# osmocom/osmo-trx

Hardware: AMD Instinct MI355X
Metric: Mbursts/s detect+demod (156.25 sym, 4 SPS) (higher is better)
Workload: dtype f32

## Files before the change

### osmo_trx_amd/csrc/trx_kernel_nb.hip

```cpp
#include "trx_k4_common.h"
#include "trx_nb_asm.inc"

#define NB_D_LEN    160
#define NB_CZ_LEN   (TRX_CZ_PAD + TRX_CORR_NARROW + TRX_CZ_PAD)
#define NB_SLICE    (K4_XS + NB_D_LEN + NB_CZ_LEN)
#define NB_COMP_ROWS (TRX_DELAY_FILTS + 1)
#define NB_TABLES_FLOATS (TRX_SINCV_LDS + 16 * WAVE + NB_COMP_ROWS * 36 + 16 + 8 * 8 + 5 * WAVE + 5 * WAVE + 2 * 8 * 16)
#define NB_TABLES_BYTES (NB_TABLES_FLOATS * 4)
#define NB_WPB 16
#define NB_POOL_RING 64
#define NB_POOL_UNSET (-1)
#define NB_POOL_END (-2)
#define NB_NO_BURST 0xffffffffu
#define NB_LDS_TAIL (16 + 4 * NB_POOL_RING)
#define NB_LDS_BYTES (NB_TABLES_BYTES + NB_WPB * NB_SLICE * 8 + NB_LDS_TAIL)
#define NB_MAX_TOA 32



typedef float v3f __attribute__((ext_vector_type(3)));
typedef int v4i __attribute__((ext_vector_type(4)));

template <typename T>
__device__ __forceinline__ unsigned lds_addr(const T *p)
{
	return (unsigned)(uintptr_t)(const __attribute__((address_space(3))) T *)p;
}

__global__ void __launch_bounds__(NB_WPB * WAVE)
nb_pull4_kernel(const uint32_t *__restrict__ iq, const trxhip_burst_params *__restrict__ params,
		trxhip_burst_result *__restrict__ results, float *__restrict__ soft, const trx_tables *__restrict__ tab,
		unsigned n_bursts, float thresh, float full_scale, unsigned *__restrict__ pool_ctr, unsigned *__restrict__ redo,
		float gk5, float gk6, float gk7, float gk8)
{
	static_assert(NB_TABLES_BYTES % 16 == 0 && (NB_SLICE * 8) % 16 == 0 && (K4_XS * 8) % 16 == 0 && (NB_D_LEN * 8) % 16 == 0, "16-byte LDS accesses");
	static_assert(NB_LDS_BYTES <= 160 * 1024, "LDS");
	static_assert(NB_ASM_GDEC_OFF == (TRX_SINCV_LDS + 16 * WAVE + NB_COMP_ROWS * 36) * 4, "tools/gen_nb_asm.py: LDS offset of the decimator taps");
	static_assert(NB_ASM_DEC_MAX_NACT == 15 + NB_ASM_CORR_MAX_LEN, "tools/gen_nb_asm.py: DEC and CORR change form at the same window");
	static_assert(NB_ASM_LSEQ_OFF == (NB_TABLES_FLOATS - 2 * 8 * 16) * 4, "tools/gen_nb_asm.py: LDS offset of the training-sequence taps");
	constexpr int NLD = 10;
	extern __shared__ __attribute__((aligned(16))) char smem[];
	const int lane0 = threadIdx.x & (WAVE - 1);
	const int wave = uni((int)(threadIdx.x >> 6));

	float *const sincv = reinterpret_cast<float *>(smem);
	float *const wa4f = sincv + TRX_SINCV_LDS;
	const float4 *const wa4 = reinterpret_cast<const float4 *>(wa4f);
	float *const comp = wa4f + 16 * WAVE;
	float *const gdec = comp + NB_COMP_ROWS * 36;
	float *const lhdr = gdec + 16;
	int *const pkcl = reinterpret_cast<int *>(lhdr + 8 * 8);
	int *const lcn = pkcl + 5 * WAVE;
	c32 *const lseq = reinterpret_cast<c32 *>(lcn + 5 * WAVE);
	c32 *const wbase = reinterpret_cast<c32 *>(smem + NB_TABLES_BYTES) + (size_t)wave * NB_SLICE;
	int *const wg_next = reinterpret_cast<int *>(reinterpret_cast<c32 *>(smem + NB_TABLES_BYTES) + (size_t)NB_WPB * NB_SLICE);
	int *const pool_g = wg_next + 4;
	c32 *const P = wbase;
	c32 *const D = wbase + K4_XS;
	c32 *const cz = D + NB_D_LEN + TRX_CZ_PAD;

	for (int i = threadIdx.x; i < TRX_SINCV_LDS; i += blockDim.x)
		sincv[i] = (i < TRX_SINCV_LEN) ? tab->sincv[i] : 0.0f;
	for (int i = threadIdx.x; i < 16 * WAVE; i += blockDim.x) {
		const int l = i & (WAVE - 1), u = i >> 6;
		const PeakConst pcl = peak_const(l);
		const int q = (u < 8) ? pcl.loA + 512 * (7 - u) : pcl.hiA + 512 * (u - 8);
		wa4f[((u >> 2) * WAVE + l) * 4 + (u & 3)] = (q < TRX_SINCV_LEN) ? tab->sincv[q] : 0.0f;
	}
	for (int i = threadIdx.x; i < NB_COMP_ROWS * 36; i += blockDim.x) {
		const int f = i / 36, j = i % 36;
		comp[i] = (j >= TRX_FUSED_SH) ? tab->comp_filt[f][j - TRX_FUSED_SH] : 0.0f;
	}
	if (threadIdx.x < 16)
		gdec[threadIdx.x] = tab->dec_taps[threadIdx.x];
	if (threadIdx.x < 128)
		lseq[threadIdx.x] = make_float2(tab->seq[TRX_SEQ_TSC0 + (threadIdx.x >> 4)].taps[threadIdx.x & 15].re,
						tab->seq[TRX_SEQ_TSC0 + (threadIdx.x >> 4)].taps[threadIdx.x & 15].im);
	if (threadIdx.x < 64)
		lhdr[threadIdx.x] = reinterpret_cast<const float *>(&tab->seq[TRX_SEQ_TSC0 + (threadIdx.x >> 3)].gain)[threadIdx.x & 7];
	if (threadIdx.x < WAVE) {
		const PeakConst pc0 = peak_const(threadIdx.x);
		pkcl[0 * WAVE + threadIdx.x] = pc0.flA;
		pkcl[1 * WAVE + threadIdx.x] = pc0.loA;
		pkcl[2 * WAVE + threadIdx.x] = pc0.hiA;
		pkcl[3 * WAVE + threadIdx.x] = pc0.offB;
		pkcl[4 * WAVE + threadIdx.x] = pc0.ratio_off;
		lcn[0 * WAVE + threadIdx.x] = pc0.ratio_off * 8;
		lcn[1 * WAVE + threadIdx.x] = (pc0.flA - 8) * 8;
		lcn[2 * WAVE + threadIdx.x] = pc0.offB;
		const int l = threadIdx.x, e = (l - 52) / 3, t = (l - 52) % 3;
		const bool sp = l >= 52;
		lcn[3 * WAVE + l] = 8 * (sp ? (t == 0 ? e : t == 1 ? e + 3 : e - 3) : 4 + 3 * (l < 49 ? l : 49));
		lcn[4 * WAVE + l] = sp ? (e + (t == 2 ? 4 : 0)) * K4_NTP * 4 : -1;
	}
	for (int i = lane0; i < NB_SLICE; i += WAVE)
		wbase[i] = make_float2(0.0f, 0.0f);
	if (threadIdx.x == 0) {
		wg_next[0] = NB_WPB;
		wg_next[1] = 0;
	}
	if (threadIdx.x < NB_POOL_RING)
		pool_g[threadIdx.x] = NB_POOL_UNSET;
	__syncthreads();

	const float fs_db = 6.02059991f * __log2f(full_scale);
	const float thr2 = thresh * thresh;
	const float gc0 = thr2 * 1.0001e-5f;
	int t5pk = 0;
	bool t5_ok = true;
	for (int t = 0; t < 8; t++) {
		const int v = (int)(lhdr[8 * t + 5] * 512.0f);
		t5_ok = t5_ok && v >= -8 && v <= 7 && (float)v == lhdr[8 * t + 5] * 512.0f;
		t5pk |= (v & 15) << (4 * t);
	}
	t5pk = uni(t5pk);
	const unsigned long long e8_addr = reinterpret_cast<unsigned long long>(&tab->edge8[0][0][0]);
	const unsigned n_wg = gridDim.x;
	const unsigned n_groups = (n_bursts + 15u) >> 4;
	const bool pooled = pool_ctr != nullptr;
	const unsigned n_static_groups = pooled ? ((n_groups - (n_groups >> 3)) / n_wg) * n_wg : n_groups;
	const unsigned n_pool_groups = n_groups - n_static_groups;
	const unsigned gq = n_static_groups / n_wg, gr = n_static_groups % n_wg;
	const unsigned my_groups = gq + (blockIdx.x < gr ? 1u : 0u);
	const unsigned base16 = (blockIdx.x * gq + (blockIdx.x < gr ? blockIdx.x : gr)) << 4;
	unsigned items = my_groups << 4;
	if (base16 + items > n_bursts)
		items = (base16 < n_bursts) ? n_bursts - base16 : 0u;
	auto burst_of = [&](unsigned jj) -> unsigned {
		if (jj < items)
			return base16 + jj;
		if (!pooled)
			return NB_NO_BURST;
		const unsigned k = (jj - items) >> 4;
		volatile int *slot = pool_g + (k & (NB_POOL_RING - 1));
		int g;
		while ((g = *slot) == NB_POOL_UNSET)
			__builtin_amdgcn_s_sleep(2);
		g = uni(g);
		if (g < 0)
			return NB_NO_BURST;
		const unsigned bb = ((n_static_groups + (unsigned)g) << 4) + (jj & 15u);
		return bb < n_bursts ? bb : NB_NO_BURST;
	};
	auto pool_draw = [&](unsigned jj, bool ended, int lane) {
		const unsigned k = (jj + 16u - items) >> 4;
		int g = NB_POOL_END;
		if (!ended) {
			unsigned p = 0;
			if (lane == 0)
				p = __hip_atomic_fetch_add(pool_ctr, 1u, __ATOMIC_RELAXED, __HIP_MEMORY_SCOPE_AGENT);
			p = (unsigned)uni((int)p);
			g = (p < n_pool_groups) ? (int)p : NB_POOL_END;
		}
		if (lane == 0) {
			pool_g[(k + NB_POOL_RING / 2) & (NB_POOL_RING - 1)] = NB_POOL_UNSET;
			pool_g[k & (NB_POOL_RING - 1)] = g;
		}
	};

	uint32_t pre_i[NLD];
	uint32_t pre_prm = 0u;
	auto prefetch = [&](unsigned bb, int lane) {
		pre_prm = reinterpret_cast<const uint32_t *>(params)[2 * (size_t)bb];
		const uint32_t *src = iq + (size_t)bb * 625;
		const unsigned ul = (unsigned)lane & 63u;
#pragma unroll
		for (int r = 0; r < NLD - 1; r++)
			pre_i[r] = __builtin_nontemporal_load(src + (unsigned)(r * WAVE) + ul);
		pre_i[NLD - 1] = __builtin_nontemporal_load(src + (unsigned)((NLD - 1) * WAVE) + min(ul, 48u));
	};
	const unsigned b_first = burst_of((unsigned)wave);
	if (b_first != NB_NO_BURST)
		prefetch(b_first, lane0);

	v3f o = { 0.0f, 0.0f, 0.0f };
	int recw = 0;
	bool pend_any = false;
	bool pend_rec = false;
	unsigned pend_b = 0;
	bool left_any = false;
	int q_xr = 0, q_xi = 0, q_es = 0, q_toa = 0, q_s = 0, q_fl = 0, q_b = 0;
	int q_n = 0;
	auto flush_records = [&](const int lane) {
		if (lane < q_n) {
			const float *const h = lhdr + 8 * (q_fl & 0xff);
			const float xr = __int_as_float(q_xr), xi = __int_as_float(q_xi);
			const float a0 = xr * h[2], a1 = xr * h[3], a2 = xi * h[3], a3 = xi * h[2];
			const float amp_re = a0 - a2, amp_im = a1 + a3;
			const float toa = (float)q_toa * 0.001953125f;
			const float energy = __int_as_float(q_es) * 0.0125f;
			const float rssi = fs_db - 3.01029996f * __log2f(energy);
			const float p2 = xi * xi + xr * xr;
			const float C = p2 * h[7];
			const float S = __int_as_float(q_s);
			const float ci = 3.0103f * __log2f(C * __builtin_amdgcn_rcpf(S - C));
			const v4i r0 = { 1, __float_as_int(toa), __float_as_int(amp_re), __float_as_int(amp_im) };
			const v4i r1 = { __float_as_int(ci), __float_as_int(energy), __float_as_int(rssi), q_fl };
			asm volatile("global_store_dwordx4 %0, %1, off\n\t"
				     "global_store_dwordx4 %0, %2, off offset:16\n\t"
				     "s_nop 1"
				     :: "v"(results + (unsigned)q_b), "v"(r0), "v"(r1) : "memory");
		}
		q_n = 0;
	};

	auto demod_general = [&](const int nk, const c32 ampv, const int lane) -> bool {
		constexpr int L = 625, nwrite = 148;
		c32 *const dec = D;
		const trx_tables *tabc = tab;
		asm volatile("" : "+s"(tabc));
		const int w = nk >> 7, fr = nk & 127;
		const int fidx = (fr >= 2) ? (fr >> 1) : TRX_DELAY_FILTS;
		const float ian = __builtin_amdgcn_rcpf(norm2(ampv));
		const c32 scale = make_float2(ampv.x * ian, -ampv.y * ian);
		const int n_lo = w > 0 ? w : 0;
		const int n_hi = (L - 1 + w < 623) ? L - 1 + w : 623;
		const int i_full_lo = cdiv4(n_lo + 15), i_full_hi = fdiv4(n_hi);
		const int i0l = cdiv4(n_lo), i0h = i_full_hi + 1;
		const bool need_lo = (n_hi >= n_lo) && (i0l < i_full_lo) && (i0l < nwrite);
		const bool need_hi = (n_hi >= n_lo) && (i0h <= fdiv4(n_hi + 15)) && (i0h < nwrite);
		const bool lo_tab = need_lo && (n_hi >= 4 * (i_full_lo - 1));
		float ct0 = 0.0f, ct1 = 0.0f, ct2 = 0.0f;
		const int le = lane >> 4, lt = lane & 15;
		const int li = i0l + le;
		const int lt0 = n_lo + 15 - 4 * li;
		const bool lact = lt0 >= 1;
		if (lo_tab) {
			const float *row = &tabc->edge_lo[fidx][(lact ? lt0 : 1) - 1][lt];
			ct0 = row[0];
			ct1 = row[16];
			ct2 = (lt < 4) ? row[32] : 0.0f;
		}
		const bool hi_tab = need_hi && (w <= -2) && (n_lo <= 4 * i0h - 15);
		if ((need_lo && !lo_tab) || (need_hi && !hi_tab))
			return false;
		float ch0 = 0.0f, ch1 = 0.0f, ch2 = 0.0f;
		const int hi_i = i0h + le;
		const int htm = n_hi + 15 - 4 * hi_i;
		const bool hact = htm >= 0;
		if (hi_tab) {
			const float *row = &tabc->edge_hi[fidx][hact ? htm : 0][lt];
			ch0 = row[0];
			ch1 = row[16];
			ch2 = (lt < 4) ? row[32] : 0.0f;
		}
		{
			const int c_full = -24 - w;
			const int i_min = cdiv4(-36 - c_full), i_max = fdiv4(L + 1 - c_full);
			int ic = 3 * lane;
			if (ic < i_min) ic = i_min;
			if (ic > i_max - 2) ic = i_max - 2;
			v2f acc[3];
			asm volatile(NB_ASM_FIRG
				     : [a0] "=&v"(acc[0]), [a1] "=&v"(acc[1]), [a2] "=&v"(acc[2])
				     : [nk] "s"(nk), [pb] "s"(lds_addr(P)), [cb] "s"(lds_addr(comp) + 4u * (K4_U0 + TRX_FUSED_SH)), [kic] "v"(8 * ic)
				     : NB_ASM_CLOBBERS);
			if (n_lo == 0 && lo_tab && i_full_hi >= nwrite - 1) {
				if (lane < 52) {
#pragma unroll
					for (int j = 0; j < 3; j++)
						dec[3 * lane + j] = cmul(make_float2(acc[j].x, acc[j].y), scale);
				}
			} else {
#pragma unroll
				for (int j = 0; j < 3; j++) {
					const int i = 3 * lane + j;
					const bool full = (i >= i_full_lo) && (i <= i_full_hi);
					const c32 d = full ? cmul(make_float2(acc[j].x, acc[j].y), scale) : make_float2(0.0f, 0.0f);
					if (i < 156)
						dec[i] = d;
				}
			}
		}
		if (lo_tab) {
			const int s0 = 4 * li - 24 - w + lt;
			const c32 *pp = P + ((s0 & 3) * PH_A + PH_M0 + (s0 >> 2));
			const c32 x0 = lds_c32(pp), x1 = lds_c32(pp + 4), x2 = lds_c32(pp + 8);
			float ar = x0.x * ct0, ai = x0.y * ct0;
			ar = fmaf(x1.x, ct1, ar); ai = fmaf(x1.y, ct1, ai);
			ar = fmaf(x2.x, ct2, ar); ai = fmaf(x2.y, ct2, ai);
			const float sr = row_sum(ar), si = row_sum(ai);
			if (lt == 0 && lact)
				dec[li] = cmul(make_float2(sr, si), scale);
		}
		if (hi_tab) {
			const int s0 = 4 * hi_i - 24 - w + lt;
			const c32 *pp = P + ((s0 & 3) * PH_A + PH_M0 + (s0 >> 2));
			const c32 x0 = lds_c32(pp), x1 = lds_c32(pp + 4), x2 = lds_c32(pp + 8);
			float ar = x0.x * ch0, ai = x0.y * ch0;
			ar = fmaf(x1.x, ch1, ar); ai = fmaf(x1.y, ch1, ai);
			ar = fmaf(x2.x, ch2, ar); ai = fmaf(x2.y, ch2, ai);
			const float sr = row_sum(ar), si = row_sum(ai);
			if (lt == 0 && hact && hi_i < 156)
				dec[hi_i] = cmul(make_float2(sr, si), scale);
		}
		wave_sync();
		auto pick = [&](int i) {
			const float d = reinterpret_cast<const float *>(dec + i)[i & 1];
			return __builtin_amdgcn_fmed3f(fmaf((i & 2) ? -0.5f : 0.5f, d, 0.5f), 0.0f, 1.0f);
		};
		const bool reg = lane >= 2 && lane < 50;
		const int i0 = reg ? 3 * lane - 2 : ((((lane - 54) * 11) >> 5) & 3);
		o.x = pick(i0);
		o.y = pick(reg ? i0 + 1 : 0);
		o.z = pick(reg ? i0 + 2 : 0);
		wave_sync();
		return true;
	};

	DIAG_DECL;
	unsigned j_next = 0, b_next = NB_NO_BURST;
	for (unsigned b = b_first; b != NB_NO_BURST; b = b_next) {
		int lane;
		asm volatile("v_mbcnt_lo_u32_b32 %0, -1, 0\n\tv_mbcnt_hi_u32_b32 %0, -1, %0" : "=v"(lane));
		const int ticket = claim_issue(wg_next);
		const unsigned prm0 = (unsigned)uni((int)pre_prm);
		const unsigned max_toa = prm0 >> 16;
		const int tsc = (prm0 >> 8) & 0xff;
		bool leave = ((prm0 & 0xf8ffu) != (unsigned)TRXHIP_TSC) || (max_toa > NB_MAX_TOA) || !t5_ok;

		c32 *const pload = P + (lane & 3) * PH_A + PH_M0 + (lane >> 2);
		float amax = 0.0f, epart = 0.0f;
#ifdef TRX_DIAG
		DIAG_MARK(12);
		asm volatile("s_waitcnt vmcnt(0)" ::: "memory");
		DIAG_MARK(13);
#endif
		if (!leave) {
#pragma unroll
			for (int r = 0; r < NLD; r++) {
				const int i = r * WAVE + lane;
				if (r < NLD - 1 || i < 625) {
					const c32 v = make_float2((float)(int16_t)(pre_i[r] & 0xffffu), (float)(int16_t)(pre_i[r] >> 16));
					pload[16 * r] = v;
					asm("v_max3_f32 %0, %0, |%1|, |%2|" : "+v"(amax) : "v"(v.x), "v"(v.y));
					if (r < 5)
						epart = fmaf(v.x, v.x, fmaf(v.y, v.y, epart));
				}
			}
		} else {
#pragma unroll
			for (int r = 0; r < NLD; r++)
				asm volatile("" :: "v"(pre_i[r]));
		}
		DIAG_MARK(14);
		if (pend_any) {
			float *const so = soft + (size_t)pend_b * 148;
			int *const rp = reinterpret_cast<int *>(results + pend_b);
			const float oe = o.x;
			asm volatile("s_bfm_b64 exec, 48, 2\n\t"
				     "global_store_dwordx3 %0, %1, %2 offset:16\n\t"
				     "s_mov_b32 exec_lo, 0\n\t"
			     "s_mov_b32 exec_hi, 0x92400000\n\t"
				     "global_store_dword %3, %4, %2\n\t"
				     "s_mov_b64 exec, %8\n\t"
				     "global_store_dword %5, %6, %7\n\t"
				     "s_mov_b64 exec, -1\n\t"
				     "s_nop 0"
				     :: "v"((lane - 2) * 12), "v"(o), "s"(so), "v"((((lane - 54) * 11) >> 5) * 4), "v"(oe), "v"(lane * 4), "v"(recw), "s"(rp),
				        "s"(pend_rec ? 0xffull : 0ull)
				     : "memory");
		}
		pend_any = false;
		DIAG_MARK(16);
		j_next = (unsigned)(leave ? claim_take(ticket) : claim_take_behind<5>(ticket));
		b_next = burst_of(j_next);
		if (pooled && (j_next & 15u) == 0u && j_next + 16u >= items)
			pool_draw(j_next, b_next == NB_NO_BURST && j_next >= items, lane);
		DIAG_MARK(17);
		if (b_next != NB_NO_BURST)
			prefetch(b_next, lane);
		DIAG_MARK(15);

		int clip = 0;
		if (!leave) {
			clip = __ballot(amax > TRX_CLIP_THRESH) != 0ull;

			const int len = 16 + (int)max_toa;
			__builtin_assume(len >= 16 && len <= 16 + NB_MAX_TOA);
			const unsigned vd_addr = lds_addr(D) + 8u * (unsigned)lane, vcz_addr = lds_addr(cz) + 8u * (unsigned)lane;
			unsigned long long bad;
			float dr, di;
			asm volatile(NB_ASM_DEC
				     : [bad] "=s"(bad), [dr] "=&v"(dr), [di] "=&v"(di)
				     : [pd] "v"(lds_addr(P + PH_M0 + 52) + 8u * (unsigned)lane), [vd] "v"(vd_addr), [vd4] "v"(vd_addr - 32u), [zero] "v"(0),
				       [nact] "s"(15 + len)
				     : NB_ASM_CLOBBERS);
			DIAG_MARK(2);
			{
				float v;
				const int lag0 = (len <= NB_ASM_CORR_MAX_LEN) ? NB_ASM_CORR_LANE0 : 0;
				asm volatile(NB_ASM_CORR
					     : [nrm] "=&v"(v)
					     : [vd] "v"(vd_addr), [vcz] "v"(vcz_addr), [vdm] "v"(vd_addr - 8u * NB_ASM_CORR_LANE0),
					       [vczm] "v"(vcz_addr - 8u * NB_ASM_CORR_LANE0), [dr] "v"(dr), [di] "v"(di), [len] "s"(len), [tsc] "s"(tsc), [bad] "s"(bad)
					     : NB_ASM_CLOBBERS);
				DIAG_MARK(3);
				int m_bits, es_bits, bidx;
				int kr, ka, kb, kic, ktp;
				asm volatile(NB_ASM_AMAX("ds_read_b32 %[kr], %[l4] offset:%c[lc]", "ds_read_b32 %[ka], %[l4] offset:%c[lc]+256",
							 "ds_read_b32 %[kb], %[l4] offset:%c[lc]+512", "ds_read_b32 %[kic], %[l4] offset:%c[lc]+768",
							 "ds_read_b32 %[ktp], %[l4] offset:%c[lc]+1024", "s_nop 0", "s_nop 0", "s_nop 0")
					     "s_sub_u32 %[bidx], %[bidx], %[lag0]\n\t"
					     "s_waitcnt lgkmcnt(0)"
					     : [m] "=&s"(m_bits), [es] "=&s"(es_bits), [bidx] "=&s"(bidx), [kr] "=&v"(kr), [ka] "=&v"(ka), [kb] "=&v"(kb),
					       [kic] "=&v"(kic), [ktp] "=&v"(ktp)
					     : [nrm] "v"(v), [ep] "v"(epart), [l4] "v"(4 * lane), [lag0] "s"(lag0),
					       [lc] "n"((TRX_SINCV_LDS + 16 * WAVE + NB_COMP_ROWS * 36 + 16 + 64 + 5 * WAVE) * 4)
					     : NB_ASM_CLOBBERS);
				DIAG_MARK(4);
				int hit = 0;
				int toa512 = 0;
				if (m_bits != 0) {
					int st, e512;
					float km;
					asm volatile(NB_ASM_DETA
						     : [st] "=&s"(st), [e] "=&s"(e512), [km] "=&v"(km)
						     : [bidx] "s"(bidx), [len] "s"(len), [czb] "s"(lds_addr(cz)), [kr] "v"(kr), [ka] "v"(ka), [l16] "v"(16 * lane),
						       [k5] "s"(gk5), [k6] "s"(gk6), [k7] "s"(gk7), [k8] "s"(gk8), [c0] "v"(gc0)
						     : NB_ASM_CLOBBERS);
					DIAG_MARK(5);
					int xr_bits = 0, xi_bits = 0;
					if (st == 1) {
						asm volatile(NB_ASM_DETB
							     : [st] "=&s"(st), [toa] "=&s"(toa512), [xr] "=&s"(xr_bits), [xi] "=&s"(xi_bits)
							     : [e] "s"(e512), [kb] "v"(kb), [czb] "s"(lds_addr(cz)), [km] "v"(km)
							     : NB_ASM_CLOBBERS);
						DIAG_MARK(6);
					}
					if (st == 3) {
						if (lane == 0)
							atomicAdd(&g_trx_fast_stats[0], 1ull);
						PeakConst pkc;
						pkc.flA = pkcl[0 * WAVE + lane]; pkc.loA = pkcl[1 * WAVE + lane]; pkc.hiA = pkcl[2 * WAVE + lane];
						pkc.offB = pkcl[3 * WAVE + lane]; pkc.ratio_off = pkcl[4 * WAVE + lane];
						c32 xcorr;
						peak_detect_spec(cz, bidx, sincv, pkc, lane, &toa512, &xcorr, wa4);
						toa512 = uni(toa512);
						xr_bits = uni(__float_as_int(xcorr.x));
						xi_bits = uni(__float_as_int(xcorr.y));
						st = 1;
					}
					if (st == 2) {
						leave = true;
						if (lane == 0) atomicAdd(&g_trx_fast_stats[2], 1ull);
					}
					if (st == 1) {
						hit = 1;
						int ok, s_bits;
						float d0, d1, d2;
						const int t5 = (t5pk << (28 - 4 * tsc)) >> 28;
						asm volatile("s_setprio 0");
						asm volatile(NB_ASM_TAIL
							     : [ok] "=&s"(ok), [ssum] "=&s"(s_bits), [d0] "=&v"(d0), [d1] "=&v"(d1), [d2] "=&v"(d2)
							     : [toa] "s"(toa512), [xr] "s"(xr_bits), [xi] "s"(xi_bits), [t5] "s"(t5), [hdrb] "s"(lds_addr(lhdr) + 32u * (unsigned)tsc),
							       [e8lo] "s"((unsigned)e8_addr), [e8hi] "s"((unsigned)(e8_addr >> 32)), [l16] "v"(16 * lane),
							       [vd] "v"(vd_addr), [pb] "s"(lds_addr(P)), [cb] "s"(lds_addr(comp) + 4u * (K4_U0 + TRX_FUSED_SH)), [db] "s"(lds_addr(D)),
							       [kic] "v"(kic), [ktp] "v"(ktp)
							     : NB_ASM_CLOBBERS);
						DIAG_MARK(10);
						asm volatile("s_setprio 2");
						if (!ok) {
							if (lane == 0) atomicAdd(&g_trx_fast_stats[3], 1ull);
							const float *const h = lhdr + 8 * tsc;
							const float xr = __int_as_float(xr_bits), xi = __int_as_float(xi_bits);
							const float a0 = xr * h[2], a1 = xr * h[3], a2 = xi * h[3], a3 = xi * h[2];
							const c32 ampv = make_float2(unif(a0 - a2), unif(a1 + a3));
							if (!demod_general(t5 + 10 * 512 - toa512, ampv, lane))
								leave = true;
						}
						if (!leave) {
							asm("s_lshl_b64 exec, 1, %[n]\n\t"
						    "v_mov_b32_e32 %[qxr], %[xr]\n\t"
						    "v_mov_b32_e32 %[qxi], %[xi]\n\t"
						    "v_mov_b32_e32 %[qes], %[es]\n\t"
						    "v_mov_b32_e32 %[qtoa], %[toa]\n\t"
						    "v_mov_b32_e32 %[qs], %[ss]\n\t"
						    "v_mov_b32_e32 %[qfl], %[fl]\n\t"
						    "v_mov_b32_e32 %[qb], %[b]\n\t"
						    "s_mov_b64 exec, -1"
						    : [qxr] "+v"(q_xr), [qxi] "+v"(q_xi), [qes] "+v"(q_es), [qtoa] "+v"(q_toa), [qs] "+v"(q_s), [qfl] "+v"(q_fl),
						      [qb] "+v"(q_b)
						    : [n] "s"(uni(q_n)), [xr] "s"(xr_bits), [xi] "s"(xi_bits), [es] "s"(es_bits), [toa] "s"(toa512 - t5 - 10 * 512),
						      [ss] "s"(s_bits), [fl] "s"((int)((uint32_t)tsc | ((uint32_t)clip << 8) | (37u << 24))), [b] "s"((int)b));
						q_n++;
						}
						if (ok) {
							o.x = __builtin_amdgcn_fmed3f(fmaf(0.5f, d0, 0.5f), 0.0f, 1.0f);
							o.y = __builtin_amdgcn_fmed3f(fmaf(0.5f, d1, 0.5f), 0.0f, 1.0f);
							o.z = __builtin_amdgcn_fmed3f(fmaf(0.5f, d2, 0.5f), 0.0f, 1.0f);
						}
					}
				}
				if (!hit && !leave) {
					const float energy = __int_as_float(es_bits) * 0.0125f;
					const float rssi = fs_db - 3.01029996f * __log2f(energy);
					const uint32_t flags = ((uint32_t)clip << 8) | (1u << 16);
					int word = clip ? -TRXHIP_SIGERR_CLIP : 0;
					word = put_lane<1>(word, 0.0f);
					word = put_lane<2>(word, 0.0f);
					word = put_lane<3>(word, 0.0f);
					word = put_lane<4>(word, 0.0f);
					word = put_lane<5>(word, energy);
					word = put_lane<6>(word, rssi);
					word = write_lane<7>(word, (int)flags);
					recw = word;
					o = (v3f){ 0.0f, 0.0f, 0.0f };
				}
				pend_rec = !hit;
			}
		}
		if (leave) {
			if (lane == 0) {
				reinterpret_cast<uint8_t *>(redo + TRX_REDO_HDR)[b] = 1;
				if (!left_any)
					__hip_atomic_store(redo, 1u, __ATOMIC_RELAXED, __HIP_MEMORY_SCOPE_AGENT);
			}
			left_any = true;
			continue;
		}
		pend_b = b;
		pend_any = true;
		if (q_n == WAVE)
			flush_records(lane);
		DIAG_MARK(11);
	}
	if (pend_any) {
		int lane;
		asm volatile("v_mbcnt_lo_u32_b32 %0, -1, 0\n\tv_mbcnt_hi_u32_b32 %0, -1, %0" : "=v"(lane));
		float *const so = soft + (size_t)pend_b * 148;
		int *const rp = reinterpret_cast<int *>(results + pend_b);
		const float oe = o.x;
		asm volatile("s_bfm_b64 exec, 48, 2\n\t"
			     "global_store_dwordx3 %0, %1, %2 offset:16\n\t"
		     "s_mov_b32 exec_lo, 0\n\t"
		     "s_mov_b32 exec_hi, 0x92400000\n\t"
			     "global_store_dword %3, %4, %2\n\t"
			     "s_mov_b64 exec, %8\n\t"
			     "global_store_dword %5, %6, %7\n\t"
			     "s_mov_b64 exec, -1\n\t"
			     "s_nop 0"
			     :: "v"((lane - 2) * 12), "v"(o), "s"(so), "v"((((lane - 54) * 11) >> 5) * 4), "v"(oe), "v"(lane * 4), "v"(recw), "s"(rp),
			        "s"(pend_rec ? 0xffull : 0ull)
			     : "memory");
	}
	{
		int lane;
		asm volatile("v_mbcnt_lo_u32_b32 %0, -1, 0\n\tv_mbcnt_hi_u32_b32 %0, -1, %0" : "=v"(lane));
		flush_records(lane);
	}
	DIAG_FLUSH();
	if (pooled) {
		__syncthreads();
		int tid0;
		asm volatile("v_mbcnt_lo_u32_b32 %0, -1, 0\n\tv_mbcnt_hi_u32_b32 %0, -1, %0" : "=v"(tid0));
		if (tid0 == 0 && atomicAdd(wg_next + 1, 1) == 0) {
			const unsigned d = __hip_atomic_fetch_add(pool_ctr + 1, 1u, __ATOMIC_ACQ_REL, __HIP_MEMORY_SCOPE_AGENT);
			if (d == gridDim.x - 1u) {
				__hip_atomic_store(pool_ctr, 0u, __ATOMIC_RELAXED, __HIP_MEMORY_SCOPE_AGENT);
				__hip_atomic_store(pool_ctr + 1, 0u, __ATOMIC_RELEASE, __HIP_MEMORY_SCOPE_AGENT);
			}
		}
	}
}
```

### osmo_trx_amd/csrc/trx_nb_asm.inc

```
#define NB_ASM_GDEC_OFF 29968
#define NB_ASM_LSEQ_OFF 32848
#define NB_ASM_DEC_MAX_NACT 60
#define NB_ASM_CORR_LANE0 19
#define NB_ASM_CORR_MAX_LEN 45
#define NB_ASM_CLOBBERS "v64", "v65", "v66", "v67", "v68", "v69", "v70", "v71", "v72", "v73", "v74", "v75", "v76", "v77", "v78", "v79", "v80", "v81", "v82", "v83", "v84", "v85", "v86", "v87", "v88", "v89", "v90", "v91", "v92", "v93", "v94", "v95", "v96", "v97", "v98", "v99", "v100", "v101", "v102", "v103", "v104", "v105", "v106", "v107", "v108", "v109", "v110", "v111", "v112", "v113", "v114", "v115", "v116", "v117", "v118", "v119", "v120", "v121", "v122", "v123", "v124", "v125", "v126", "v127", "s87", "s88", "s89", "s90", "s91", "s92", "s93", "s94", "s95", "s96", "s97", "s98", "s99", "vcc", "scc", "memory"
#define NB_ASM_DEC \
	"s_cmp_gt_u32 %[nact], 60\n\t" \
	"s_cbranch_scc1 .Lnb_dec_wide\n\t" \
	"s_sub_u32 s88, 60, %[nact]\n\t" \
	"s_lshr_b64 exec, -1, s88\n\t" \
	"ds_read_b128 v[120:123], %[zero] offset:29968\n\t" \
	"ds_read_b128 v[124:127], %[zero] offset:29984\n\t" \
	"ds_read_b64 v[98:99], %[pd] offset:1440\n\t" \
	"ds_read_b64 v[100:101], %[pd] offset:2880\n\t" \
	"ds_read_b64 v[102:103], %[pd] offset:4320\n\t" \
	"ds_read_b64 v[96:97], %[pd] offset:0\n\t" \
	"s_waitcnt lgkmcnt(3)\n\t" \
	"v_pk_mul_f32 v[64:65], v[98:99], v[120:121] op_sel:[0,0] op_sel_hi:[1,0]\n\t" \
	"s_waitcnt lgkmcnt(2)\n\t" \
	"v_pk_mul_f32 v[66:67], v[100:101], v[120:121] op_sel:[0,1] op_sel_hi:[1,1]\n\t" \
	"s_waitcnt lgkmcnt(1)\n\t" \
	"v_pk_mul_f32 v[68:69], v[102:103], v[122:123] op_sel:[0,0] op_sel_hi:[1,0]\n\t" \
	"v_pk_add_f32 v[104:105], v[64:65], v[66:67]\n\t" \
	"s_waitcnt lgkmcnt(0)\n\t" \
	"v_pk_mul_f32 v[70:71], v[96:97], v[122:123] op_sel:[0,1] op_sel_hi:[1,1]\n\t" \
	"v_pk_add_f32 v[104:105], v[104:105], v[68:69]\n\t" \
	"v_pk_mul_f32 v[72:73], v[98:99], v[124:125] op_sel:[0,0] op_sel_hi:[1,0]\n\t" \
	"v_pk_mul_f32 v[74:75], v[100:101], v[124:125] op_sel:[0,1] op_sel_hi:[1,1]\n\t" \
	"v_add_f32_dpp v104, v104, v70 wave_shr:1 row_mask:0xf bank_mask:0xf bound_ctrl:0\n\t" \
	"v_add_f32_dpp v105, v105, v71 wave_shr:1 row_mask:0xf bank_mask:0xf bound_ctrl:0\n\t" \
	"v_pk_mul_f32 v[76:77], v[102:103], v[126:127] op_sel:[0,0] op_sel_hi:[1,0]\n\t" \
	"v_pk_add_f32 v[104:105], v[104:105], v[72:73]\n\t" \
	"v_pk_mul_f32 v[78:79], v[96:97], v[126:127] op_sel:[0,1] op_sel_hi:[1,1]\n\t" \
	"v_pk_add_f32 v[104:105], v[104:105], v[74:75]\n\t" \
	"v_pk_mul_f32 v[80:81], v[98:99], v[126:127] op_sel:[0,1] op_sel_hi:[1,1]\n\t" \
	"v_pk_add_f32 v[104:105], v[104:105], v[76:77]\n\t" \
	"v_pk_mul_f32 v[82:83], v[100:101], v[126:127] op_sel:[0,0] op_sel_hi:[1,0]\n\t" \
	"v_pk_mul_f32 v[84:85], v[102:103], v[124:125] op_sel:[0,1] op_sel_hi:[1,1]\n\t" \
	"v_add_f32_dpp v104, v104, v78 wave_shr:1 row_mask:0xf bank_mask:0xf bound_ctrl:0\n\t" \
	"v_add_f32_dpp v105, v105, v79 wave_shr:1 row_mask:0xf bank_mask:0xf bound_ctrl:0\n\t" \
	"v_pk_mul_f32 v[86:87], v[96:97], v[124:125] op_sel:[0,0] op_sel_hi:[1,0]\n\t" \
	"v_pk_add_f32 v[104:105], v[104:105], v[80:81]\n\t" \
	"v_pk_mul_f32 v[88:89], v[98:99], v[122:123] op_sel:[0,1] op_sel_hi:[1,1]\n\t" \
	"v_pk_add_f32 v[104:105], v[104:105], v[82:83]\n\t" \
	"v_pk_mul_f32 v[90:91], v[100:101], v[122:123] op_sel:[0,0] op_sel_hi:[1,0]\n\t" \
	"v_pk_add_f32 v[104:105], v[104:105], v[84:85]\n\t" \
	"v_pk_mul_f32 v[92:93], v[102:103], v[120:121] op_sel:[0,1] op_sel_hi:[1,1]\n\t" \
	"v_pk_mul_f32 v[94:95], v[96:97], v[120:121] op_sel:[0,0] op_sel_hi:[1,0]\n\t" \
	"v_add_f32_dpp v104, v104, v86 wave_shr:1 row_mask:0xf bank_mask:0xf bound_ctrl:0\n\t" \
	"v_add_f32_dpp v105, v105, v87 wave_shr:1 row_mask:0xf bank_mask:0xf bound_ctrl:0\n\t" \
	"v_pk_add_f32 v[104:105], v[104:105], v[88:89]\n\t" \
	"s_nop 0\n\t" \
	"v_pk_add_f32 v[104:105], v[104:105], v[90:91]\n\t" \
	"s_nop 0\n\t" \
	"v_pk_add_f32 v[104:105], v[104:105], v[92:93]\n\t" \
	"s_nop 1\n\t" \
	"v_add_f32_dpp %[dr], v104, v94 wave_shr:1 row_mask:0xf bank_mask:0xf bound_ctrl:0\n\t" \
	"v_add_f32_dpp %[di], v105, v95 wave_shr:1 row_mask:0xf bank_mask:0xf bound_ctrl:0\n\t" \
	"s_bfm_b64 exec, %[nact], 4\n\t" \
	"ds_write2_b32 %[vd4], %[dr], %[di] offset1:1\n\t" \
	"v_min_f32_e64 v106, |%[dr]|, |%[di]|\n\t" \
	"v_max_f32_e64 v107, |%[dr]|, |%[di]|\n\t" \
	"v_ldexp_f32 v106, v106, 17\n\t" \
	"v_cmp_lt_f32_e32 vcc, v106, v107\n\t" \
	"s_mov_b64 exec, -1\n\t" \
	"s_mov_b64 %[bad], vcc\n\t" \
	"s_waitcnt lgkmcnt(0)\n\t" \
	"s_branch .Lnb_dec_end\n\t" \
	".Lnb_dec_wide:\n\t" \
	"s_bfm_b64 exec, %[nact], 0\n\t" \
	"ds_read_b128 v[120:123], %[zero] offset:29968\n\t" \
	"ds_read_b128 v[124:127], %[zero] offset:29984\n\t" \
	"ds_read_b64 v[88:89], %[pd] offset:1440\n\t" \
	"ds_read_b64 v[90:91], %[pd] offset:2880\n\t" \
	"ds_read_b64 v[92:93], %[pd] offset:4320\n\t" \
	"ds_read_b64 v[94:95], %[pd] offset:8\n\t" \
	"ds_read_b64 v[96:97], %[pd] offset:1448\n\t" \
	"ds_read_b64 v[98:99], %[pd] offset:2888\n\t" \
	"ds_read_b64 v[100:101], %[pd] offset:4328\n\t" \
	"ds_read_b64 v[102:103], %[pd] offset:16\n\t" \
	"ds_read_b64 v[104:105], %[pd] offset:1456\n\t" \
	"ds_read_b64 v[106:107], %[pd] offset:2896\n\t" \
	"ds_read_b64 v[108:109], %[pd] offset:4336\n\t" \
	"ds_read_b64 v[110:111], %[pd] offset:24\n\t" \
	"ds_read_b64 v[112:113], %[pd] offset:1464\n\t" \
	"ds_read_b64 v[114:115], %[pd] offset:2904\n\t" \
	"ds_read_b64 v[116:117], %[pd] offset:4344\n\t" \
	"ds_read_b64 v[118:119], %[pd] offset:32\n\t" \
	"s_waitcnt lgkmcnt(12)\n\t" \
	"v_pk_mul_f32 v[88:89], v[88:89], v[120:121] op_sel:[0,0] op_sel_hi:[1,0]\n\t" \
	"v_pk_mul_f32 v[90:91], v[90:91], v[120:121] op_sel:[0,1] op_sel_hi:[1,1]\n\t" \
	"v_pk_mul_f32 v[92:93], v[92:93], v[122:123] op_sel:[0,0] op_sel_hi:[1,0]\n\t" \
	"v_pk_add_f32 v[88:89], v[88:89], v[90:91]\n\t" \
	"v_pk_mul_f32 v[94:95], v[94:95], v[122:123] op_sel:[0,1] op_sel_hi:[1,1]\n\t" \
	"v_pk_add_f32 v[88:89], v[88:89], v[92:93]\n\t" \
	"s_waitcnt lgkmcnt(8)\n\t" \
	"v_pk_mul_f32 v[96:97], v[96:97], v[124:125] op_sel:[0,0] op_sel_hi:[1,0]\n\t" \
	"v_pk_add_f32 v[88:89], v[88:89], v[94:95]\n\t" \
	"v_pk_mul_f32 v[98:99], v[98:99], v[124:125] op_sel:[0,1] op_sel_hi:[1,1]\n\t" \
	"v_pk_add_f32 v[88:89], v[88:89], v[96:97]\n\t" \
	"v_pk_mul_f32 v[100:101], v[100:101], v[126:127] op_sel:[0,0] op_sel_hi:[1,0]\n\t" \
	"v_pk_add_f32 v[88:89], v[88:89], v[98:99]\n\t" \
	"v_pk_mul_f32 v[102:103], v[102:103], v[126:127] op_sel:[0,1] op_sel_hi:[1,1]\n\t" \
	"v_pk_add_f32 v[88:89], v[88:89], v[100:101]\n\t" \
	"s_waitcnt lgkmcnt(4)\n\t" \
	"v_pk_mul_f32 v[104:105], v[104:105], v[126:127] op_sel:[0,1] op_sel_hi:[1,1]\n\t" \
	"v_pk_add_f32 v[88:89], v[88:89], v[102:103]\n\t" \
	"v_pk_mul_f32 v[106:107], v[106:107], v[126:127] op_sel:[0,0] op_sel_hi:[1,0]\n\t" \
	"v_pk_add_f32 v[88:89], v[88:89], v[104:105]\n\t" \
	"v_pk_mul_f32 v[108:109], v[108:109], v[124:125] op_sel:[0,1] op_sel_hi:[1,1]\n\t" \
	"v_pk_add_f32 v[88:89], v[88:89], v[106:107]\n\t" \
	"v_pk_mul_f32 v[110:111], v[110:111], v[124:125] op_sel:[0,0] op_sel_hi:[1,0]\n\t" \
	"v_pk_add_f32 v[88:89], v[88:89], v[108:109]\n\t" \
	"s_waitcnt lgkmcnt(0)\n\t" \
	"v_pk_mul_f32 v[112:113], v[112:113], v[122:123] op_sel:[0,1] op_sel_hi:[1,1]\n\t" \
	"v_pk_add_f32 v[88:89], v[88:89], v[110:111]\n\t" \
	"v_pk_mul_f32 v[114:115], v[114:115], v[122:123] op_sel:[0,0] op_sel_hi:[1,0]\n\t" \
	"v_pk_add_f32 v[88:89], v[88:89], v[112:113]\n\t" \
	"v_pk_mul_f32 v[116:117], v[116:117], v[120:121] op_sel:[0,1] op_sel_hi:[1,1]\n\t" \
	"v_pk_add_f32 v[88:89], v[88:89], v[114:115]\n\t" \
	"v_pk_mul_f32 v[118:119], v[118:119], v[120:121] op_sel:[0,0] op_sel_hi:[1,0]\n\t" \
	"v_pk_add_f32 v[88:89], v[88:89], v[116:117]\n\t" \
	"s_nop 0\n\t" \
	"v_pk_add_f32 v[88:89], v[88:89], v[118:119]\n\t" \
	"ds_write_b64 %[vd], v[88:89]\n\t" \
	"v_min_f32_e64 v90, |v88|, |v89|\n\t" \
	"v_max_f32_e64 v91, |v88|, |v89|\n\t" \
	"v_ldexp_f32 v90, v90, 17\n\t" \
	"v_cmp_lt_f32_e32 vcc, v90, v91\n\t" \
	"s_mov_b64 exec, -1\n\t" \
	"s_mov_b64 %[bad], vcc\n\t" \
	"s_waitcnt lgkmcnt(0)\n\t" \
	".Lnb_dec_end:\n\t"
#define NB_ASM_CORR \
	"s_cmp_gt_u32 %[len], 45\n\t" \
	"s_cbranch_scc1 .Lnb_corr_wide\n\t" \
	"v_mov_b64_e32 v[120:121], 0\n\t" \
	"v_mov_b64_e32 v[122:123], 0\n\t" \
	"v_mov_b32_e32 %[nrm], 0\n\t" \
	"s_lshl_b32 s90, %[len], 3\n\t" \
	"s_sub_u32 s91, 45, %[len]\n\t" \
	"v_add_u32_e32 v64, s90, %[vcz]\n\t" \
	"s_lshr_b64 exec, -1, s91\n\t" \
	"s_cmp_lg_u64 %[bad], 0\n\t" \
	"s_cbranch_scc1 .Lnb_corrr_mul\n\t" \
	"s_getpc_b64 s[88:89]\n\t" \
	".Lnb_corrr_pc:\n\t" \
	"s_mul_i32 s90, %[tsc], .Lnb_corrr_v1-.Lnb_corrr_v0\n\t" \
	"s_add_u32 s88, s88, s90\n\t" \
	"s_addc_u32 s89, s89, 0\n\t" \
	"s_add_u32 s88, s88, .Lnb_corrr_v0-.Lnb_corrr_pc\n\t" \
	"s_addc_u32 s89, s89, 0\n\t" \
	"s_setpc_b64 s[88:89]\n\t" \
	".Lnb_corrr_v0:\n\t" \
	"v_sub_f32_e32 v120, 0, %[dr]\n\t" \
	"v_sub_f32_e32 v121, 0, %[di]\n\t" \
	"s_nop 0\n\t" \
	"v_add_f32_dpp v120, v120, %[di] wave_shr:1 row_mask:0xf bank_mask:0xf bound_ctrl:0\n\t" \
	"v_sub_f32_dpp v121, v121, %[dr] wave_shr:1 row_mask:0xf bank_mask:0xf bound_ctrl:0\n\t" \
	"s_nop 0\n\t" \
	"v_add_f32_dpp v120, v120, %[dr] wave_shr:1 row_mask:0xf bank_mask:0xf bound_ctrl:0\n\t" \
	"v_add_f32_dpp v121, v121, %[di] wave_shr:1 row_mask:0xf bank_mask:0xf bound_ctrl:0\n\t" \
	"s_nop 0\n\t" \
	"v_add_f32_dpp v120, v120, %[di] wave_shr:1 row_mask:0xf bank_mask:0xf bound_ctrl:0\n\t" \
	"v_sub_f32_dpp v121, v121, %[dr] wave_shr:1 row_mask:0xf bank_mask:0xf bound_ctrl:0\n\t" \
	"s_nop 0\n\t" \
	"v_sub_f32_dpp v120, v120, %[dr] wave_shr:1 row_mask:0xf bank_mask:0xf bound_ctrl:0\n\t" \
	"v_sub_f32_dpp v121, v121, %[di] wave_shr:1 row_mask:0xf bank_mask:0xf bound_ctrl:0\n\t" \
	"s_nop 0\n\t" \
	"v_add_f32_dpp v120, v120, %[di] wave_shr:1 row_mask:0xf bank_mask:0xf bound_ctrl:0\n\t" \
	"v_sub_f32_dpp v121, v121, %[dr] wave_shr:1 row_mask:0xf bank_mask:0xf bound_ctrl:0\n\t" \
	"s_nop 0\n\t" \
	"v_sub_f32_dpp v120, v120, %[dr] wave_shr:1 row_mask:0xf bank_mask:0xf bound_ctrl:0\n\t" \
	"v_sub_f32_dpp v121, v121, %[di] wave_shr:1 row_mask:0xf bank_mask:0xf bound_ctrl:0\n\t" \
	"s_nop 0\n\t" \
	"v_sub_f32_dpp v120, v120, %[di] wave_shr:1 row_mask:0xf bank_mask:0xf bound_ctrl:0\n\t" \
	"v_add_f32_dpp v121, v121, %[dr] wave_shr:1 row_mask:0xf bank_mask:0xf bound_ctrl:0\n\t" \
	"s_nop 0\n\t" \
	"v_add_f32_dpp v120, v120, %[dr] wave_shr:1 row_mask:0xf bank_mask:0xf bound_ctrl:0\n\t" \
	"v_add_f32_dpp v121, v121, %[di] wave_shr:1 row_mask:0xf bank_mask:0xf bound_ctrl:0\n\t" \
	"s_nop 0\n\t" \
	"v_sub_f32_dpp v120, v120, %[di] wave_shr:1 row_mask:0xf bank_mask:0xf bound_ctrl:0\n\t" \
	"v_add_f32_dpp v121, v121, %[dr] wave_shr:1 row_mask:0xf bank_mask:0xf bound_ctrl:0\n\t" \
	"s_nop 0\n\t" \
	"v_sub_f32_dpp v120, v120, %[dr] wave_shr:1 row_mask:0xf bank_mask:0xf bound_ctrl:0\n\t" \
	"v_sub_f32_dpp v121, v121, %[di] wave_shr:1 row_mask:0xf bank_mask:0xf bound_ctrl:0\n\t" \
	"s_nop 0\n\t" \
	"v_sub_f32_dpp v120, v120, %[di] wave_shr:1 row_mask:0xf bank_mask:0xf bound_ctrl:0\n\t" \
	"v_add_f32_dpp v121, v121, %[dr] wave_shr:1 row_mask:0xf bank_mask:0xf bound_ctrl:0\n\t" \
	"s_nop 0\n\t" \
	"v_add_f32_dpp v120, v120, %[dr] wave_shr:1 row_mask:0xf bank_mask:0xf bound_ctrl:0\n\t" \
	"v_add_f32_dpp v121, v121, %[di] wave_shr:1 row_mask:0xf bank_mask:0xf bound_ctrl:0\n\t" \
	"s_nop 0\n\t" \
	"v_sub_f32_dpp v120, v120, %[di] wave_shr:1 row_mask:0xf bank_mask:0xf bound_ctrl:0\n\t" \
	"v_add_f32_dpp v121, v121, %[dr] wave_shr:1 row_mask:0xf bank_mask:0xf bound_ctrl:0\n\t" \
	"s_nop 0\n\t" \
	"v_sub_f32_dpp v120, v120, %[dr] wave_shr:1 row_mask:0xf bank_mask:0xf bound_ctrl:0\n\t" \
	"v_sub_f32_dpp v121, v121, %[di] wave_shr:1 row_mask:0xf bank_mask:0xf bound_ctrl:0\n\t" \
	"s_nop 0\n\t" \
	"v_sub_f32_dpp v120, v120, %[di] wave_shr:1 row_mask:0xf bank_mask:0xf bound_ctrl:0\n\t" \
	"v_add_f32_dpp v121, v121, %[dr] wave_shr:1 row_mask:0xf bank_mask:0xf bound_ctrl:0\n\t" \
	"s_branch .Lnb_corrr_join\n\t" \
	".Lnb_corrr_v1:\n\t" \
	"v_sub_f32_e32 v120, 0, %[dr]\n\t" \
	"v_sub_f32_e32 v121, 0, %[di]\n\t" \
	"s_nop 0\n\t" \
	"v_add_f32_dpp v120, v120, %[di] wave_shr:1 row_mask:0xf bank_mask:0xf bound_ctrl:0\n\t" \
	"v_sub_f32_dpp v121, v121, %[dr] wave_shr:1 row_mask:0xf bank_mask:0xf bound_ctrl:0\n\t" \
	"s_nop 0\n\t" \
	"v_add_f32_dpp v120, v120, %[dr] wave_shr:1 row_mask:0xf bank_mask:0xf bound_ctrl:0\n\t" \
	"v_add_f32_dpp v121, v121, %[di] wave_shr:1 row_mask:0xf bank_mask:0xf bound_ctrl:0\n\t" \
	"s_nop 0\n\t" \
	"v_add_f32_dpp v120, v120, %[di] wave_shr:1 row_mask:0xf bank_mask:0xf bound_ctrl:0\n\t" \
	"v_sub_f32_dpp v121, v121, %[dr] wave_shr:1 row_mask:0xf bank_mask:0xf bound_ctrl:0\n\t" \
	"s_nop 0\n\t" \
	"v_sub_f32_dpp v120, v120, %[dr] wave_shr:1 row_mask:0xf bank_mask:0xf bound_ctrl:0\n\t" \
	"v_sub_f32_dpp v121, v121, %[di] wave_shr:1 row_mask:0xf bank_mask:0xf bound_ctrl:0\n\t" \
	"s_nop 0\n\t" \
	"v_add_f32_dpp v120, v120, %[di] wave_shr:1 row_mask:0xf bank_mask:0xf bound_ctrl:0\n\t" \
	"v_sub_f32_dpp v121, v121, %[dr] wave_shr:1 row_mask:0xf bank_mask:0xf bound_ctrl:0\n\t" \
	"s_nop 0\n\t" \
	"v_add_f32_dpp v120, v120, %[dr] wave_shr:1 row_mask:0xf bank_mask:0xf bound_ctrl:0\n\t" \
	"v_add_f32_dpp v121, v121, %[di] wave_shr:1 row_mask:0xf bank_mask:0xf bound_ctrl:0\n\t" \
	"s_nop 0\n\t" \
	"v_add_f32_dpp v120, v120, %[di] wave_shr:1 row_mask:0xf bank_mask:0xf bound_ctrl:0\n\t" \
	"v_sub_f32_dpp v121, v121, %[dr] wave_shr:1 row_mask:0xf bank_mask:0xf bound_ctrl:0\n\t" \
	"s_nop 0\n\t" \
	"v_sub_f32_dpp v120, v120, %[dr] wave_shr:1 row_mask:0xf bank_mask:0xf bound_ctrl:0\n\t" \
	"v_sub_f32_dpp v121, v121, %[di] wave_shr:1 row_mask:0xf bank_mask:0xf bound_ctrl:0\n\t" \
	"s_nop 0\n\t" \
	"v_sub_f32_dpp v120, v120, %[di] wave_shr:1 row_mask:0xf bank_mask:0xf bound_ctrl:0\n\t" \
	"v_add_f32_dpp v121, v121, %[dr] wave_shr:1 row_mask:0xf bank_mask:0xf bound_ctrl:0\n\t" \
	"s_nop 0\n\t" \
	"v_sub_f32_dpp v120, v120, %[dr] wave_shr:1 row_mask:0xf bank_mask:0xf bound_ctrl:0\n\t" \
	"v_sub_f32_dpp v121, v121, %[di] wave_shr:1 row_mask:0xf bank_mask:0xf bound_ctrl:0\n\t" \
	"s_nop 0\n\t" \
	"v_sub_f32_dpp v120, v120, %[di] wave_shr:1 row_mask:0xf bank_mask:0xf bound_ctrl:0\n\t" \
	"v_add_f32_dpp v121, v121, %[dr] wave_shr:1 row_mask:0xf bank_mask:0xf bound_ctrl:0\n\t" \
	"s_nop 0\n\t" \
	"v_add_f32_dpp v120, v120, %[dr] wave_shr:1 row_mask:0xf bank_mask:0xf bound_ctrl:0\n\t" \
	"v_add_f32_dpp v121, v121, %[di] wave_shr:1 row_mask:0xf bank_mask:0xf bound_ctrl:0\n\t" \
	"s_nop 0\n\t" \
	"v_sub_f32_dpp v120, v120, %[di] wave_shr:1 row_mask:0xf bank_mask:0xf bound_ctrl:0\n\t" \
	"v_add_f32_dpp v121, v121, %[dr] wave_shr:1 row_mask:0xf bank_mask:0xf bound_ctrl:0\n\t" \
	"s_nop 0\n\t" \
	"v_sub_f32_dpp v120, v120, %[dr] wave_shr:1 row_mask:0xf bank_mask:0xf bound_ctrl:0\n\t" \
	"v_sub_f32_dpp v121, v121, %[di] wave_shr:1 row_mask:0xf bank_mask:0xf bound_ctrl:0\n\t" \
	"s_nop 0\n\t" \
	"v_add_f32_dpp v120, v120, %[di] wave_shr:1 row_mask:0xf bank_mask:0xf bound_ctrl:0\n\t" \
	"v_sub_f32_dpp v121, v121, %[dr] wave_shr:1 row_mask:0xf bank_mask:0xf bound_ctrl:0\n\t" \
	"s_branch .Lnb_corrr_join\n\t" \
	".Lnb_corrr_v2:\n\t" \
	"v_add_f32_e32 v120, 0, %[dr]\n\t" \
	"v_add_f32_e32 v121, 0, %[di]\n\t" \
	"s_nop 0\n\t" \
	"v_sub_f32_dpp v120, v120, %[di] wave_shr:1 row_mask:0xf bank_mask:0xf bound_ctrl:0\n\t" \
	"v_add_f32_dpp v121, v121, %[dr] wave_shr:1 row_mask:0xf bank_mask:0xf bound_ctrl:0\n\t" \
	"s_nop 0\n\t" \
	"v_add_f32_dpp v120, v120, %[dr] wave_shr:1 row_mask:0xf bank_mask:0xf bound_ctrl:0\n\t" \
	"v_add_f32_dpp v121, v121, %[di] wave_shr:1 row_mask:0xf bank_mask:0xf bound_ctrl:0\n\t" \
	"s_nop 0\n\t" \
	"v_add_f32_dpp v120, v120, %[di] wave_shr:1 row_mask:0xf bank_mask:0xf bound_ctrl:0\n\t" \
	"v_sub_f32_dpp v121, v121, %[dr] wave_shr:1 row_mask:0xf bank_mask:0xf bound_ctrl:0\n\t" \
	"s_nop 0\n\t" \
	"v_add_f32_dpp v120, v120, %[dr] wave_shr:1 row_mask:0xf bank_mask:0xf bound_ctrl:0\n\t" \
	"v_add_f32_dpp v121, v121, %[di] wave_shr:1 row_mask:0xf bank_mask:0xf bound_ctrl:0\n\t" \
	"s_nop 0\n\t" \
	"v_sub_f32_dpp v120, v120, %[di] wave_shr:1 row_mask:0xf bank_mask:0xf bound_ctrl:0\n\t" \
	"v_add_f32_dpp v121, v121, %[dr] wave_shr:1 row_mask:0xf bank_mask:0xf bound_ctrl:0\n\t" \
	"s_nop 0\n\t" \
	"v_add_f32_dpp v120, v120, %[dr] wave_shr:1 row_mask:0xf bank_mask:0xf bound_ctrl:0\n\t" \
	"v_add_f32_dpp v121, v121, %[di] wave_shr:1 row_mask:0xf bank_mask:0xf bound_ctrl:0\n\t" \
	"s_nop 0\n\t" \
	"v_add_f32_dpp v120, v120, %[di] wave_shr:1 row_mask:0xf bank_mask:0xf bound_ctrl:0\n\t" \
	"v_sub_f32_dpp v121, v121, %[dr] wave_shr:1 row_mask:0xf bank_mask:0xf bound_ctrl:0\n\t" \
	"s_nop 0\n\t" \
	"v_add_f32_dpp v120, v120, %[dr] wave_shr:1 row_mask:0xf bank_mask:0xf bound_ctrl:0\n\t" \
	"v_add_f32_dpp v121, v121, %[di] wave_shr:1 row_mask:0xf bank_mask:0xf bound_ctrl:0\n\t" \
	"s_nop 0\n\t" \
	"v_sub_f32_dpp v120, v120, %[di] wave_shr:1 row_mask:0xf bank_mask:0xf bound_ctrl:0\n\t" \
	"v_add_f32_dpp v121, v121, %[dr] wave_shr:1 row_mask:0xf bank_mask:0xf bound_ctrl:0\n\t" \
	"s_nop 0\n\t" \
	"v_sub_f32_dpp v120, v120, %[dr] wave_shr:1 row_mask:0xf bank_mask:0xf bound_ctrl:0\n\t" \
	"v_sub_f32_dpp v121, v121, %[di] wave_shr:1 row_mask:0xf bank_mask:0xf bound_ctrl:0\n\t" \
	"s_nop 0\n\t" \
	"v_sub_f32_dpp v120, v120, %[di] wave_shr:1 row_mask:0xf bank_mask:0xf bound_ctrl:0\n\t" \
	"v_add_f32_dpp v121, v121, %[dr] wave_shr:1 row_mask:0xf bank_mask:0xf bound_ctrl:0\n\t" \
	"s_nop 0\n\t" \
	"v_sub_f32_dpp v120, v120, %[dr] wave_shr:1 row_mask:0xf bank_mask:0xf bound_ctrl:0\n\t" \
	"v_sub_f32_dpp v121, v121, %[di] wave_shr:1 row_mask:0xf bank_mask:0xf bound_ctrl:0\n\t" \
	"s_nop 0\n\t" \
	"v_add_f32_dpp v120, v120, %[di] wave_shr:1 row_mask:0xf bank_mask:0xf bound_ctrl:0\n\t" \
	"v_sub_f32_dpp v121, v121, %[dr] wave_shr:1 row_mask:0xf bank_mask:0xf bound_ctrl:0\n\t" \
	"s_nop 0\n\t" \
	"v_sub_f32_dpp v120, v120, %[dr] wave_shr:1 row_mask:0xf bank_mask:0xf bound_ctrl:0\n\t" \
	"v_sub_f32_dpp v121, v121, %[di] wave_shr:1 row_mask:0xf bank_mask:0xf bound_ctrl:0\n\t" \
	"s_nop 0\n\t" \
	"v_sub_f32_dpp v120, v120, %[di] wave_shr:1 row_mask:0xf bank_mask:0xf bound_ctrl:0\n\t" \
	"v_add_f32_dpp v121, v121, %[dr] wave_shr:1 row_mask:0xf bank_mask:0xf bound_ctrl:0\n\t" \
	"s_branch .Lnb_corrr_join\n\t" \
	".Lnb_corrr_v3:\n\t" \
	"v_sub_f32_e32 v120, 0, %[dr]\n\t" \
	"v_sub_f32_e32 v121, 0, %[di]\n\t" \
	"s_nop 0\n\t" \
	"v_sub_f32_dpp v120, v120, %[di] wave_shr:1 row_mask:0xf bank_mask:0xf bound_ctrl:0\n\t" \
	"v_add_f32_dpp v121, v121, %[dr] wave_shr:1 row_mask:0xf bank_mask:0xf bound_ctrl:0\n\t" \
	"s_nop 0\n\t" \
	"v_add_f32_dpp v120, v120, %[dr] wave_shr:1 row_mask:0xf bank_mask:0xf bound_ctrl:0\n\t" \
	"v_add_f32_dpp v121, v121, %[di] wave_shr:1 row_mask:0xf bank_mask:0xf bound_ctrl:0\n\t" \
	"s_nop 0\n\t" \
	"v_add_f32_dpp v120, v120, %[di] wave_shr:1 row_mask:0xf bank_mask:0xf bound_ctrl:0\n\t" \
	"v_sub_f32_dpp v121, v121, %[dr] wave_shr:1 row_mask:0xf bank_mask:0xf bound_ctrl:0\n\t" \
	"s_nop 0\n\t" \
	"v_add_f32_dpp v120, v120, %[dr] wave_shr:1 row_mask:0xf bank_mask:0xf bound_ctrl:0\n\t" \
	"v_add_f32_dpp v121, v121, %[di] wave_shr:1 row_mask:0xf bank_mask:0xf bound_ctrl:0\n\t" \
	"s_nop 0\n\t" \
	"v_sub_f32_dpp v120, v120, %[di] wave_shr:1 row_mask:0xf bank_mask:0xf bound_ctrl:0\n\t" \
	"v_add_f32_dpp v121, v121, %[dr] wave_shr:1 row_mask:0xf bank_mask:0xf bound_ctrl:0\n\t" \
	"s_nop 0\n\t" \
	"v_add_f32_dpp v120, v120, %[dr] wave_shr:1 row_mask:0xf bank_mask:0xf bound_ctrl:0\n\t" \
	"v_add_f32_dpp v121, v121, %[di] wave_shr:1 row_mask:0xf bank_mask:0xf bound_ctrl:0\n\t" \
	"s_nop 0\n\t" \
	"v_sub_f32_dpp v120, v120, %[di] wave_shr:1 row_mask:0xf bank_mask:0xf bound_ctrl:0\n\t" \
	"v_add_f32_dpp v121, v121, %[dr] wave_shr:1 row_mask:0xf bank_mask:0xf bound_ctrl:0\n\t" \
	"s_nop 0\n\t" \
	"v_sub_f32_dpp v120, v120, %[dr] wave_shr:1 row_mask:0xf bank_mask:0xf bound_ctrl:0\n\t" \
	"v_sub_f32_dpp v121, v121, %[di] wave_shr:1 row_mask:0xf bank_mask:0xf bound_ctrl:0\n\t" \
	"s_nop 0\n\t" \
	"v_add_f32_dpp v120, v120, %[di] wave_shr:1 row_mask:0xf bank_mask:0xf bound_ctrl:0\n\t" \
	"v_sub_f32_dpp v121, v121, %[dr] wave_shr:1 row_mask:0xf bank_mask:0xf bound_ctrl:0\n\t" \
	"s_nop 0\n\t" \
	"v_sub_f32_dpp v120, v120, %[dr] wave_shr:1 row_mask:0xf bank_mask:0xf bound_ctrl:0\n\t" \
	"v_sub_f32_dpp v121, v121, %[di] wave_shr:1 row_mask:0xf bank_mask:0xf bound_ctrl:0\n\t" \
	"s_nop 0\n\t" \
	"v_sub_f32_dpp v120, v120, %[di] wave_shr:1 row_mask:0xf bank_mask:0xf bound_ctrl:0\n\t" \
	"v_add_f32_dpp v121, v121, %[dr] wave_shr:1 row_mask:0xf bank_mask:0xf bound_ctrl:0\n\t" \
	"s_nop 0\n\t" \
	"v_sub_f32_dpp v120, v120, %[dr] wave_shr:1 row_mask:0xf bank_mask:0xf bound_ctrl:0\n\t" \
	"v_sub_f32_dpp v121, v121, %[di] wave_shr:1 row_mask:0xf bank_mask:0xf bound_ctrl:0\n\t" \
	"s_nop 0\n\t" \
	"v_add_f32_dpp v120, v120, %[di] wave_shr:1 row_mask:0xf bank_mask:0xf bound_ctrl:0\n\t" \
	"v_sub_f32_dpp v121, v121, %[dr] wave_shr:1 row_mask:0xf bank_mask:0xf bound_ctrl:0\n\t" \
	"s_nop 0\n\t" \
	"v_sub_f32_dpp v120, v120, %[dr] wave_shr:1 row_mask:0xf bank_mask:0xf bound_ctrl:0\n\t" \
	"v_sub_f32_dpp v121, v121, %[di] wave_shr:1 row_mask:0xf bank_mask:0xf bound_ctrl:0\n\t" \
	"s_nop 0\n\t" \
	"v_sub_f32_dpp v120, v120, %[di] wave_shr:1 row_mask:0xf bank_mask:0xf bound_ctrl:0\n\t" \
	"v_add_f32_dpp v121, v121, %[dr] wave_shr:1 row_mask:0xf bank_mask:0xf bound_ctrl:0\n\t" \
	"s_branch .Lnb_corrr_join\n\t" \
	".Lnb_corrr_v4:\n\t" \
	"v_add_f32_e32 v120, 0, %[dr]\n\t" \
	"v_add_f32_e32 v121, 0, %[di]\n\t" \
	"s_nop 0\n\t" \
	"v_sub_f32_dpp v120, v120, %[di] wave_shr:1 row_mask:0xf bank_mask:0xf bound_ctrl:0\n\t" \
	"v_add_f32_dpp v121, v121, %[dr] wave_shr:1 row_mask:0xf bank_mask:0xf bound_ctrl:0\n\t" \
	"s_nop 0\n\t" \
	"v_sub_f32_dpp v120, v120, %[dr] wave_shr:1 row_mask:0xf bank_mask:0xf bound_ctrl:0\n\t" \
	"v_sub_f32_dpp v121, v121, %[di] wave_shr:1 row_mask:0xf bank_mask:0xf bound_ctrl:0\n\t" \
	"s_nop 0\n\t" \
	"v_add_f32_dpp v120, v120, %[di] wave_shr:1 row_mask:0xf bank_mask:0xf bound_ctrl:0\n\t" \
	"v_sub_f32_dpp v121, v121, %[dr] wave_shr:1 row_mask:0xf bank_mask:0xf bound_ctrl:0\n\t" \
	"s_nop 0\n\t" \
	"v_sub_f32_dpp v120, v120, %[dr] wave_shr:1 row_mask:0xf bank_mask:0xf bound_ctrl:0\n\t" \
	"v_sub_f32_dpp v121, v121, %[di] wave_shr:1 row_mask:0xf bank_mask:0xf bound_ctrl:0\n\t" \
	"s_nop 0\n\t" \
	"v_sub_f32_dpp v120, v120, %[di] wave_shr:1 row_mask:0xf bank_mask:0xf bound_ctrl:0\n\t" \
	"v_add_f32_dpp v121, v121, %[dr] wave_shr:1 row_mask:0xf bank_mask:0xf bound_ctrl:0\n\t" \
	"s_nop 0\n\t" \
	"v_sub_f32_dpp v120, v120, %[dr] wave_shr:1 row_mask:0xf bank_mask:0xf bound_ctrl:0\n\t" \
	"v_sub_f32_dpp v121, v121, %[di] wave_shr:1 row_mask:0xf bank_mask:0xf bound_ctrl:0\n\t" \
	"s_nop 0\n\t" \
	"v_sub_f32_dpp v120, v120, %[di] wave_shr:1 row_mask:0xf bank_mask:0xf bound_ctrl:0\n\t" \
	"v_add_f32_dpp v121, v121, %[dr] wave_shr:1 row_mask:0xf bank_mask:0xf bound_ctrl:0\n\t" \
	"s_nop 0\n\t" \
	"v_sub_f32_dpp v120, v120, %[dr] wave_shr:1 row_mask:0xf bank_mask:0xf bound_ctrl:0\n\t" \
	"v_sub_f32_dpp v121, v121, %[di] wave_shr:1 row_mask:0xf bank_mask:0xf bound_ctrl:0\n\t" \
	"s_nop 0\n\t" \
	"v_add_f32_dpp v120, v120, %[di] wave_shr:1 row_mask:0xf bank_mask:0xf bound_ctrl:0\n\t" \
	"v_sub_f32_dpp v121, v121, %[dr] wave_shr:1 row_mask:0xf bank_mask:0xf bound_ctrl:0\n\t" \
	"s_nop 0\n\t" \
	"v_sub_f32_dpp v120, v120, %[dr] wave_shr:1 row_mask:0xf bank_mask:0xf bound_ctrl:0\n\t" \
	"v_sub_f32_dpp v121, v121, %[di] wave_shr:1 row_mask:0xf bank_mask:0xf bound_ctrl:0\n\t" \
	"s_nop 0\n\t" \
	"v_sub_f32_dpp v120, v120, %[di] wave_shr:1 row_mask:0xf bank_mask:0xf bound_ctrl:0\n\t" \
	"v_add_f32_dpp v121, v121, %[dr] wave_shr:1 row_mask:0xf bank_mask:0xf bound_ctrl:0\n\t" \
	"s_nop 0\n\t" \
	"v_add_f32_dpp v120, v120, %[dr] wave_shr:1 row_mask:0xf bank_mask:0xf bound_ctrl:0\n\t" \
	"v_add_f32_dpp v121, v121, %[di] wave_shr:1 row_mask:0xf bank_mask:0xf bound_ctrl:0\n\t" \
	"s_nop 0\n\t" \
	"v_add_f32_dpp v120, v120, %[di] wave_shr:1 row_mask:0xf bank_mask:0xf bound_ctrl:0\n\t" \
	"v_sub_f32_dpp v121, v121, %[dr] wave_shr:1 row_mask:0xf bank_mask:0xf bound_ctrl:0\n\t" \
	"s_nop 0\n\t" \
	"v_add_f32_dpp v120, v120, %[dr] wave_shr:1 row_mask:0xf bank_mask:0xf bound_ctrl:0\n\t" \
	"v_add_f32_dpp v121, v121, %[di] wave_shr:1 row_mask:0xf bank_mask:0xf bound_ctrl:0\n\t" \
	"s_nop 0\n\t" \
	"v_add_f32_dpp v120, v120, %[di] wave_shr:1 row_mask:0xf bank_mask:0xf bound_ctrl:0\n\t" \
	"v_sub_f32_dpp v121, v121, %[dr] wave_shr:1 row_mask:0xf bank_mask:0xf bound_ctrl:0\n\t" \
	"s_branch .Lnb_corrr_join\n\t" \
	".Lnb_corrr_v5:\n\t" \
	"v_sub_f32_e32 v120, 0, %[dr]\n\t" \
	"v_sub_f32_e32 v121, 0, %[di]\n\t" \
	"s_nop 0\n\t" \
	"v_sub_f32_dpp v120, v120, %[di] wave_shr:1 row_mask:0xf bank_mask:0xf bound_ctrl:0\n\t" \
	"v_add_f32_dpp v121, v121, %[dr] wave_shr:1 row_mask:0xf bank_mask:0xf bound_ctrl:0\n\t" \
	"s_nop 0\n\t" \
	"v_sub_f32_dpp v120, v120, %[dr] wave_shr:1 row_mask:0xf bank_mask:0xf bound_ctrl:0\n\t" \
	"v_sub_f32_dpp v121, v121, %[di] wave_shr:1 row_mask:0xf bank_mask:0xf bound_ctrl:0\n\t" \
	"s_nop 0\n\t" \
	"v_add_f32_dpp v120, v120, %[di] wave_shr:1 row_mask:0xf bank_mask:0xf bound_ctrl:0\n\t" \
	"v_sub_f32_dpp v121, v121, %[dr] wave_shr:1 row_mask:0xf bank_mask:0xf bound_ctrl:0\n\t" \
	"s_nop 0\n\t" \
	"v_add_f32_dpp v120, v120, %[dr] wave_shr:1 row_mask:0xf bank_mask:0xf bound_ctrl:0\n\t" \
	"v_add_f32_dpp v121, v121, %[di] wave_shr:1 row_mask:0xf bank_mask:0xf bound_ctrl:0\n\t" \
	"s_nop 0\n\t" \
	"v_sub_f32_dpp v120, v120, %[di] wave_shr:1 row_mask:0xf bank_mask:0xf bound_ctrl:0\n\t" \
	"v_add_f32_dpp v121, v121, %[dr] wave_shr:1 row_mask:0xf bank_mask:0xf bound_ctrl:0\n\t" \
	"s_nop 0\n\t" \
	"v_add_f32_dpp v120, v120, %[dr] wave_shr:1 row_mask:0xf bank_mask:0xf bound_ctrl:0\n\t" \
	"v_add_f32_dpp v121, v121, %[di] wave_shr:1 row_mask:0xf bank_mask:0xf bound_ctrl:0\n\t" \
	"s_nop 0\n\t" \
	"v_sub_f32_dpp v120, v120, %[di] wave_shr:1 row_mask:0xf bank_mask:0xf bound_ctrl:0\n\t" \
	"v_add_f32_dpp v121, v121, %[dr] wave_shr:1 row_mask:0xf bank_mask:0xf bound_ctrl:0\n\t" \
	"s_nop 0\n\t" \
	"v_add_f32_dpp v120, v120, %[dr] wave_shr:1 row_mask:0xf bank_mask:0xf bound_ctrl:0\n\t" \
	"v_add_f32_dpp v121, v121, %[di] wave_shr:1 row_mask:0xf bank_mask:0xf bound_ctrl:0\n\t" \
	"s_nop 0\n\t" \
	"v_add_f32_dpp v120, v120, %[di] wave_shr:1 row_mask:0xf bank_mask:0xf bound_ctrl:0\n\t" \
	"v_sub_f32_dpp v121, v121, %[dr] wave_shr:1 row_mask:0xf bank_mask:0xf bound_ctrl:0\n\t" \
	"s_nop 0\n\t" \
	"v_sub_f32_dpp v120, v120, %[dr] wave_shr:1 row_mask:0xf bank_mask:0xf bound_ctrl:0\n\t" \
	"v_sub_f32_dpp v121, v121, %[di] wave_shr:1 row_mask:0xf bank_mask:0xf bound_ctrl:0\n\t" \
	"s_nop 0\n\t" \
	"v_sub_f32_dpp v120, v120, %[di] wave_shr:1 row_mask:0xf bank_mask:0xf bound_ctrl:0\n\t" \
	"v_add_f32_dpp v121, v121, %[dr] wave_shr:1 row_mask:0xf bank_mask:0xf bound_ctrl:0\n\t" \
	"s_nop 0\n\t" \
	"v_sub_f32_dpp v120, v120, %[dr] wave_shr:1 row_mask:0xf bank_mask:0xf bound_ctrl:0\n\t" \
	"v_sub_f32_dpp v121, v121, %[di] wave_shr:1 row_mask:0xf bank_mask:0xf bound_ctrl:0\n\t" \
	"s_nop 0\n\t" \
	"v_add_f32_dpp v120, v120, %[di] wave_shr:1 row_mask:0xf bank_mask:0xf bound_ctrl:0\n\t" \
	"v_sub_f32_dpp v121, v121, %[dr] wave_shr:1 row_mask:0xf bank_mask:0xf bound_ctrl:0\n\t" \
	"s_nop 0\n\t" \
	"v_sub_f32_dpp v120, v120, %[dr] wave_shr:1 row_mask:0xf bank_mask:0xf bound_ctrl:0\n\t" \
	"v_sub_f32_dpp v121, v121, %[di] wave_shr:1 row_mask:0xf bank_mask:0xf bound_ctrl:0\n\t" \
	"s_nop 0\n\t" \
	"v_add_f32_dpp v120, v120, %[di] wave_shr:1 row_mask:0xf bank_mask:0xf bound_ctrl:0\n\t" \
	"v_sub_f32_dpp v121, v121, %[dr] wave_shr:1 row_mask:0xf bank_mask:0xf bound_ctrl:0\n\t" \
	"s_branch .Lnb_corrr_join\n\t" \
	".Lnb_corrr_v6:\n\t" \
	"v_sub_f32_e32 v120, 0, %[dr]\n\t" \
	"v_sub_f32_e32 v121, 0, %[di]\n\t" \
	"s_nop 0\n\t" \
	"v_sub_f32_dpp v120, v120, %[di] wave_shr:1 row_mask:0xf bank_mask:0xf bound_ctrl:0\n\t" \
	"v_add_f32_dpp v121, v121, %[dr] wave_shr:1 row_mask:0xf bank_mask:0xf bound_ctrl:0\n\t" \
	"s_nop 0\n\t" \
	"v_add_f32_dpp v120, v120, %[dr] wave_shr:1 row_mask:0xf bank_mask:0xf bound_ctrl:0\n\t" \
	"v_add_f32_dpp v121, v121, %[di] wave_shr:1 row_mask:0xf bank_mask:0xf bound_ctrl:0\n\t" \
	"s_nop 0\n\t" \
	"v_add_f32_dpp v120, v120, %[di] wave_shr:1 row_mask:0xf bank_mask:0xf bound_ctrl:0\n\t" \
	"v_sub_f32_dpp v121, v121, %[dr] wave_shr:1 row_mask:0xf bank_mask:0xf bound_ctrl:0\n\t" \
	"s_nop 0\n\t" \
	"v_sub_f32_dpp v120, v120, %[dr] wave_shr:1 row_mask:0xf bank_mask:0xf bound_ctrl:0\n\t" \
	"v_sub_f32_dpp v121, v121, %[di] wave_shr:1 row_mask:0xf bank_mask:0xf bound_ctrl:0\n\t" \
	"s_nop 0\n\t" \
	"v_add_f32_dpp v120, v120, %[di] wave_shr:1 row_mask:0xf bank_mask:0xf bound_ctrl:0\n\t" \
	"v_sub_f32_dpp v121, v121, %[dr] wave_shr:1 row_mask:0xf bank_mask:0xf bound_ctrl:0\n\t" \
	"s_nop 0\n\t" \
	"v_add_f32_dpp v120, v120, %[dr] wave_shr:1 row_mask:0xf bank_mask:0xf bound_ctrl:0\n\t" \
	"v_add_f32_dpp v121, v121, %[di] wave_shr:1 row_mask:0xf bank_mask:0xf bound_ctrl:0\n\t" \
	"s_nop 0\n\t" \
	"v_add_f32_dpp v120, v120, %[di] wave_shr:1 row_mask:0xf bank_mask:0xf bound_ctrl:0\n\t" \
	"v_sub_f32_dpp v121, v121, %[dr] wave_shr:1 row_mask:0xf bank_mask:0xf bound_ctrl:0\n\t" \
	"s_nop 0\n\t" \
	"v_add_f32_dpp v120, v120, %[dr] wave_shr:1 row_mask:0xf bank_mask:0xf bound_ctrl:0\n\t" \
	"v_add_f32_dpp v121, v121, %[di] wave_shr:1 row_mask:0xf bank_mask:0xf bound_ctrl:0\n\t" \
	"s_nop 0\n\t" \
	"v_add_f32_dpp v120, v120, %[di] wave_shr:1 row_mask:0xf bank_mask:0xf bound_ctrl:0\n\t" \
	"v_sub_f32_dpp v121, v121, %[dr] wave_shr:1 row_mask:0xf bank_mask:0xf bound_ctrl:0\n\t" \
	"s_nop 0\n\t" \
	"v_sub_f32_dpp v120, v120, %[dr] wave_shr:1 row_mask:0xf bank_mask:0xf bound_ctrl:0\n\t" \
	"v_sub_f32_dpp v121, v121, %[di] wave_shr:1 row_mask:0xf bank_mask:0xf bound_ctrl:0\n\t" \
	"s_nop 0\n\t" \
	"v_add_f32_dpp v120, v120, %[di] wave_shr:1 row_mask:0xf bank_mask:0xf bound_ctrl:0\n\t" \
	"v_sub_f32_dpp v121, v121, %[dr] wave_shr:1 row_mask:0xf bank_mask:0xf bound_ctrl:0\n\t" \
	"s_nop 0\n\t" \
	"v_add_f32_dpp v120, v120, %[dr] wave_shr:1 row_mask:0xf bank_mask:0xf bound_ctrl:0\n\t" \
	"v_add_f32_dpp v121, v121, %[di] wave_shr:1 row_mask:0xf bank_mask:0xf bound_ctrl:0\n\t" \
	"s_nop 0\n\t" \
	"v_sub_f32_dpp v120, v120, %[di] wave_shr:1 row_mask:0xf bank_mask:0xf bound_ctrl:0\n\t" \
	"v_add_f32_dpp v121, v121, %[dr] wave_shr:1 row_mask:0xf bank_mask:0xf bound_ctrl:0\n\t" \
	"s_nop 0\n\t" \
	"v_sub_f32_dpp v120, v120, %[dr] wave_shr:1 row_mask:0xf bank_mask:0xf bound_ctrl:0\n\t" \
	"v_sub_f32_dpp v121, v121, %[di] wave_shr:1 row_mask:0xf bank_mask:0xf bound_ctrl:0\n\t" \
	"s_nop 0\n\t" \
	"v_sub_f32_dpp v120, v120, %[di] wave_shr:1 row_mask:0xf bank_mask:0xf bound_ctrl:0\n\t" \
	"v_add_f32_dpp v121, v121, %[dr] wave_shr:1 row_mask:0xf bank_mask:0xf bound_ctrl:0\n\t" \
	"s_branch .Lnb_corrr_join\n\t" \
	".Lnb_corrr_v7:\n\t" \
	"v_sub_f32_e32 v120, 0, %[dr]\n\t" \
	"v_sub_f32_e32 v121, 0, %[di]\n\t" \
	"s_nop 0\n\t" \
	"v_sub_f32_dpp v120, v120, %[di] wave_shr:1 row_mask:0xf bank_mask:0xf bound_ctrl:0\n\t" \
	"v_add_f32_dpp v121, v121, %[dr] wave_shr:1 row_mask:0xf bank_mask:0xf bound_ctrl:0\n\t" \
	"s_nop 0\n\t" \
	"v_add_f32_dpp v120, v120, %[dr] wave_shr:1 row_mask:0xf bank_mask:0xf bound_ctrl:0\n\t" \
	"v_add_f32_dpp v121, v121, %[di] wave_shr:1 row_mask:0xf bank_mask:0xf bound_ctrl:0\n\t" \
	"s_nop 0\n\t" \
	"v_sub_f32_dpp v120, v120, %[di] wave_shr:1 row_mask:0xf bank_mask:0xf bound_ctrl:0\n\t" \
	"v_add_f32_dpp v121, v121, %[dr] wave_shr:1 row_mask:0xf bank_mask:0xf bound_ctrl:0\n\t" \
	"s_nop 0\n\t" \
	"v_add_f32_dpp v120, v120, %[dr] wave_shr:1 row_mask:0xf bank_mask:0xf bound_ctrl:0\n\t" \
	"v_add_f32_dpp v121, v121, %[di] wave_shr:1 row_mask:0xf bank_mask:0xf bound_ctrl:0\n\t" \
	"s_nop 0\n\t" \
	"v_add_f32_dpp v120, v120, %[di] wave_shr:1 row_mask:0xf bank_mask:0xf bound_ctrl:0\n\t" \
	"v_sub_f32_dpp v121, v121, %[dr] wave_shr:1 row_mask:0xf bank_mask:0xf bound_ctrl:0\n\t" \
	"s_nop 0\n\t" \
	"v_add_f32_dpp v120, v120, %[dr] wave_shr:1 row_mask:0xf bank_mask:0xf bound_ctrl:0\n\t" \
	"v_add_f32_dpp v121, v121, %[di] wave_shr:1 row_mask:0xf bank_mask:0xf bound_ctrl:0\n\t" \
	"s_nop 0\n\t" \
	"v_sub_f32_dpp v120, v120, %[di] wave_shr:1 row_mask:0xf bank_mask:0xf bound_ctrl:0\n\t" \
	"v_add_f32_dpp v121, v121, %[dr] wave_shr:1 row_mask:0xf bank_mask:0xf bound_ctrl:0\n\t" \
	"s_nop 0\n\t" \
	"v_add_f32_dpp v120, v120, %[dr] wave_shr:1 row_mask:0xf bank_mask:0xf bound_ctrl:0\n\t" \
	"v_add_f32_dpp v121, v121, %[di] wave_shr:1 row_mask:0xf bank_mask:0xf bound_ctrl:0\n\t" \
	"s_nop 0\n\t" \
	"v_sub_f32_dpp v120, v120, %[di] wave_shr:1 row_mask:0xf bank_mask:0xf bound_ctrl:0\n\t" \
	"v_add_f32_dpp v121, v121, %[dr] wave_shr:1 row_mask:0xf bank_mask:0xf bound_ctrl:0\n\t" \
	"s_nop 0\n\t" \
	"v_sub_f32_dpp v120, v120, %[dr] wave_shr:1 row_mask:0xf bank_mask:0xf bound_ctrl:0\n\t" \
	"v_sub_f32_dpp v121, v121, %[di] wave_shr:1 row_mask:0xf bank_mask:0xf bound_ctrl:0\n\t" \
	"s_nop 0\n\t" \
	"v_add_f32_dpp v120, v120, %[di] wave_shr:1 row_mask:0xf bank_mask:0xf bound_ctrl:0\n\t" \
	"v_sub_f32_dpp v121, v121, %[dr] wave_shr:1 row_mask:0xf bank_mask:0xf bound_ctrl:0\n\t" \
	"s_nop 0\n\t" \
	"v_sub_f32_dpp v120, v120, %[dr] wave_shr:1 row_mask:0xf bank_mask:0xf bound_ctrl:0\n\t" \
	"v_sub_f32_dpp v121, v121, %[di] wave_shr:1 row_mask:0xf bank_mask:0xf bound_ctrl:0\n\t" \
	"s_nop 0\n\t" \
	"v_sub_f32_dpp v120, v120, %[di] wave_shr:1 row_mask:0xf bank_mask:0xf bound_ctrl:0\n\t" \
	"v_add_f32_dpp v121, v121, %[dr] wave_shr:1 row_mask:0xf bank_mask:0xf bound_ctrl:0\n\t" \
	"s_nop 0\n\t" \
	"v_sub_f32_dpp v120, v120, %[dr] wave_shr:1 row_mask:0xf bank_mask:0xf bound_ctrl:0\n\t" \
	"v_sub_f32_dpp v121, v121, %[di] wave_shr:1 row_mask:0xf bank_mask:0xf bound_ctrl:0\n\t" \
	"s_nop 0\n\t" \
	"v_add_f32_dpp v120, v120, %[di] wave_shr:1 row_mask:0xf bank_mask:0xf bound_ctrl:0\n\t" \
	"v_sub_f32_dpp v121, v121, %[dr] wave_shr:1 row_mask:0xf bank_mask:0xf bound_ctrl:0\n\t" \
	"s_branch .Lnb_corrr_join\n\t" \
	".Lnb_corrr_join:\n\t" \
	"s_bfm_b64 exec, 12, 0\n\t" \
	"ds_write_b64 v64, v[122:123]\n\t" \
	"s_bfm_b64 exec, %[len], 19\n\t" \
	"ds_write_b64 %[vczm], v[120:121]\n\t" \
	"v_pk_mul_f32 v[124:125], v[120:121], v[120:121]\n\t" \
	"s_nop 0\n\t" \
	"v_add_f32_e32 %[nrm], v125, v124\n\t" \
	"s_mov_b64 exec, -1\n\t" \
	"s_waitcnt lgkmcnt(0)\n\t" \
	"s_branch .Lnb_corr_end\n\t" \
	".Lnb_corrr_mul:\n\t" \
	"s_bfm_b64 exec, %[len], 19\n\t" \
	"ds_read_b64 v[88:89], %[vdm] offset:0\n\t" \
	"ds_read_b64 v[90:91], %[vdm] offset:8\n\t" \
	"ds_read_b64 v[92:93], %[vdm] offset:16\n\t" \
	"ds_read_b64 v[94:95], %[vdm] offset:24\n\t" \
	"ds_read_b64 v[96:97], %[vdm] offset:32\n\t" \
	"ds_read_b64 v[98:99], %[vdm] offset:40\n\t" \
	"ds_read_b64 v[100:101], %[vdm] offset:48\n\t" \
	"ds_read_b64 v[102:103], %[vdm] offset:56\n\t" \
	"ds_read_b64 v[104:105], %[vdm] offset:64\n\t" \
	"ds_read_b64 v[106:107], %[vdm] offset:72\n\t" \
	"ds_read_b64 v[108:109], %[vdm] offset:80\n\t" \
	"ds_read_b64 v[110:111], %[vdm] offset:88\n\t" \
	"ds_read_b64 v[112:113], %[vdm] offset:96\n\t" \
	"ds_read_b64 v[114:115], %[vdm] offset:104\n\t" \
	"ds_read_b64 v[116:117], %[vdm] offset:112\n\t" \
	"ds_read_b64 v[118:119], %[vdm] offset:120\n\t" \
	"s_lshl_b32 s90, %[tsc], 7\n\t" \
	"v_mov_b32_e32 v64, s90\n\t" \
	"ds_read_b128 v[66:69], v64 offset:32848\n\t" \
	"ds_read_b128 v[70:73], v64 offset:32864\n\t" \
	"ds_read_b128 v[74:77], v64 offset:32880\n\t" \
	"ds_read_b128 v[78:81], v64 offset:32896\n\t" \
	"s_waitcnt lgkmcnt(0)\n\t" \
	"v_pk_mul_f32 v[82:83], v[88:89], v[66:67] op_sel:[0,0] op_sel_hi:[0,1]\n\t" \
	"v_pk_mul_f32 v[84:85], v[88:89], v[66:67] op_sel:[1,1] op_sel_hi:[1,0]\n\t" \
	"s_nop 0\n\t" \
	"v_pk_add_f32 v[86:87], v[82:83], v[84:85] neg_lo:[0,1] neg_hi:[0,0]\n\t" \
	"s_nop 0\n\t" \
	"v_pk_add_f32 v[120:121], v[120:121], v[86:87]\n\t" \
	"v_pk_mul_f32 v[82:83], v[90:91], v[68:69] op_sel:[0,0] op_sel_hi:[0,1]\n\t" \
	"v_pk_mul_f32 v[84:85], v[90:91], v[68:69] op_sel:[1,1] op_sel_hi:[1,0]\n\t" \
	"s_nop 0\n\t" \
	"v_pk_add_f32 v[86:87], v[82:83], v[84:85] neg_lo:[0,1] neg_hi:[0,0]\n\t" \
	"s_nop 0\n\t" \
	"v_pk_add_f32 v[120:121], v[120:121], v[86:87]\n\t" \
	"v_pk_mul_f32 v[82:83], v[92:93], v[70:71] op_sel:[0,0] op_sel_hi:[0,1]\n\t" \
	"v_pk_mul_f32 v[84:85], v[92:93], v[70:71] op_sel:[1,1] op_sel_hi:[1,0]\n\t" \
	"s_nop 0\n\t" \
	"v_pk_add_f32 v[86:87], v[82:83], v[84:85] neg_lo:[0,1] neg_hi:[0,0]\n\t" \
	"s_nop 0\n\t" \
	"v_pk_add_f32 v[120:121], v[120:121], v[86:87]\n\t" \
	"v_pk_mul_f32 v[82:83], v[94:95], v[72:73] op_sel:[0,0] op_sel_hi:[0,1]\n\t" \
	"v_pk_mul_f32 v[84:85], v[94:95], v[72:73] op_sel:[1,1] op_sel_hi:[1,0]\n\t" \
	"s_nop 0\n\t" \
	"v_pk_add_f32 v[86:87], v[82:83], v[84:85] neg_lo:[0,1] neg_hi:[0,0]\n\t" \
	"s_nop 0\n\t" \
	"v_pk_add_f32 v[120:121], v[120:121], v[86:87]\n\t" \
	"v_pk_mul_f32 v[82:83], v[96:97], v[74:75] op_sel:[0,0] op_sel_hi:[0,1]\n\t" \
	"v_pk_mul_f32 v[84:85], v[96:97], v[74:75] op_sel:[1,1] op_sel_hi:[1,0]\n\t" \
	"s_nop 0\n\t" \
	"v_pk_add_f32 v[86:87], v[82:83], v[84:85] neg_lo:[0,1] neg_hi:[0,0]\n\t" \
	"s_nop 0\n\t" \
	"v_pk_add_f32 v[120:121], v[120:121], v[86:87]\n\t" \
	"v_pk_mul_f32 v[82:83], v[98:99], v[76:77] op_sel:[0,0] op_sel_hi:[0,1]\n\t" \
	"v_pk_mul_f32 v[84:85], v[98:99], v[76:77] op_sel:[1,1] op_sel_hi:[1,0]\n\t" \
	"s_nop 0\n\t" \
	"v_pk_add_f32 v[86:87], v[82:83], v[84:85] neg_lo:[0,1] neg_hi:[0,0]\n\t" \
	"s_nop 0\n\t" \
	"v_pk_add_f32 v[120:121], v[120:121], v[86:87]\n\t" \
	"v_pk_mul_f32 v[82:83], v[100:101], v[78:79] op_sel:[0,0] op_sel_hi:[0,1]\n\t" \
	"v_pk_mul_f32 v[84:85], v[100:101], v[78:79] op_sel:[1,1] op_sel_hi:[1,0]\n\t" \
	"s_nop 0\n\t" \
	"v_pk_add_f32 v[86:87], v[82:83], v[84:85] neg_lo:[0,1] neg_hi:[0,0]\n\t" \
	"s_nop 0\n\t" \
	"v_pk_add_f32 v[120:121], v[120:121], v[86:87]\n\t" \
	"v_pk_mul_f32 v[82:83], v[102:103], v[80:81] op_sel:[0,0] op_sel_hi:[0,1]\n\t" \
	"v_pk_mul_f32 v[84:85], v[102:103], v[80:81] op_sel:[1,1] op_sel_hi:[1,0]\n\t" \
	"s_nop 0\n\t" \
	"v_pk_add_f32 v[86:87], v[82:83], v[84:85] neg_lo:[0,1] neg_hi:[0,0]\n\t" \
	"s_nop 0\n\t" \
	"v_pk_add_f32 v[120:121], v[120:121], v[86:87]\n\t" \
	"ds_read_b128 v[66:69], v64 offset:32912\n\t" \
	"ds_read_b128 v[70:73], v64 offset:32928\n\t" \
	"ds_read_b128 v[74:77], v64 offset:32944\n\t" \
	"ds_read_b128 v[78:81], v64 offset:32960\n\t" \
	"s_waitcnt lgkmcnt(0)\n\t" \
	"v_pk_mul_f32 v[82:83], v[104:105], v[66:67] op_sel:[0,0] op_sel_hi:[0,1]\n\t" \
	"v_pk_mul_f32 v[84:85], v[104:105], v[66:67] op_sel:[1,1] op_sel_hi:[1,0]\n\t" \
	"s_nop 0\n\t" \
	"v_pk_add_f32 v[86:87], v[82:83], v[84:85] neg_lo:[0,1] neg_hi:[0,0]\n\t" \
	"s_nop 0\n\t" \
	"v_pk_add_f32 v[120:121], v[120:121], v[86:87]\n\t" \
	"v_pk_mul_f32 v[82:83], v[106:107], v[68:69] op_sel:[0,0] op_sel_hi:[0,1]\n\t" \
	"v_pk_mul_f32 v[84:85], v[106:107], v[68:69] op_sel:[1,1] op_sel_hi:[1,0]\n\t" \
	"s_nop 0\n\t" \
	"v_pk_add_f32 v[86:87], v[82:83], v[84:85] neg_lo:[0,1] neg_hi:[0,0]\n\t" \
	"s_nop 0\n\t" \
	"v_pk_add_f32 v[120:121], v[120:121], v[86:87]\n\t" \
	"v_pk_mul_f32 v[82:83], v[108:109], v[70:71] op_sel:[0,0] op_sel_hi:[0,1]\n\t" \
	"v_pk_mul_f32 v[84:85], v[108:109], v[70:71] op_sel:[1,1] op_sel_hi:[1,0]\n\t" \
	"s_nop 0\n\t" \
	"v_pk_add_f32 v[86:87], v[82:83], v[84:85] neg_lo:[0,1] neg_hi:[0,0]\n\t" \
	"s_nop 0\n\t" \
	"v_pk_add_f32 v[120:121], v[120:121], v[86:87]\n\t" \
	"v_pk_mul_f32 v[82:83], v[110:111], v[72:73] op_sel:[0,0] op_sel_hi:[0,1]\n\t" \
	"v_pk_mul_f32 v[84:85], v[110:111], v[72:73] op_sel:[1,1] op_sel_hi:[1,0]\n\t" \
	"s_nop 0\n\t" \
	"v_pk_add_f32 v[86:87], v[82:83], v[84:85] neg_lo:[0,1] neg_hi:[0,0]\n\t" \
	"s_nop 0\n\t" \
	"v_pk_add_f32 v[120:121], v[120:121], v[86:87]\n\t" \
	"v_pk_mul_f32 v[82:83], v[112:113], v[74:75] op_sel:[0,0] op_sel_hi:[0,1]\n\t" \
	"v_pk_mul_f32 v[84:85], v[112:113], v[74:75] op_sel:[1,1] op_sel_hi:[1,0]\n\t" \
	"s_nop 0\n\t" \
	"v_pk_add_f32 v[86:87], v[82:83], v[84:85] neg_lo:[0,1] neg_hi:[0,0]\n\t" \
	"s_nop 0\n\t" \
	"v_pk_add_f32 v[120:121], v[120:121], v[86:87]\n\t" \
	"v_pk_mul_f32 v[82:83], v[114:115], v[76:77] op_sel:[0,0] op_sel_hi:[0,1]\n\t" \
	"v_pk_mul_f32 v[84:85], v[114:115], v[76:77] op_sel:[1,1] op_sel_hi:[1,0]\n\t" \
	"s_nop 0\n\t" \
	"v_pk_add_f32 v[86:87], v[82:83], v[84:85] neg_lo:[0,1] neg_hi:[0,0]\n\t" \
	"s_nop 0\n\t" \
	"v_pk_add_f32 v[120:121], v[120:121], v[86:87]\n\t" \
	"v_pk_mul_f32 v[82:83], v[116:117], v[78:79] op_sel:[0,0] op_sel_hi:[0,1]\n\t" \
	"v_pk_mul_f32 v[84:85], v[116:117], v[78:79] op_sel:[1,1] op_sel_hi:[1,0]\n\t" \
	"s_nop 0\n\t" \
	"v_pk_add_f32 v[86:87], v[82:83], v[84:85] neg_lo:[0,1] neg_hi:[0,0]\n\t" \
	"s_nop 0\n\t" \
	"v_pk_add_f32 v[120:121], v[120:121], v[86:87]\n\t" \
	"v_pk_mul_f32 v[82:83], v[118:119], v[80:81] op_sel:[0,0] op_sel_hi:[0,1]\n\t" \
	"v_pk_mul_f32 v[84:85], v[118:119], v[80:81] op_sel:[1,1] op_sel_hi:[1,0]\n\t" \
	"s_nop 0\n\t" \
	"v_pk_add_f32 v[86:87], v[82:83], v[84:85] neg_lo:[0,1] neg_hi:[0,0]\n\t" \
	"s_nop 0\n\t" \
	"v_pk_add_f32 v[120:121], v[120:121], v[86:87]\n\t" \
	"s_branch .Lnb_corrr_join\n\t" \
	".Lnb_corr_wide:\n\t" \
	"v_mov_b64_e32 v[120:121], 0\n\t" \
	"s_bfm_b64 exec, %[len], 0\n\t" \
	"ds_read_b64 v[88:89], %[vd] offset:0\n\t" \
	"ds_read_b64 v[90:91], %[vd] offset:8\n\t" \
	"ds_read_b64 v[92:93], %[vd] offset:16\n\t" \
	"ds_read_b64 v[94:95], %[vd] offset:24\n\t" \
	"ds_read_b64 v[96:97], %[vd] offset:32\n\t" \
	"ds_read_b64 v[98:99], %[vd] offset:40\n\t" \
	"ds_read_b64 v[100:101], %[vd] offset:48\n\t" \
	"ds_read_b64 v[102:103], %[vd] offset:56\n\t" \
	"ds_read_b64 v[104:105], %[vd] offset:64\n\t" \
	"ds_read_b64 v[106:107], %[vd] offset:72\n\t" \
	"ds_read_b64 v[108:109], %[vd] offset:80\n\t" \
	"ds_read_b64 v[110:111], %[vd] offset:88\n\t" \
	"ds_read_b64 v[112:113], %[vd] offset:96\n\t" \
	"ds_read_b64 v[114:115], %[vd] offset:104\n\t" \
	"ds_read_b64 v[116:117], %[vd] offset:112\n\t" \
	"ds_read_b64 v[118:119], %[vd] offset:120\n\t" \
	"s_cmp_lg_u64 %[bad], 0\n\t" \
	"s_cbranch_scc1 .Lnb_corrw_mul\n\t" \
	"s_getpc_b64 s[88:89]\n\t" \
	".Lnb_corrw_pc:\n\t" \
	"s_mul_i32 s90, %[tsc], .Lnb_corrw_v1-.Lnb_corrw_v0\n\t" \
	"s_add_u32 s88, s88, s90\n\t" \
	"s_addc_u32 s89, s89, 0\n\t" \
	"s_add_u32 s88, s88, .Lnb_corrw_v0-.Lnb_corrw_pc\n\t" \
	"s_addc_u32 s89, s89, 0\n\t" \
	"s_setpc_b64 s[88:89]\n\t" \
	".Lnb_corrw_v0:\n\t" \
	"s_waitcnt lgkmcnt(15)\n\t" \
	"v_pk_add_f32 v[120:121], v[120:121], v[88:89] neg_lo:[0,1] neg_hi:[0,1]\n\t" \
	"s_waitcnt lgkmcnt(14)\n\t" \
	"v_pk_add_f32 v[120:121], v[120:121], v[90:91] op_sel:[0,1] op_sel_hi:[1,0] neg_lo:[0,0] neg_hi:[0,1]\n\t" \
	"s_waitcnt lgkmcnt(13)\n\t" \
	"v_pk_add_f32 v[120:121], v[120:121], v[92:93]\n\t" \
	"s_waitcnt lgkmcnt(12)\n\t" \
	"v_pk_add_f32 v[120:121], v[120:121], v[94:95] op_sel:[0,1] op_sel_hi:[1,0] neg_lo:[0,0] neg_hi:[0,1]\n\t" \
	"s_waitcnt lgkmcnt(11)\n\t" \
	"v_pk_add_f32 v[120:121], v[120:121], v[96:97] neg_lo:[0,1] neg_hi:[0,1]\n\t" \
	"s_waitcnt lgkmcnt(10)\n\t" \
	"v_pk_add_f32 v[120:121], v[120:121], v[98:99] op_sel:[0,1] op_sel_hi:[1,0] neg_lo:[0,0] neg_hi:[0,1]\n\t" \
	"s_waitcnt lgkmcnt(9)\n\t" \
	"v_pk_add_f32 v[120:121], v[120:121], v[100:101] neg_lo:[0,1] neg_hi:[0,1]\n\t" \
	"s_waitcnt lgkmcnt(8)\n\t" \
	"v_pk_add_f32 v[120:121], v[120:121], v[102:103] op_sel:[0,1] op_sel_hi:[1,0] neg_lo:[0,1] neg_hi:[0,0]\n\t" \
	"s_waitcnt lgkmcnt(7)\n\t" \
	"v_pk_add_f32 v[120:121], v[120:121], v[104:105]\n\t" \
	"s_waitcnt lgkmcnt(6)\n\t" \
	"v_pk_add_f32 v[120:121], v[120:121], v[106:107] op_sel:[0,1] op_sel_hi:[1,0] neg_lo:[0,1] neg_hi:[0,0]\n\t" \
	"s_waitcnt lgkmcnt(5)\n\t" \
	"v_pk_add_f32 v[120:121], v[120:121], v[108:109] neg_lo:[0,1] neg_hi:[0,1]\n\t" \
	"s_waitcnt lgkmcnt(4)\n\t" \
	"v_pk_add_f32 v[120:121], v[120:121], v[110:111] op_sel:[0,1] op_sel_hi:[1,0] neg_lo:[0,1] neg_hi:[0,0]\n\t" \
	"s_waitcnt lgkmcnt(3)\n\t" \
	"v_pk_add_f32 v[120:121], v[120:121], v[112:113]\n\t" \
	"s_waitcnt lgkmcnt(2)\n\t" \
	"v_pk_add_f32 v[120:121], v[120:121], v[114:115] op_sel:[0,1] op_sel_hi:[1,0] neg_lo:[0,1] neg_hi:[0,0]\n\t" \
	"s_waitcnt lgkmcnt(1)\n\t" \
	"v_pk_add_f32 v[120:121], v[120:121], v[116:117] neg_lo:[0,1] neg_hi:[0,1]\n\t" \
	"s_waitcnt lgkmcnt(0)\n\t" \
	"v_pk_add_f32 v[120:121], v[120:121], v[118:119] op_sel:[0,1] op_sel_hi:[1,0] neg_lo:[0,1] neg_hi:[0,0]\n\t" \
	"s_branch .Lnb_corrw_join\n\t" \
	".Lnb_corrw_v1:\n\t" \
	"s_waitcnt lgkmcnt(15)\n\t" \
	"v_pk_add_f32 v[120:121], v[120:121], v[88:89] neg_lo:[0,1] neg_hi:[0,1]\n\t" \
	"s_waitcnt lgkmcnt(14)\n\t" \
	"v_pk_add_f32 v[120:121], v[120:121], v[90:91] op_sel:[0,1] op_sel_hi:[1,0] neg_lo:[0,0] neg_hi:[0,1]\n\t" \
	"s_waitcnt lgkmcnt(13)\n\t" \
	"v_pk_add_f32 v[120:121], v[120:121], v[92:93]\n\t" \
	"s_waitcnt lgkmcnt(12)\n\t" \
	"v_pk_add_f32 v[120:121], v[120:121], v[94:95] op_sel:[0,1] op_sel_hi:[1,0] neg_lo:[0,0] neg_hi:[0,1]\n\t" \
	"s_waitcnt lgkmcnt(11)\n\t" \
	"v_pk_add_f32 v[120:121], v[120:121], v[96:97] neg_lo:[0,1] neg_hi:[0,1]\n\t" \
	"s_waitcnt lgkmcnt(10)\n\t" \
	"v_pk_add_f32 v[120:121], v[120:121], v[98:99] op_sel:[0,1] op_sel_hi:[1,0] neg_lo:[0,0] neg_hi:[0,1]\n\t" \
	"s_waitcnt lgkmcnt(9)\n\t" \
	"v_pk_add_f32 v[120:121], v[120:121], v[100:101]\n\t" \
	"s_waitcnt lgkmcnt(8)\n\t" \
	"v_pk_add_f32 v[120:121], v[120:121], v[102:103] op_sel:[0,1] op_sel_hi:[1,0] neg_lo:[0,0] neg_hi:[0,1]\n\t" \
	"s_waitcnt lgkmcnt(7)\n\t" \
	"v_pk_add_f32 v[120:121], v[120:121], v[104:105] neg_lo:[0,1] neg_hi:[0,1]\n\t" \
	"s_waitcnt lgkmcnt(6)\n\t" \
	"v_pk_add_f32 v[120:121], v[120:121], v[106:107] op_sel:[0,1] op_sel_hi:[1,0] neg_lo:[0,1] neg_hi:[0,0]\n\t" \
	"s_waitcnt lgkmcnt(5)\n\t" \
	"v_pk_add_f32 v[120:121], v[120:121], v[108:109] neg_lo:[0,1] neg_hi:[0,1]\n\t" \
	"s_waitcnt lgkmcnt(4)\n\t" \
	"v_pk_add_f32 v[120:121], v[120:121], v[110:111] op_sel:[0,1] op_sel_hi:[1,0] neg_lo:[0,1] neg_hi:[0,0]\n\t" \
	"s_waitcnt lgkmcnt(3)\n\t" \
	"v_pk_add_f32 v[120:121], v[120:121], v[112:113]\n\t" \
	"s_waitcnt lgkmcnt(2)\n\t" \
	"v_pk_add_f32 v[120:121], v[120:121], v[114:115] op_sel:[0,1] op_sel_hi:[1,0] neg_lo:[0,1] neg_hi:[0,0]\n\t" \
	"s_waitcnt lgkmcnt(1)\n\t" \
	"v_pk_add_f32 v[120:121], v[120:121], v[116:117] neg_lo:[0,1] neg_hi:[0,1]\n\t" \
	"s_waitcnt lgkmcnt(0)\n\t" \
	"v_pk_add_f32 v[120:121], v[120:121], v[118:119] op_sel:[0,1] op_sel_hi:[1,0] neg_lo:[0,0] neg_hi:[0,1]\n\t" \
	"s_branch .Lnb_corrw_join\n\t" \
	".Lnb_corrw_v2:\n\t" \
	"s_waitcnt lgkmcnt(15)\n\t" \
	"v_pk_add_f32 v[120:121], v[120:121], v[88:89]\n\t" \
	"s_waitcnt lgkmcnt(14)\n\t" \
	"v_pk_add_f32 v[120:121], v[120:121], v[90:91] op_sel:[0,1] op_sel_hi:[1,0] neg_lo:[0,1] neg_hi:[0,0]\n\t" \
	"s_waitcnt lgkmcnt(13)\n\t" \
	"v_pk_add_f32 v[120:121], v[120:121], v[92:93]\n\t" \
	"s_waitcnt lgkmcnt(12)\n\t" \
	"v_pk_add_f32 v[120:121], v[120:121], v[94:95] op_sel:[0,1] op_sel_hi:[1,0] neg_lo:[0,0] neg_hi:[0,1]\n\t" \
	"s_waitcnt lgkmcnt(11)\n\t" \
	"v_pk_add_f32 v[120:121], v[120:121], v[96:97]\n\t" \
	"s_waitcnt lgkmcnt(10)\n\t" \
	"v_pk_add_f32 v[120:121], v[120:121], v[98:99] op_sel:[0,1] op_sel_hi:[1,0] neg_lo:[0,1] neg_hi:[0,0]\n\t" \
	"s_waitcnt lgkmcnt(9)\n\t" \
	"v_pk_add_f32 v[120:121], v[120:121], v[100:101]\n\t" \
	"s_waitcnt lgkmcnt(8)\n\t" \
	"v_pk_add_f32 v[120:121], v[120:121], v[102:103] op_sel:[0,1] op_sel_hi:[1,0] neg_lo:[0,0] neg_hi:[0,1]\n\t" \
	"s_waitcnt lgkmcnt(7)\n\t" \
	"v_pk_add_f32 v[120:121], v[120:121], v[104:105]\n\t" \
	"s_waitcnt lgkmcnt(6)\n\t" \
	"v_pk_add_f32 v[120:121], v[120:121], v[106:107] op_sel:[0,1] op_sel_hi:[1,0] neg_lo:[0,1] neg_hi:[0,0]\n\t" \
	"s_waitcnt lgkmcnt(5)\n\t" \
	"v_pk_add_f32 v[120:121], v[120:121], v[108:109] neg_lo:[0,1] neg_hi:[0,1]\n\t" \
	"s_waitcnt lgkmcnt(4)\n\t" \
	"v_pk_add_f32 v[120:121], v[120:121], v[110:111] op_sel:[0,1] op_sel_hi:[1,0] neg_lo:[0,1] neg_hi:[0,0]\n\t" \
	"s_waitcnt lgkmcnt(3)\n\t" \
	"v_pk_add_f32 v[120:121], v[120:121], v[112:113] neg_lo:[0,1] neg_hi:[0,1]\n\t" \
	"s_waitcnt lgkmcnt(2)\n\t" \
	"v_pk_add_f32 v[120:121], v[120:121], v[114:115] op_sel:[0,1] op_sel_hi:[1,0] neg_lo:[0,0] neg_hi:[0,1]\n\t" \
	"s_waitcnt lgkmcnt(1)\n\t" \
	"v_pk_add_f32 v[120:121], v[120:121], v[116:117] neg_lo:[0,1] neg_hi:[0,1]\n\t" \
	"s_waitcnt lgkmcnt(0)\n\t" \
	"v_pk_add_f32 v[120:121], v[120:121], v[118:119] op_sel:[0,1] op_sel_hi:[1,0] neg_lo:[0,1] neg_hi:[0,0]\n\t" \
	"s_branch .Lnb_corrw_join\n\t" \
	".Lnb_corrw_v3:\n\t" \
	"s_waitcnt lgkmcnt(15)\n\t" \
	"v_pk_add_f32 v[120:121], v[120:121], v[88:89] neg_lo:[0,1] neg_hi:[0,1]\n\t" \
	"s_waitcnt lgkmcnt(14)\n\t" \
	"v_pk_add_f32 v[120:121], v[120:121], v[90:91] op_sel:[0,1] op_sel_hi:[1,0] neg_lo:[0,1] neg_hi:[0,0]\n\t" \
	"s_waitcnt lgkmcnt(13)\n\t" \
	"v_pk_add_f32 v[120:121], v[120:121], v[92:93]\n\t" \
	"s_waitcnt lgkmcnt(12)\n\t" \
	"v_pk_add_f32 v[120:121], v[120:121], v[94:95] op_sel:[0,1] op_sel_hi:[1,0] neg_lo:[0,0] neg_hi:[0,1]\n\t" \
	"s_waitcnt lgkmcnt(11)\n\t" \
	"v_pk_add_f32 v[120:121], v[120:121], v[96:97]\n\t" \
	"s_waitcnt lgkmcnt(10)\n\t" \
	"v_pk_add_f32 v[120:121], v[120:121], v[98:99] op_sel:[0,1] op_sel_hi:[1,0] neg_lo:[0,1] neg_hi:[0,0]\n\t" \
	"s_waitcnt lgkmcnt(9)\n\t" \
	"v_pk_add_f32 v[120:121], v[120:121], v[100:101]\n\t" \
	"s_waitcnt lgkmcnt(8)\n\t" \
	"v_pk_add_f32 v[120:121], v[120:121], v[102:103] op_sel:[0,1] op_sel_hi:[1,0] neg_lo:[0,1] neg_hi:[0,0]\n\t" \
	"s_waitcnt lgkmcnt(7)\n\t" \
	"v_pk_add_f32 v[120:121], v[120:121], v[104:105] neg_lo:[0,1] neg_hi:[0,1]\n\t" \
	"s_waitcnt lgkmcnt(6)\n\t" \
	"v_pk_add_f32 v[120:121], v[120:121], v[106:107] op_sel:[0,1] op_sel_hi:[1,0] neg_lo:[0,0] neg_hi:[0,1]\n\t" \
	"s_waitcnt lgkmcnt(5)\n\t" \
	"v_pk_add_f32 v[120:121], v[120:121], v[108:109] neg_lo:[0,1] neg_hi:[0,1]\n\t" \
	"s_waitcnt lgkmcnt(4)\n\t" \
	"v_pk_add_f32 v[120:121], v[120:121], v[110:111] op_sel:[0,1] op_sel_hi:[1,0] neg_lo:[0,1] neg_hi:[0,0]\n\t" \
	"s_waitcnt lgkmcnt(3)\n\t" \
	"v_pk_add_f32 v[120:121], v[120:121], v[112:113] neg_lo:[0,1] neg_hi:[0,1]\n\t" \
	"s_waitcnt lgkmcnt(2)\n\t" \
	"v_pk_add_f32 v[120:121], v[120:121], v[114:115] op_sel:[0,1] op_sel_hi:[1,0] neg_lo:[0,0] neg_hi:[0,1]\n\t" \
	"s_waitcnt lgkmcnt(1)\n\t" \
	"v_pk_add_f32 v[120:121], v[120:121], v[116:117] neg_lo:[0,1] neg_hi:[0,1]\n\t" \
	"s_waitcnt lgkmcnt(0)\n\t" \
	"v_pk_add_f32 v[120:121], v[120:121], v[118:119] op_sel:[0,1] op_sel_hi:[1,0] neg_lo:[0,1] neg_hi:[0,0]\n\t" \
	"s_branch .Lnb_corrw_join\n\t" \
	".Lnb_corrw_v4:\n\t" \
	"s_waitcnt lgkmcnt(15)\n\t" \
	"v_pk_add_f32 v[120:121], v[120:121], v[88:89]\n\t" \
	"s_waitcnt lgkmcnt(14)\n\t" \
	"v_pk_add_f32 v[120:121], v[120:121], v[90:91] op_sel:[0,1] op_sel_hi:[1,0] neg_lo:[0,1] neg_hi:[0,0]\n\t" \
	"s_waitcnt lgkmcnt(13)\n\t" \
	"v_pk_add_f32 v[120:121], v[120:121], v[92:93] neg_lo:[0,1] neg_hi:[0,1]\n\t" \
	"s_waitcnt lgkmcnt(12)\n\t" \
	"v_pk_add_f32 v[120:121], v[120:121], v[94:95] op_sel:[0,1] op_sel_hi:[1,0] neg_lo:[0,0] neg_hi:[0,1]\n\t" \
	"s_waitcnt lgkmcnt(11)\n\t" \
	"v_pk_add_f32 v[120:121], v[120:121], v[96:97] neg_lo:[0,1] neg_hi:[0,1]\n\t" \
	"s_waitcnt lgkmcnt(10)\n\t" \
	"v_pk_add_f32 v[120:121], v[120:121], v[98:99] op_sel:[0,1] op_sel_hi:[1,0] neg_lo:[0,1] neg_hi:[0,0]\n\t" \
	"s_waitcnt lgkmcnt(9)\n\t" \
	"v_pk_add_f32 v[120:121], v[120:121], v[100:101] neg_lo:[0,1] neg_hi:[0,1]\n\t" \
	"s_waitcnt lgkmcnt(8)\n\t" \
	"v_pk_add_f32 v[120:121], v[120:121], v[102:103] op_sel:[0,1] op_sel_hi:[1,0] neg_lo:[0,1] neg_hi:[0,0]\n\t" \
	"s_waitcnt lgkmcnt(7)\n\t" \
	"v_pk_add_f32 v[120:121], v[120:121], v[104:105] neg_lo:[0,1] neg_hi:[0,1]\n\t" \
	"s_waitcnt lgkmcnt(6)\n\t" \
	"v_pk_add_f32 v[120:121], v[120:121], v[106:107] op_sel:[0,1] op_sel_hi:[1,0] neg_lo:[0,0] neg_hi:[0,1]\n\t" \
	"s_waitcnt lgkmcnt(5)\n\t" \
	"v_pk_add_f32 v[120:121], v[120:121], v[108:109] neg_lo:[0,1] neg_hi:[0,1]\n\t" \
	"s_waitcnt lgkmcnt(4)\n\t" \
	"v_pk_add_f32 v[120:121], v[120:121], v[110:111] op_sel:[0,1] op_sel_hi:[1,0] neg_lo:[0,1] neg_hi:[0,0]\n\t" \
	"s_waitcnt lgkmcnt(3)\n\t" \
	"v_pk_add_f32 v[120:121], v[120:121], v[112:113]\n\t" \
	"s_waitcnt lgkmcnt(2)\n\t" \
	"v_pk_add_f32 v[120:121], v[120:121], v[114:115] op_sel:[0,1] op_sel_hi:[1,0] neg_lo:[0,0] neg_hi:[0,1]\n\t" \
	"s_waitcnt lgkmcnt(1)\n\t" \
	"v_pk_add_f32 v[120:121], v[120:121], v[116:117]\n\t" \
	"s_waitcnt lgkmcnt(0)\n\t" \
	"v_pk_add_f32 v[120:121], v[120:121], v[118:119] op_sel:[0,1] op_sel_hi:[1,0] neg_lo:[0,0] neg_hi:[0,1]\n\t" \
	"s_branch .Lnb_corrw_join\n\t" \
	".Lnb_corrw_v5:\n\t" \
	"s_waitcnt lgkmcnt(15)\n\t" \
	"v_pk_add_f32 v[120:121], v[120:121], v[88:89] neg_lo:[0,1] neg_hi:[0,1]\n\t" \
	"s_waitcnt lgkmcnt(14)\n\t" \
	"v_pk_add_f32 v[120:121], v[120:121], v[90:91] op_sel:[0,1] op_sel_hi:[1,0] neg_lo:[0,1] neg_hi:[0,0]\n\t" \
	"s_waitcnt lgkmcnt(13)\n\t" \
	"v_pk_add_f32 v[120:121], v[120:121], v[92:93] neg_lo:[0,1] neg_hi:[0,1]\n\t" \
	"s_waitcnt lgkmcnt(12)\n\t" \
	"v_pk_add_f32 v[120:121], v[120:121], v[94:95] op_sel:[0,1] op_sel_hi:[1,0] neg_lo:[0,0] neg_hi:[0,1]\n\t" \
	"s_waitcnt lgkmcnt(11)\n\t" \
	"v_pk_add_f32 v[120:121], v[120:121], v[96:97]\n\t" \
	"s_waitcnt lgkmcnt(10)\n\t" \
	"v_pk_add_f32 v[120:121], v[120:121], v[98:99] op_sel:[0,1] op_sel_hi:[1,0] neg_lo:[0,1] neg_hi:[0,0]\n\t" \
	"s_waitcnt lgkmcnt(9)\n\t" \
	"v_pk_add_f32 v[120:121], v[120:121], v[100:101]\n\t" \
	"s_waitcnt lgkmcnt(8)\n\t" \
	"v_pk_add_f32 v[120:121], v[120:121], v[102:103] op_sel:[0,1] op_sel_hi:[1,0] neg_lo:[0,1] neg_hi:[0,0]\n\t" \
	"s_waitcnt lgkmcnt(7)\n\t" \
	"v_pk_add_f32 v[120:121], v[120:121], v[104:105]\n\t" \
	"s_waitcnt lgkmcnt(6)\n\t" \
	"v_pk_add_f32 v[120:121], v[120:121], v[106:107] op_sel:[0,1] op_sel_hi:[1,0] neg_lo:[0,0] neg_hi:[0,1]\n\t" \
	"s_waitcnt lgkmcnt(5)\n\t" \
	"v_pk_add_f32 v[120:121], v[120:121], v[108:109] neg_lo:[0,1] neg_hi:[0,1]\n\t" \
	"s_waitcnt lgkmcnt(4)\n\t" \
	"v_pk_add_f32 v[120:121], v[120:121], v[110:111] op_sel:[0,1] op_sel_hi:[1,0] neg_lo:[0,1] neg_hi:[0,0]\n\t" \
	"s_waitcnt lgkmcnt(3)\n\t" \
	"v_pk_add_f32 v[120:121], v[120:121], v[112:113] neg_lo:[0,1] neg_hi:[0,1]\n\t" \
	"s_waitcnt lgkmcnt(2)\n\t" \
	"v_pk_add_f32 v[120:121], v[120:121], v[114:115] op_sel:[0,1] op_sel_hi:[1,0] neg_lo:[0,0] neg_hi:[0,1]\n\t" \
	"s_waitcnt lgkmcnt(1)\n\t" \
	"v_pk_add_f32 v[120:121], v[120:121], v[116:117] neg_lo:[0,1] neg_hi:[0,1]\n\t" \
	"s_waitcnt lgkmcnt(0)\n\t" \
	"v_pk_add_f32 v[120:121], v[120:121], v[118:119] op_sel:[0,1] op_sel_hi:[1,0] neg_lo:[0,0] neg_hi:[0,1]\n\t" \
	"s_branch .Lnb_corrw_join\n\t" \
	".Lnb_corrw_v6:\n\t" \
	"s_waitcnt lgkmcnt(15)\n\t" \
	"v_pk_add_f32 v[120:121], v[120:121], v[88:89] neg_lo:[0,1] neg_hi:[0,1]\n\t" \
	"s_waitcnt lgkmcnt(14)\n\t" \
	"v_pk_add_f32 v[120:121], v[120:121], v[90:91] op_sel:[0,1] op_sel_hi:[1,0] neg_lo:[0,1] neg_hi:[0,0]\n\t" \
	"s_waitcnt lgkmcnt(13)\n\t" \
	"v_pk_add_f32 v[120:121], v[120:121], v[92:93]\n\t" \
	"s_waitcnt lgkmcnt(12)\n\t" \
	"v_pk_add_f32 v[120:121], v[120:121], v[94:95] op_sel:[0,1] op_sel_hi:[1,0] neg_lo:[0,0] neg_hi:[0,1]\n\t" \
	"s_waitcnt lgkmcnt(11)\n\t" \
	"v_pk_add_f32 v[120:121], v[120:121], v[96:97] neg_lo:[0,1] neg_hi:[0,1]\n\t" \
	"s_waitcnt lgkmcnt(10)\n\t" \
	"v_pk_add_f32 v[120:121], v[120:121], v[98:99] op_sel:[0,1] op_sel_hi:[1,0] neg_lo:[0,0] neg_hi:[0,1]\n\t" \
	"s_waitcnt lgkmcnt(9)\n\t" \
	"v_pk_add_f32 v[120:121], v[120:121], v[100:101]\n\t" \
	"s_waitcnt lgkmcnt(8)\n\t" \
	"v_pk_add_f32 v[120:121], v[120:121], v[102:103] op_sel:[0,1] op_sel_hi:[1,0] neg_lo:[0,0] neg_hi:[0,1]\n\t" \
	"s_waitcnt lgkmcnt(7)\n\t" \
	"v_pk_add_f32 v[120:121], v[120:121], v[104:105]\n\t" \
	"s_waitcnt lgkmcnt(6)\n\t" \
	"v_pk_add_f32 v[120:121], v[120:121], v[106:107] op_sel:[0,1] op_sel_hi:[1,0] neg_lo:[0,0] neg_hi:[0,1]\n\t" \
	"s_waitcnt lgkmcnt(5)\n\t" \
	"v_pk_add_f32 v[120:121], v[120:121], v[108:109] neg_lo:[0,1] neg_hi:[0,1]\n\t" \
	"s_waitcnt lgkmcnt(4)\n\t" \
	"v_pk_add_f32 v[120:121], v[120:121], v[110:111] op_sel:[0,1] op_sel_hi:[1,0] neg_lo:[0,0] neg_hi:[0,1]\n\t" \
	"s_waitcnt lgkmcnt(3)\n\t" \
	"v_pk_add_f32 v[120:121], v[120:121], v[112:113]\n\t" \
	"s_waitcnt lgkmcnt(2)\n\t" \
	"v_pk_add_f32 v[120:121], v[120:121], v[114:115] op_sel:[0,1] op_sel_hi:[1,0] neg_lo:[0,1] neg_hi:[0,0]\n\t" \
	"s_waitcnt lgkmcnt(1)\n\t" \
	"v_pk_add_f32 v[120:121], v[120:121], v[116:117] neg_lo:[0,1] neg_hi:[0,1]\n\t" \
	"s_waitcnt lgkmcnt(0)\n\t" \
	"v_pk_add_f32 v[120:121], v[120:121], v[118:119] op_sel:[0,1] op_sel_hi:[1,0] neg_lo:[0,1] neg_hi:[0,0]\n\t" \
	"s_branch .Lnb_corrw_join\n\t" \
	".Lnb_corrw_v7:\n\t" \
	"s_waitcnt lgkmcnt(15)\n\t" \
	"v_pk_add_f32 v[120:121], v[120:121], v[88:89] neg_lo:[0,1] neg_hi:[0,1]\n\t" \
	"s_waitcnt lgkmcnt(14)\n\t" \
	"v_pk_add_f32 v[120:121], v[120:121], v[90:91] op_sel:[0,1] op_sel_hi:[1,0] neg_lo:[0,1] neg_hi:[0,0]\n\t" \
	"s_waitcnt lgkmcnt(13)\n\t" \
	"v_pk_add_f32 v[120:121], v[120:121], v[92:93]\n\t" \
	"s_waitcnt lgkmcnt(12)\n\t" \
	"v_pk_add_f32 v[120:121], v[120:121], v[94:95] op_sel:[0,1] op_sel_hi:[1,0] neg_lo:[0,1] neg_hi:[0,0]\n\t" \
	"s_waitcnt lgkmcnt(11)\n\t" \
	"v_pk_add_f32 v[120:121], v[120:121], v[96:97]\n\t" \
	"s_waitcnt lgkmcnt(10)\n\t" \
	"v_pk_add_f32 v[120:121], v[120:121], v[98:99] op_sel:[0,1] op_sel_hi:[1,0] neg_lo:[0,0] neg_hi:[0,1]\n\t" \
	"s_waitcnt lgkmcnt(9)\n\t" \
	"v_pk_add_f32 v[120:121], v[120:121], v[100:101]\n\t" \
	"s_waitcnt lgkmcnt(8)\n\t" \
	"v_pk_add_f32 v[120:121], v[120:121], v[102:103] op_sel:[0,1] op_sel_hi:[1,0] neg_lo:[0,1] neg_hi:[0,0]\n\t" \
	"s_waitcnt lgkmcnt(7)\n\t" \
	"v_pk_add_f32 v[120:121], v[120:121], v[104:105]\n\t" \
	"s_waitcnt lgkmcnt(6)\n\t" \
	"v_pk_add_f32 v[120:121], v[120:121], v[106:107] op_sel:[0,1] op_sel_hi:[1,0] neg_lo:[0,1] neg_hi:[0,0]\n\t" \
	"s_waitcnt lgkmcnt(5)\n\t" \
	"v_pk_add_f32 v[120:121], v[120:121], v[108:109] neg_lo:[0,1] neg_hi:[0,1]\n\t" \
	"s_waitcnt lgkmcnt(4)\n\t" \
	"v_pk_add_f32 v[120:121], v[120:121], v[110:111] op_sel:[0,1] op_sel_hi:[1,0] neg_lo:[0,0] neg_hi:[0,1]\n\t" \
	"s_waitcnt lgkmcnt(3)\n\t" \
	"v_pk_add_f32 v[120:121], v[120:121], v[112:113] neg_lo:[0,1] neg_hi:[0,1]\n\t" \
	"s_waitcnt lgkmcnt(2)\n\t" \
	"v_pk_add_f32 v[120:121], v[120:121], v[114:115] op_sel:[0,1] op_sel_hi:[1,0] neg_lo:[0,1] neg_hi:[0,0]\n\t" \
	"s_waitcnt lgkmcnt(1)\n\t" \
	"v_pk_add_f32 v[120:121], v[120:121], v[116:117] neg_lo:[0,1] neg_hi:[0,1]\n\t" \
	"s_waitcnt lgkmcnt(0)\n\t" \
	"v_pk_add_f32 v[120:121], v[120:121], v[118:119] op_sel:[0,1] op_sel_hi:[1,0] neg_lo:[0,0] neg_hi:[0,1]\n\t" \
	"s_branch .Lnb_corrw_join\n\t" \
	".Lnb_corrw_join:\n\t" \
	"s_add_u32 s90, %[len], 12\n\t" \
	"s_bfm_b64 exec, s90, 0\n\t" \
// ... 823 lines not shown
```

Measured before the change: 1069.

## Interleave raw-sample conversion into DEC/CORR asm to fill LDS latency and DPP nops

Only rows 3..7 of the raw int16 IQ samples are converted and stored to LDS before the decimator. Rows 0..4 and rows 8..9 are now converted inside the DEC and CORR inline-asm blocks, placed in the LDS-read wait gaps and in place of the s_nop slots between dependent DPP ops. DEC and CORR also move ahead of the next-burst prefetch, and the claim-behind count shrinks to match the new number of head LDS writes. This hides conversion ALU work behind latency the wave already spends waiting, but it couples the layout assumptions tightly to the generated asm, with a risk of ordering errors in LDS writes and waitcnts.

```diff
diff --git a/osmo_trx_amd/csrc/trx_kernel_nb.hip b/osmo_trx_amd/csrc/trx_kernel_nb.hip
--- a/osmo_trx_amd/csrc/trx_kernel_nb.hip
+++ b/osmo_trx_amd/csrc/trx_kernel_nb.hip
@@ -38,6 +38,8 @@
 	static_assert(NB_ASM_GDEC_OFF == (TRX_SINCV_LDS + 16 * WAVE + NB_COMP_ROWS * 36) * 4, "tools/gen_nb_asm.py: LDS offset of the decimator taps");
 	static_assert(NB_ASM_DEC_MAX_NACT == 15 + NB_ASM_CORR_MAX_LEN, "tools/gen_nb_asm.py: DEC and CORR change form at the same window");
 	static_assert(NB_ASM_LSEQ_OFF == (NB_TABLES_FLOATS - 2 * 8 * 16) * 4, "tools/gen_nb_asm.py: LDS offset of the training-sequence taps");
+	static_assert(NB_ASM_HEAD_ROW0 == 3 && NB_ASM_HEAD_ROW1 == 7, "tools/gen_nb_asm.py: DEC's operands p0..p4 and CORR's p8, p9 are the rows the head leaves");
+	static_assert(64 * NB_ASM_HEAD_ROW0 <= 4 * 52 + 1 && 4 * (52 + 63 + 4) + 3 < 64 * (NB_ASM_HEAD_ROW1 + 1), "the head converts every raw sample DEC reads");
 	constexpr int NLD = 10;
 	extern __shared__ __attribute__((aligned(16))) char smem[];
 	const int lane0 = threadIdx.x & (WAVE - 1);
@@ -326,22 +328,16 @@
 		asm volatile("s_waitcnt vmcnt(0)" ::: "memory");
 		DIAG_MARK(13);
 #endif
-		if (!leave) {
 #pragma unroll
-			for (int r = 0; r < NLD; r++) {
-				const int i = r * WAVE + lane;
-				if (r < NLD - 1 || i < 625) {
-					const c32 v = make_float2((float)(int16_t)(pre_i[r] & 0xffffu), (float)(int16_t)(pre_i[r] >> 16));
-					pload[16 * r] = v;
-					asm("v_max3_f32 %0, %0, |%1|, |%2|" : "+v"(amax) : "v"(v.x), "v"(v.y));
-					if (r < 5)
-						epart = fmaf(v.x, v.x, fmaf(v.y, v.y, epart));
-				}
+		for (int r = 0; r < NLD; r++)
+			asm volatile("" :: "v"(pre_i[r]));
+		if (__builtin_expect(!leave, 1)) {
+#pragma unroll
+			for (int r = NB_ASM_HEAD_ROW0; r <= NB_ASM_HEAD_ROW1; r++) {
+				const c32 v = make_float2((float)(int16_t)(pre_i[r] & 0xffffu), (float)(int16_t)(pre_i[r] >> 16));
+				pload[16 * r] = v;
+				asm("v_max3_f32 %0, %0, |%1|, |%2|" : "+v"(amax) : "v"(v.x), "v"(v.y));
 			}
-		} else {
-#pragma unroll
-			for (int r = 0; r < NLD; r++)
-				asm volatile("" :: "v"(pre_i[r]));
 		}
 		DIAG_MARK(14);
 		if (pend_any) {
@@ -363,11 +359,33 @@
 		}
 		pend_any = false;
 		DIAG_MARK(16);
-		j_next = (unsigned)(leave ? claim_take(ticket) : claim_take_behind<5>(ticket));
+		j_next = (unsigned)(leave ? claim_take(ticket) : claim_take_behind<NB_ASM_HEAD_LDS_WRITES>(ticket));
 		b_next = burst_of(j_next);
 		if (pooled && (j_next & 15u) == 0u && j_next + 16u >= items)
 			pool_draw(j_next, b_next == NB_NO_BURST && j_next >= items, lane);
 		DIAG_MARK(17);
+
+		unsigned long long bad = 0ull;
+		float dr = 0.0f, di = 0.0f, nrm = 0.0f;
+		const int len = 16 + (int)max_toa;
+		const unsigned vd_addr = lds_addr(D) + 8u * (unsigned)lane, vcz_addr = lds_addr(cz) + 8u * (unsigned)lane;
+		if (!leave) {
+			__builtin_assume(len >= 16 && len <= 16 + NB_MAX_TOA);
+			asm volatile(NB_ASM_DEC
+				     : [bad] "=s"(bad), [dr] "=&v"(dr), [di] "=&v"(di), [amax] "+v"(amax), [ep] "+v"(epart)
+				     : [pl] "v"(lds_addr(pload)), [p0] "v"(pre_i[0]), [p1] "v"(pre_i[1]), [p2] "v"(pre_i[2]), [p3] "v"(pre_i[3]), [p4] "v"(pre_i[4]),
+				       [pd] "v"(lds_addr(P + PH_M0 + 52) + 8u * (unsigned)lane), [vd] "v"(vd_addr), [vd4] "v"(vd_addr - 32u), [zero] "v"(0),
+				       [nact] "s"(15 + len)
+				     : NB_ASM_CLOBBERS);
+			DIAG_MARK(2);
+			asm volatile(NB_ASM_CORR
+				     : [nrm] "=&v"(nrm), [amax] "+v"(amax)
+				     : [pl] "v"(lds_addr(pload)), [p8] "v"(pre_i[NLD - 2]), [p9] "v"(pre_i[NLD - 1]),
+				       [vd] "v"(vd_addr), [vcz] "v"(vcz_addr), [vdm] "v"(vd_addr - 8u * NB_ASM_CORR_LANE0),
+				       [vczm] "v"(vcz_addr - 8u * NB_ASM_CORR_LANE0), [dr] "v"(dr), [di] "v"(di), [len] "s"(len), [tsc] "s"(tsc), [bad] "s"(bad)
+				     : NB_ASM_CLOBBERS);
+			DIAG_MARK(3);
+		}
 		if (b_next != NB_NO_BURST)
 			prefetch(b_next, lane);
 		DIAG_MARK(15);
@@ -375,27 +393,9 @@
 		int clip = 0;
 		if (!leave) {
 			clip = __ballot(amax > TRX_CLIP_THRESH) != 0ull;
-
-			const int len = 16 + (int)max_toa;
-			__builtin_assume(len >= 16 && len <= 16 + NB_MAX_TOA);
-			const unsigned vd_addr = lds_addr(D) + 8u * (unsigned)lane, vcz_addr = lds_addr(cz) + 8u * (unsigned)lane;
-			unsigned long long bad;
-			float dr, di;
-			asm volatile(NB_ASM_DEC
-				     : [bad] "=s"(bad), [dr] "=&v"(dr), [di] "=&v"(di)
-				     : [pd] "v"(lds_addr(P + PH_M0 + 52) + 8u * (unsigned)lane), [vd] "v"(vd_addr), [vd4] "v"(vd_addr - 32u), [zero] "v"(0),
-				       [nact] "s"(15 + len)
-				     : NB_ASM_CLOBBERS);
-			DIAG_MARK(2);
 			{
-				float v;
+				const float v = nrm;
 				const int lag0 = (len <= NB_ASM_CORR_MAX_LEN) ? NB_ASM_CORR_LANE0 : 0;
-				asm volatile(NB_ASM_CORR
-					     : [nrm] "=&v"(v)
-					     : [vd] "v"(vd_addr), [vcz] "v"(vcz_addr), [vdm] "v"(vd_addr - 8u * NB_ASM_CORR_LANE0),
-					       [vczm] "v"(vcz_addr - 8u * NB_ASM_CORR_LANE0), [dr] "v"(dr), [di] "v"(di), [len] "s"(len), [tsc] "s"(tsc), [bad] "s"(bad)
-					     : NB_ASM_CLOBBERS);
-				DIAG_MARK(3);
 				int m_bits, es_bits, bidx;
 				int kr, ka, kb, kic, ktp;
 				asm volatile(NB_ASM_AMAX("ds_read_b32 %[kr], %[l4] offset:%c[lc]", "ds_read_b32 %[ka], %[l4] offset:%c[lc]+256",
diff --git a/osmo_trx_amd/csrc/trx_nb_asm.inc b/osmo_trx_amd/csrc/trx_nb_asm.inc
--- a/osmo_trx_amd/csrc/trx_nb_asm.inc
+++ b/osmo_trx_amd/csrc/trx_nb_asm.inc
@@ -3,6 +3,9 @@
 #define NB_ASM_DEC_MAX_NACT 60
 #define NB_ASM_CORR_LANE0 19
 #define NB_ASM_CORR_MAX_LEN 45
+#define NB_ASM_HEAD_ROW0 3
+#define NB_ASM_HEAD_ROW1 7
+#define NB_ASM_HEAD_LDS_WRITES 3
 #define NB_ASM_CLOBBERS "v64", "v65", "v66", "v67", "v68", "v69", "v70", "v71", "v72", "v73", "v74", "v75", "v76", "v77", "v78", "v79", "v80", "v81", "v82", "v83", "v84", "v85", "v86", "v87", "v88", "v89", "v90", "v91", "v92", "v93", "v94", "v95", "v96", "v97", "v98", "v99", "v100", "v101", "v102", "v103", "v104", "v105", "v106", "v107", "v108", "v109", "v110", "v111", "v112", "v113", "v114", "v115", "v116", "v117", "v118", "v119", "v120", "v121", "v122", "v123", "v124", "v125", "v126", "v127", "s87", "s88", "s89", "s90", "s91", "s92", "s93", "s94", "s95", "s96", "s97", "s98", "s99", "vcc", "scc", "memory"
 #define NB_ASM_DEC \
 	"s_cmp_gt_u32 %[nact], 60\n\t" \
@@ -15,14 +18,41 @@
 	"ds_read_b64 v[100:101], %[pd] offset:2880\n\t" \
 	"ds_read_b64 v[102:103], %[pd] offset:4320\n\t" \
 	"ds_read_b64 v[96:97], %[pd] offset:0\n\t" \
+	"s_mov_b64 exec, -1\n\t" \
+	"v_cvt_f32_i32_sdwa v109, sext(%[p0]) dst_sel:DWORD dst_unused:UNUSED_PAD src0_sel:WORD_1\n\t" \
+	"v_cvt_f32_i32_sdwa v108, sext(%[p0]) dst_sel:DWORD dst_unused:UNUSED_PAD src0_sel:WORD_0\n\t" \
+	"v_cvt_f32_i32_sdwa v111, sext(%[p1]) dst_sel:DWORD dst_unused:UNUSED_PAD src0_sel:WORD_1\n\t" \
+	"v_cvt_f32_i32_sdwa v110, sext(%[p1]) dst_sel:DWORD dst_unused:UNUSED_PAD src0_sel:WORD_0\n\t" \
+	"v_cvt_f32_i32_sdwa v113, sext(%[p2]) dst_sel:DWORD dst_unused:UNUSED_PAD src0_sel:WORD_1\n\t" \
+	"v_cvt_f32_i32_sdwa v112, sext(%[p2]) dst_sel:DWORD dst_unused:UNUSED_PAD src0_sel:WORD_0\n\t" \
+	"v_cvt_f32_i32_sdwa v115, sext(%[p3]) dst_sel:DWORD dst_unused:UNUSED_PAD src0_sel:WORD_1\n\t" \
+	"v_cvt_f32_i32_sdwa v114, sext(%[p3]) dst_sel:DWORD dst_unused:UNUSED_PAD src0_sel:WORD_0\n\t" \
+	"v_cvt_f32_i32_sdwa v117, sext(%[p4]) dst_sel:DWORD dst_unused:UNUSED_PAD src0_sel:WORD_1\n\t" \
+	"v_cvt_f32_i32_sdwa v116, sext(%[p4]) dst_sel:DWORD dst_unused:UNUSED_PAD src0_sel:WORD_0\n\t" \
+	"v_max3_f32 %[amax], %[amax], |v108|, |v109|\n\t" \
+	"v_max3_f32 %[amax], %[amax], |v110|, |v111|\n\t" \
+	"v_max3_f32 %[amax], %[amax], |v112|, |v113|\n\t" \
+	"v_fmac_f32_e32 %[ep], v109, v109\n\t" \
+	"v_fmac_f32_e32 %[ep], v108, v108\n\t" \
+	"v_fmac_f32_e32 %[ep], v111, v111\n\t" \
+	"v_fmac_f32_e32 %[ep], v110, v110\n\t" \
+	"v_fmac_f32_e32 %[ep], v113, v113\n\t" \
+	"v_fmac_f32_e32 %[ep], v112, v112\n\t" \
+	"v_fmac_f32_e32 %[ep], v115, v115\n\t" \
+	"v_fmac_f32_e32 %[ep], v114, v114\n\t" \
+	"v_fmac_f32_e32 %[ep], v117, v117\n\t" \
+	"v_fmac_f32_e32 %[ep], v116, v116\n\t" \
+	"ds_write2_b64 %[pl], v[108:109], v[110:111] offset0:0 offset1:16\n\t" \
+	"ds_write_b64 %[pl], v[112:113] offset:256\n\t" \
+	"s_lshr_b64 exec, -1, s88\n\t" \
+	"s_waitcnt lgkmcnt(5)\n\t" \
+	"v_pk_mul_f32 v[64:65], v[98:99], v[120:121] op_sel:[0,0] op_sel_hi:[1,0]\n\t" \
+	"s_waitcnt lgkmcnt(4)\n\t" \
+	"v_pk_mul_f32 v[66:67], v[100:101], v[120:121] op_sel:[0,1] op_sel_hi:[1,1]\n\t" \
 	"s_waitcnt lgkmcnt(3)\n\t" \
-	"v_pk_mul_f32 v[64:65], v[98:99], v[120:121] op_sel:[0,0] op_sel_hi:[1,0]\n\t" \
-	"s_waitcnt lgkmcnt(2)\n\t" \
-	"v_pk_mul_f32 v[66:67], v[100:101], v[120:121] op_sel:[0,1] op_sel_hi:[1,1]\n\t" \
-	"s_waitcnt lgkmcnt(1)\n\t" \
 	"v_pk_mul_f32 v[68:69], v[102:103], v[122:123] op_sel:[0,0] op_sel_hi:[1,0]\n\t" \
 	"v_pk_add_f32 v[104:105], v[64:65], v[66:67]\n\t" \
-	"s_waitcnt lgkmcnt(0)\n\t" \
+	"s_waitcnt lgkmcnt(2)\n\t" \
 	"v_pk_mul_f32 v[70:71], v[96:97], v[122:123] op_sel:[0,1] op_sel_hi:[1,1]\n\t" \
 	"v_pk_add_f32 v[104:105], v[104:105], v[68:69]\n\t" \
 	"v_pk_mul_f32 v[72:73], v[98:99], v[124:125] op_sel:[0,0] op_sel_hi:[1,0]\n\t" \
@@ -68,6 +98,31 @@
 	"s_waitcnt lgkmcnt(0)\n\t" \
 	"s_branch .Lnb_dec_end\n\t" \
 	".Lnb_dec_wide:\n\t" \
+	"v_cvt_f32_i32_sdwa v65, sext(%[p0]) dst_sel:DWORD dst_unused:UNUSED_PAD src0_sel:WORD_1\n\t" \
+	"v_cvt_f32_i32_sdwa v64, sext(%[p0]) dst_sel:DWORD dst_unused:UNUSED_PAD src0_sel:WORD_0\n\t" \
+	"v_cvt_f32_i32_sdwa v67, sext(%[p1]) dst_sel:DWORD dst_unused:UNUSED_PAD src0_sel:WORD_1\n\t" \
+	"v_cvt_f32_i32_sdwa v66, sext(%[p1]) dst_sel:DWORD dst_unused:UNUSED_PAD src0_sel:WORD_0\n\t" \
+	"v_cvt_f32_i32_sdwa v69, sext(%[p2]) dst_sel:DWORD dst_unused:UNUSED_PAD src0_sel:WORD_1\n\t" \
+	"v_cvt_f32_i32_sdwa v68, sext(%[p2]) dst_sel:DWORD dst_unused:UNUSED_PAD src0_sel:WORD_0\n\t" \
+	"v_cvt_f32_i32_sdwa v71, sext(%[p3]) dst_sel:DWORD dst_unused:UNUSED_PAD src0_sel:WORD_1\n\t" \
+	"v_cvt_f32_i32_sdwa v70, sext(%[p3]) dst_sel:DWORD dst_unused:UNUSED_PAD src0_sel:WORD_0\n\t" \
+	"v_cvt_f32_i32_sdwa v73, sext(%[p4]) dst_sel:DWORD dst_unused:UNUSED_PAD src0_sel:WORD_1\n\t" \
+	"v_cvt_f32_i32_sdwa v72, sext(%[p4]) dst_sel:DWORD dst_unused:UNUSED_PAD src0_sel:WORD_0\n\t" \
+	"v_max3_f32 %[amax], %[amax], |v64|, |v65|\n\t" \
+	"v_max3_f32 %[amax], %[amax], |v66|, |v67|\n\t" \
+	"v_max3_f32 %[amax], %[amax], |v68|, |v69|\n\t" \
+	"v_fmac_f32_e32 %[ep], v65, v65\n\t" \
+	"v_fmac_f32_e32 %[ep], v64, v64\n\t" \
+	"v_fmac_f32_e32 %[ep], v67, v67\n\t" \
+	"v_fmac_f32_e32 %[ep], v66, v66\n\t" \
+	"v_fmac_f32_e32 %[ep], v69, v69\n\t" \
+	"v_fmac_f32_e32 %[ep], v68, v68\n\t" \
+	"v_fmac_f32_e32 %[ep], v71, v71\n\t" \
+	"v_fmac_f32_e32 %[ep], v70, v70\n\t" \
+	"v_fmac_f32_e32 %[ep], v73, v73\n\t" \
+	"v_fmac_f32_e32 %[ep], v72, v72\n\t" \
+	"ds_write2_b64 %[pl], v[64:65], v[66:67] offset0:0 offset1:16\n\t" \
+	"ds_write_b64 %[pl], v[68:69] offset:256\n\t" \
 	"s_bfm_b64 exec, %[nact], 0\n\t" \
 	"ds_read_b128 v[120:123], %[zero] offset:29968\n\t" \
 	"ds_read_b128 v[124:127], %[zero] offset:29984\n\t" \
@@ -139,9 +194,7 @@
 	"v_mov_b64_e32 v[122:123], 0\n\t" \
 	"v_mov_b32_e32 %[nrm], 0\n\t" \
 	"s_lshl_b32 s90, %[len], 3\n\t" \
-	"s_sub_u32 s91, 45, %[len]\n\t" \
 	"v_add_u32_e32 v64, s90, %[vcz]\n\t" \
-	"s_lshr_b64 exec, -1, s91\n\t" \
 	"s_cmp_lg_u64 %[bad], 0\n\t" \
 	"s_cbranch_scc1 .Lnb_corrr_mul\n\t" \
 	"s_getpc_b64 s[88:89]\n\t" \
@@ -155,28 +208,30 @@
 	".Lnb_corrr_v0:\n\t" \
 	"v_sub_f32_e32 v120, 0, %[dr]\n\t" \
 	"v_sub_f32_e32 v121, 0, %[di]\n\t" \
-	"s_nop 0\n\t" \
-	"v_add_f32_dpp v120, v120, %[di] wave_shr:1 row_mask:0xf bank_mask:0xf bound_ctrl:0\n\t" \
-	"v_sub_f32_dpp v121, v121, %[dr] wave_shr:1 row_mask:0xf bank_mask:0xf bound_ctrl:0\n\t" \
-	"s_nop 0\n\t" \
-	"v_add_f32_dpp v120, v120, %[dr] wave_shr:1 row_mask:0xf bank_mask:0xf bound_ctrl:0\n\t" \
-	"v_add_f32_dpp v121, v121, %[di] wave_shr:1 row_mask:0xf bank_mask:0xf bound_ctrl:0\n\t" \
-	"s_nop 0\n\t" \
-	"v_add_f32_dpp v120, v120, %[di] wave_shr:1 row_mask:0xf bank_mask:0xf bound_ctrl:0\n\t" \
-	"v_sub_f32_dpp v121, v121, %[dr] wave_shr:1 row_mask:0xf bank_mask:0xf bound_ctrl:0\n\t" \
-	"s_nop 0\n\t" \
-	"v_sub_f32_dpp v120, v120, %[dr] wave_shr:1 row_mask:0xf bank_mask:0xf bound_ctrl:0\n\t" \
-	"v_sub_f32_dpp v121, v121, %[di] wave_shr:1 row_mask:0xf bank_mask:0xf bound_ctrl:0\n\t" \
-	"s_nop 0\n\t" \
-	"v_add_f32_dpp v120, v120, %[di] wave_shr:1 row_mask:0xf bank_mask:0xf bound_ctrl:0\n\t" \
-	"v_sub_f32_dpp v121, v121, %[dr] wave_shr:1 row_mask:0xf bank_mask:0xf bound_ctrl:0\n\t" \
-	"s_nop 0\n\t" \
-	"v_sub_f32_dpp v120, v120, %[dr] wave_shr:1 row_mask:0xf bank_mask:0xf bound_ctrl:0\n\t" \
-	"v_sub_f32_dpp v121, v121, %[di] wave_shr:1 row_mask:0xf bank_mask:0xf bound_ctrl:0\n\t" \
-	"s_nop 0\n\t" \
-	"v_sub_f32_dpp v120, v120, %[di] wave_shr:1 row_mask:0xf bank_mask:0xf bound_ctrl:0\n\t" \
-	"v_add_f32_dpp v121, v121, %[dr] wave_shr:1 row_mask:0xf bank_mask:0xf bound_ctrl:0\n\t" \
-	"s_nop 0\n\t" \
+	"v_cvt_f32_i32_sdwa v67, sext(%[p8]) dst_sel:DWORD dst_unused:UNUSED_PAD src0_sel:WORD_1\n\t" \
+	"v_add_f32_dpp v120, v120, %[di] wave_shr:1 row_mask:0xf bank_mask:0xf bound_ctrl:0\n\t" \
+	"v_sub_f32_dpp v121, v121, %[dr] wave_shr:1 row_mask:0xf bank_mask:0xf bound_ctrl:0\n\t" \
+	"v_cvt_f32_i32_sdwa v66, sext(%[p8]) dst_sel:DWORD dst_unused:UNUSED_PAD src0_sel:WORD_0\n\t" \
+	"v_add_f32_dpp v120, v120, %[dr] wave_shr:1 row_mask:0xf bank_mask:0xf bound_ctrl:0\n\t" \
+	"v_add_f32_dpp v121, v121, %[di] wave_shr:1 row_mask:0xf bank_mask:0xf bound_ctrl:0\n\t" \
+	"v_cvt_f32_i32_sdwa v69, sext(%[p9]) dst_sel:DWORD dst_unused:UNUSED_PAD src0_sel:WORD_1\n\t" \
+	"v_add_f32_dpp v120, v120, %[di] wave_shr:1 row_mask:0xf bank_mask:0xf bound_ctrl:0\n\t" \
+	"v_sub_f32_dpp v121, v121, %[dr] wave_shr:1 row_mask:0xf bank_mask:0xf bound_ctrl:0\n\t" \
+	"v_cvt_f32_i32_sdwa v68, sext(%[p9]) dst_sel:DWORD dst_unused:UNUSED_PAD src0_sel:WORD_0\n\t" \
+	"v_sub_f32_dpp v120, v120, %[dr] wave_shr:1 row_mask:0xf bank_mask:0xf bound_ctrl:0\n\t" \
+	"v_sub_f32_dpp v121, v121, %[di] wave_shr:1 row_mask:0xf bank_mask:0xf bound_ctrl:0\n\t" \
+	"v_max3_f32 %[amax], %[amax], |v66|, |v67|\n\t" \
+	"v_add_f32_dpp v120, v120, %[di] wave_shr:1 row_mask:0xf bank_mask:0xf bound_ctrl:0\n\t" \
+	"v_sub_f32_dpp v121, v121, %[dr] wave_shr:1 row_mask:0xf bank_mask:0xf bound_ctrl:0\n\t" \
+	"v_max3_f32 %[amax], %[amax], |v68|, |v69|\n\t" \
+	"v_sub_f32_dpp v120, v120, %[dr] wave_shr:1 row_mask:0xf bank_mask:0xf bound_ctrl:0\n\t" \
+	"v_sub_f32_dpp v121, v121, %[di] wave_shr:1 row_mask:0xf bank_mask:0xf bound_ctrl:0\n\t" \
+	"ds_write_b64 %[pl], v[66:67] offset:1024\n\t" \
+	"v_sub_f32_dpp v120, v120, %[di] wave_shr:1 row_mask:0xf bank_mask:0xf bound_ctrl:0\n\t" \
+	"v_add_f32_dpp v121, v121, %[dr] wave_shr:1 row_mask:0xf bank_mask:0xf bound_ctrl:0\n\t" \
+	"s_bfm_b64 exec, 49, 0\n\t" \
+	"ds_write_b64 %[pl], v[68:69] offset:1152\n\t" \
+	"s_mov_b64 exec, -1\n\t" \
 	"v_add_f32_dpp v120, v120, %[dr] wave_shr:1 row_mask:0xf bank_mask:0xf bound_ctrl:0\n\t" \
 	"v_add_f32_dpp v121, v121, %[di] wave_shr:1 row_mask:0xf bank_mask:0xf bound_ctrl:0\n\t" \
 	"s_nop 0\n\t" \
@@ -204,28 +259,30 @@
 	".Lnb_corrr_v1:\n\t" \
 	"v_sub_f32_e32 v120, 0, %[dr]\n\t" \
 	"v_sub_f32_e32 v121, 0, %[di]\n\t" \
-	"s_nop 0\n\t" \
-	"v_add_f32_dpp v120, v120, %[di] wave_shr:1 row_mask:0xf bank_mask:0xf bound_ctrl:0\n\t" \
-	"v_sub_f32_dpp v121, v121, %[dr] wave_shr:1 row_mask:0xf bank_mask:0xf bound_ctrl:0\n\t" \
-	"s_nop 0\n\t" \
-	"v_add_f32_dpp v120, v120, %[dr] wave_shr:1 row_mask:0xf bank_mask:0xf bound_ctrl:0\n\t" \
-	"v_add_f32_dpp v121, v121, %[di] wave_shr:1 row_mask:0xf bank_mask:0xf bound_ctrl:0\n\t" \
-	"s_nop 0\n\t" \
-	"v_add_f32_dpp v120, v120, %[di] wave_shr:1 row_mask:0xf bank_mask:0xf bound_ctrl:0\n\t" \
-	"v_sub_f32_dpp v121, v121, %[dr] wave_shr:1 row_mask:0xf bank_mask:0xf bound_ctrl:0\n\t" \
-	"s_nop 0\n\t" \
-	"v_sub_f32_dpp v120, v120, %[dr] wave_shr:1 row_mask:0xf bank_mask:0xf bound_ctrl:0\n\t" \
-	"v_sub_f32_dpp v121, v121, %[di] wave_shr:1 row_mask:0xf bank_mask:0xf bound_ctrl:0\n\t" \
-	"s_nop 0\n\t" \
-	"v_add_f32_dpp v120, v120, %[di] wave_shr:1 row_mask:0xf bank_mask:0xf bound_ctrl:0\n\t" \
-	"v_sub_f32_dpp v121, v121, %[dr] wave_shr:1 row_mask:0xf bank_mask:0xf bound_ctrl:0\n\t" \
-	"s_nop 0\n\t" \
-	"v_add_f32_dpp v120, v120, %[dr] wave_shr:1 row_mask:0xf bank_mask:0xf bound_ctrl:0\n\t" \
-	"v_add_f32_dpp v121, v121, %[di] wave_shr:1 row_mask:0xf bank_mask:0xf bound_ctrl:0\n\t" \
-	"s_nop 0\n\t" \
-	"v_add_f32_dpp v120, v120, %[di] wave_shr:1 row_mask:0xf bank_mask:0xf bound_ctrl:0\n\t" \
-	"v_sub_f32_dpp v121, v121, %[dr] wave_shr:1 row_mask:0xf bank_mask:0xf bound_ctrl:0\n\t" \
-	"s_nop 0\n\t" \
+	"v_cvt_f32_i32_sdwa v67, sext(%[p8]) dst_sel:DWORD dst_unused:UNUSED_PAD src0_sel:WORD_1\n\t" \
+	"v_add_f32_dpp v120, v120, %[di] wave_shr:1 row_mask:0xf bank_mask:0xf bound_ctrl:0\n\t" \
+	"v_sub_f32_dpp v121, v121, %[dr] wave_shr:1 row_mask:0xf bank_mask:0xf bound_ctrl:0\n\t" \
+	"v_cvt_f32_i32_sdwa v66, sext(%[p8]) dst_sel:DWORD dst_unused:UNUSED_PAD src0_sel:WORD_0\n\t" \
+	"v_add_f32_dpp v120, v120, %[dr] wave_shr:1 row_mask:0xf bank_mask:0xf bound_ctrl:0\n\t" \
+	"v_add_f32_dpp v121, v121, %[di] wave_shr:1 row_mask:0xf bank_mask:0xf bound_ctrl:0\n\t" \
+	"v_cvt_f32_i32_sdwa v69, sext(%[p9]) dst_sel:DWORD dst_unused:UNUSED_PAD src0_sel:WORD_1\n\t" \
+	"v_add_f32_dpp v120, v120, %[di] wave_shr:1 row_mask:0xf bank_mask:0xf bound_ctrl:0\n\t" \
+	"v_sub_f32_dpp v121, v121, %[dr] wave_shr:1 row_mask:0xf bank_mask:0xf bound_ctrl:0\n\t" \
+	"v_cvt_f32_i32_sdwa v68, sext(%[p9]) dst_sel:DWORD dst_unused:UNUSED_PAD src0_sel:WORD_0\n\t" \
+	"v_sub_f32_dpp v120, v120, %[dr] wave_shr:1 row_mask:0xf bank_mask:0xf bound_ctrl:0\n\t" \
+	"v_sub_f32_dpp v121, v121, %[di] wave_shr:1 row_mask:0xf bank_mask:0xf bound_ctrl:0\n\t" \
+	"v_max3_f32 %[amax], %[amax], |v66|, |v67|\n\t" \
+	"v_add_f32_dpp v120, v120, %[di] wave_shr:1 row_mask:0xf bank_mask:0xf bound_ctrl:0\n\t" \
+	"v_sub_f32_dpp v121, v121, %[dr] wave_shr:1 row_mask:0xf bank_mask:0xf bound_ctrl:0\n\t" \
+	"v_max3_f32 %[amax], %[amax], |v68|, |v69|\n\t" \
+	"v_add_f32_dpp v120, v120, %[dr] wave_shr:1 row_mask:0xf bank_mask:0xf bound_ctrl:0\n\t" \
+	"v_add_f32_dpp v121, v121, %[di] wave_shr:1 row_mask:0xf bank_mask:0xf bound_ctrl:0\n\t" \
+	"ds_write_b64 %[pl], v[66:67] offset:1024\n\t" \
+	"v_add_f32_dpp v120, v120, %[di] wave_shr:1 row_mask:0xf bank_mask:0xf bound_ctrl:0\n\t" \
+	"v_sub_f32_dpp v121, v121, %[dr] wave_shr:1 row_mask:0xf bank_mask:0xf bound_ctrl:0\n\t" \
+	"s_bfm_b64 exec, 49, 0\n\t" \
+	"ds_write_b64 %[pl], v[68:69] offset:1152\n\t" \
+	"s_mov_b64 exec, -1\n\t" \
 	"v_sub_f32_dpp v120, v120, %[dr] wave_shr:1 row_mask:0xf bank_mask:0xf bound_ctrl:0\n\t" \
 	"v_sub_f32_dpp v121, v121, %[di] wave_shr:1 row_mask:0xf bank_mask:0xf bound_ctrl:0\n\t" \
 	"s_nop 0\n\t" \
@@ -253,28 +310,30 @@
 	".Lnb_corrr_v2:\n\t" \
 	"v_add_f32_e32 v120, 0, %[dr]\n\t" \
 	"v_add_f32_e32 v121, 0, %[di]\n\t" \
-	"s_nop 0\n\t" \
-	"v_sub_f32_dpp v120, v120, %[di] wave_shr:1 row_mask:0xf bank_mask:0xf bound_ctrl:0\n\t" \
-	"v_add_f32_dpp v121, v121, %[dr] wave_shr:1 row_mask:0xf bank_mask:0xf bound_ctrl:0\n\t" \
-	"s_nop 0\n\t" \
-	"v_add_f32_dpp v120, v120, %[dr] wave_shr:1 row_mask:0xf bank_mask:0xf bound_ctrl:0\n\t" \
-	"v_add_f32_dpp v121, v121, %[di] wave_shr:1 row_mask:0xf bank_mask:0xf bound_ctrl:0\n\t" \
-	"s_nop 0\n\t" \
-	"v_add_f32_dpp v120, v120, %[di] wave_shr:1 row_mask:0xf bank_mask:0xf bound_ctrl:0\n\t" \
-	"v_sub_f32_dpp v121, v121, %[dr] wave_shr:1 row_mask:0xf bank_mask:0xf bound_ctrl:0\n\t" \
-	"s_nop 0\n\t" \
-	"v_add_f32_dpp v120, v120, %[dr] wave_shr:1 row_mask:0xf bank_mask:0xf bound_ctrl:0\n\t" \
-	"v_add_f32_dpp v121, v121, %[di] wave_shr:1 row_mask:0xf bank_mask:0xf bound_ctrl:0\n\t" \
-	"s_nop 0\n\t" \
-	"v_sub_f32_dpp v120, v120, %[di] wave_shr:1 row_mask:0xf bank_mask:0xf bound_ctrl:0\n\t" \
-	"v_add_f32_dpp v121, v121, %[dr] wave_shr:1 row_mask:0xf bank_mask:0xf bound_ctrl:0\n\t" \
-	"s_nop 0\n\t" \
-	"v_add_f32_dpp v120, v120, %[dr] wave_shr:1 row_mask:0xf bank_mask:0xf bound_ctrl:0\n\t" \
-	"v_add_f32_dpp v121, v121, %[di] wave_shr:1 row_mask:0xf bank_mask:0xf bound_ctrl:0\n\t" \
-	"s_nop 0\n\t" \
-	"v_add_f32_dpp v120, v120, %[di] wave_shr:1 row_mask:0xf bank_mask:0xf bound_ctrl:0\n\t" \
-	"v_sub_f32_dpp v121, v121, %[dr] wave_shr:1 row_mask:0xf bank_mask:0xf bound_ctrl:0\n\t" \
-	"s_nop 0\n\t" \
+	"v_cvt_f32_i32_sdwa v67, sext(%[p8]) dst_sel:DWORD dst_unused:UNUSED_PAD src0_sel:WORD_1\n\t" \
+	"v_sub_f32_dpp v120, v120, %[di] wave_shr:1 row_mask:0xf bank_mask:0xf bound_ctrl:0\n\t" \
+	"v_add_f32_dpp v121, v121, %[dr] wave_shr:1 row_mask:0xf bank_mask:0xf bound_ctrl:0\n\t" \
+	"v_cvt_f32_i32_sdwa v66, sext(%[p8]) dst_sel:DWORD dst_unused:UNUSED_PAD src0_sel:WORD_0\n\t" \
+	"v_add_f32_dpp v120, v120, %[dr] wave_shr:1 row_mask:0xf bank_mask:0xf bound_ctrl:0\n\t" \
+	"v_add_f32_dpp v121, v121, %[di] wave_shr:1 row_mask:0xf bank_mask:0xf bound_ctrl:0\n\t" \
+	"v_cvt_f32_i32_sdwa v69, sext(%[p9]) dst_sel:DWORD dst_unused:UNUSED_PAD src0_sel:WORD_1\n\t" \
+	"v_add_f32_dpp v120, v120, %[di] wave_shr:1 row_mask:0xf bank_mask:0xf bound_ctrl:0\n\t" \
+	"v_sub_f32_dpp v121, v121, %[dr] wave_shr:1 row_mask:0xf bank_mask:0xf bound_ctrl:0\n\t" \
+	"v_cvt_f32_i32_sdwa v68, sext(%[p9]) dst_sel:DWORD dst_unused:UNUSED_PAD src0_sel:WORD_0\n\t" \
+	"v_add_f32_dpp v120, v120, %[dr] wave_shr:1 row_mask:0xf bank_mask:0xf bound_ctrl:0\n\t" \
+	"v_add_f32_dpp v121, v121, %[di] wave_shr:1 row_mask:0xf bank_mask:0xf bound_ctrl:0\n\t" \
+	"v_max3_f32 %[amax], %[amax], |v66|, |v67|\n\t" \
+	"v_sub_f32_dpp v120, v120, %[di] wave_shr:1 row_mask:0xf bank_mask:0xf bound_ctrl:0\n\t" \
+	"v_add_f32_dpp v121, v121, %[dr] wave_shr:1 row_mask:0xf bank_mask:0xf bound_ctrl:0\n\t" \
+	"v_max3_f32 %[amax], %[amax], |v68|, |v69|\n\t" \
+	"v_add_f32_dpp v120, v120, %[dr] wave_shr:1 row_mask:0xf bank_mask:0xf bound_ctrl:0\n\t" \
+	"v_add_f32_dpp v121, v121, %[di] wave_shr:1 row_mask:0xf bank_mask:0xf bound_ctrl:0\n\t" \
+	"ds_write_b64 %[pl], v[66:67] offset:1024\n\t" \
+	"v_add_f32_dpp v120, v120, %[di] wave_shr:1 row_mask:0xf bank_mask:0xf bound_ctrl:0\n\t" \
+	"v_sub_f32_dpp v121, v121, %[dr] wave_shr:1 row_mask:0xf bank_mask:0xf bound_ctrl:0\n\t" \
+	"s_bfm_b64 exec, 49, 0\n\t" \
+	"ds_write_b64 %[pl], v[68:69] offset:1152\n\t" \
+	"s_mov_b64 exec, -1\n\t" \
 	"v_add_f32_dpp v120, v120, %[dr] wave_shr:1 row_mask:0xf bank_mask:0xf bound_ctrl:0\n\t" \
 	"v_add_f32_dpp v121, v121, %[di] wave_shr:1 row_mask:0xf bank_mask:0xf bound_ctrl:0\n\t" \
 	"s_nop 0\n\t" \
@@ -302,28 +361,30 @@
 	".Lnb_corrr_v3:\n\t" \
 	"v_sub_f32_e32 v120, 0, %[dr]\n\t" \
 	"v_sub_f32_e32 v121, 0, %[di]\n\t" \
-	"s_nop 0\n\t" \
-	"v_sub_f32_dpp v120, v120, %[di] wave_shr:1 row_mask:0xf bank_mask:0xf bound_ctrl:0\n\t" \
-	"v_add_f32_dpp v121, v121, %[dr] wave_shr:1 row_mask:0xf bank_mask:0xf bound_ctrl:0\n\t" \
-	"s_nop 0\n\t" \
-	"v_add_f32_dpp v120, v120, %[dr] wave_shr:1 row_mask:0xf bank_mask:0xf bound_ctrl:0\n\t" \
-	"v_add_f32_dpp v121, v121, %[di] wave_shr:1 row_mask:0xf bank_mask:0xf bound_ctrl:0\n\t" \
-	"s_nop 0\n\t" \
-	"v_add_f32_dpp v120, v120, %[di] wave_shr:1 row_mask:0xf bank_mask:0xf bound_ctrl:0\n\t" \
-	"v_sub_f32_dpp v121, v121, %[dr] wave_shr:1 row_mask:0xf bank_mask:0xf bound_ctrl:0\n\t" \
-	"s_nop 0\n\t" \
-	"v_add_f32_dpp v120, v120, %[dr] wave_shr:1 row_mask:0xf bank_mask:0xf bound_ctrl:0\n\t" \
-	"v_add_f32_dpp v121, v121, %[di] wave_shr:1 row_mask:0xf bank_mask:0xf bound_ctrl:0\n\t" \
-	"s_nop 0\n\t" \
-	"v_sub_f32_dpp v120, v120, %[di] wave_shr:1 row_mask:0xf bank_mask:0xf bound_ctrl:0\n\t" \
-	"v_add_f32_dpp v121, v121, %[dr] wave_shr:1 row_mask:0xf bank_mask:0xf bound_ctrl:0\n\t" \
-	"s_nop 0\n\t" \
-	"v_add_f32_dpp v120, v120, %[dr] wave_shr:1 row_mask:0xf bank_mask:0xf bound_ctrl:0\n\t" \
-	"v_add_f32_dpp v121, v121, %[di] wave_shr:1 row_mask:0xf bank_mask:0xf bound_ctrl:0\n\t" \
-	"s_nop 0\n\t" \
-	"v_sub_f32_dpp v120, v120, %[di] wave_shr:1 row_mask:0xf bank_mask:0xf bound_ctrl:0\n\t" \
-	"v_add_f32_dpp v121, v121, %[dr] wave_shr:1 row_mask:0xf bank_mask:0xf bound_ctrl:0\n\t" \
-	"s_nop 0\n\t" \
+	"v_cvt_f32_i32_sdwa v67, sext(%[p8]) dst_sel:DWORD dst_unused:UNUSED_PAD src0_sel:WORD_1\n\t" \
+	"v_sub_f32_dpp v120, v120, %[di] wave_shr:1 row_mask:0xf bank_mask:0xf bound_ctrl:0\n\t" \
+	"v_add_f32_dpp v121, v121, %[dr] wave_shr:1 row_mask:0xf bank_mask:0xf bound_ctrl:0\n\t" \
+	"v_cvt_f32_i32_sdwa v66, sext(%[p8]) dst_sel:DWORD dst_unused:UNUSED_PAD src0_sel:WORD_0\n\t" \
+	"v_add_f32_dpp v120, v120, %[dr] wave_shr:1 row_mask:0xf bank_mask:0xf bound_ctrl:0\n\t" \
+	"v_add_f32_dpp v121, v121, %[di] wave_shr:1 row_mask:0xf bank_mask:0xf bound_ctrl:0\n\t" \
+	"v_cvt_f32_i32_sdwa v69, sext(%[p9]) dst_sel:DWORD dst_unused:UNUSED_PAD src0_sel:WORD_1\n\t" \
+	"v_add_f32_dpp v120, v120, %[di] wave_shr:1 row_mask:0xf bank_mask:0xf bound_ctrl:0\n\t" \
+	"v_sub_f32_dpp v121, v121, %[dr] wave_shr:1 row_mask:0xf bank_mask:0xf bound_ctrl:0\n\t" \
+	"v_cvt_f32_i32_sdwa v68, sext(%[p9]) dst_sel:DWORD dst_unused:UNUSED_PAD src0_sel:WORD_0\n\t" \
+	"v_add_f32_dpp v120, v120, %[dr] wave_shr:1 row_mask:0xf bank_mask:0xf bound_ctrl:0\n\t" \
+	"v_add_f32_dpp v121, v121, %[di] wave_shr:1 row_mask:0xf bank_mask:0xf bound_ctrl:0\n\t" \
+	"v_max3_f32 %[amax], %[amax], |v66|, |v67|\n\t" \
+	"v_sub_f32_dpp v120, v120, %[di] wave_shr:1 row_mask:0xf bank_mask:0xf bound_ctrl:0\n\t" \
+	"v_add_f32_dpp v121, v121, %[dr] wave_shr:1 row_mask:0xf bank_mask:0xf bound_ctrl:0\n\t" \
+	"v_max3_f32 %[amax], %[amax], |v68|, |v69|\n\t" \
+	"v_add_f32_dpp v120, v120, %[dr] wave_shr:1 row_mask:0xf bank_mask:0xf bound_ctrl:0\n\t" \
+	"v_add_f32_dpp v121, v121, %[di] wave_shr:1 row_mask:0xf bank_mask:0xf bound_ctrl:0\n\t" \
+	"ds_write_b64 %[pl], v[66:67] offset:1024\n\t" \
+	"v_sub_f32_dpp v120, v120, %[di] wave_shr:1 row_mask:0xf bank_mask:0xf bound_ctrl:0\n\t" \
+	"v_add_f32_dpp v121, v121, %[dr] wave_shr:1 row_mask:0xf bank_mask:0xf bound_ctrl:0\n\t" \
+	"s_bfm_b64 exec, 49, 0\n\t" \
+	"ds_write_b64 %[pl], v[68:69] offset:1152\n\t" \
+	"s_mov_b64 exec, -1\n\t" \
 	"v_sub_f32_dpp v120, v120, %[dr] wave_shr:1 row_mask:0xf bank_mask:0xf bound_ctrl:0\n\t" \
 	"v_sub_f32_dpp v121, v121, %[di] wave_shr:1 row_mask:0xf bank_mask:0xf bound_ctrl:0\n\t" \
 	"s_nop 0\n\t" \
@@ -351,28 +412,30 @@
 	".Lnb_corrr_v4:\n\t" \
 	"v_add_f32_e32 v120, 0, %[dr]\n\t" \
 	"v_add_f32_e32 v121, 0, %[di]\n\t" \
-	"s_nop 0\n\t" \
-	"v_sub_f32_dpp v120, v120, %[di] wave_shr:1 row_mask:0xf bank_mask:0xf bound_ctrl:0\n\t" \
-	"v_add_f32_dpp v121, v121, %[dr] wave_shr:1 row_mask:0xf bank_mask:0xf bound_ctrl:0\n\t" \
-	"s_nop 0\n\t" \
-	"v_sub_f32_dpp v120, v120, %[dr] wave_shr:1 row_mask:0xf bank_mask:0xf bound_ctrl:0\n\t" \
-	"v_sub_f32_dpp v121, v121, %[di] wave_shr:1 row_mask:0xf bank_mask:0xf bound_ctrl:0\n\t" \
-	"s_nop 0\n\t" \
-	"v_add_f32_dpp v120, v120, %[di] wave_shr:1 row_mask:0xf bank_mask:0xf bound_ctrl:0\n\t" \
-	"v_sub_f32_dpp v121, v121, %[dr] wave_shr:1 row_mask:0xf bank_mask:0xf bound_ctrl:0\n\t" \
-	"s_nop 0\n\t" \
-	"v_sub_f32_dpp v120, v120, %[dr] wave_shr:1 row_mask:0xf bank_mask:0xf bound_ctrl:0\n\t" \
-	"v_sub_f32_dpp v121, v121, %[di] wave_shr:1 row_mask:0xf bank_mask:0xf bound_ctrl:0\n\t" \
-	"s_nop 0\n\t" \
-	"v_sub_f32_dpp v120, v120, %[di] wave_shr:1 row_mask:0xf bank_mask:0xf bound_ctrl:0\n\t" \
-	"v_add_f32_dpp v121, v121, %[dr] wave_shr:1 row_mask:0xf bank_mask:0xf bound_ctrl:0\n\t" \
-	"s_nop 0\n\t" \
-	"v_sub_f32_dpp v120, v120, %[dr] wave_shr:1 row_mask:0xf bank_mask:0xf bound_ctrl:0\n\t" \
-	"v_sub_f32_dpp v121, v121, %[di] wave_shr:1 row_mask:0xf bank_mask:0xf bound_ctrl:0\n\t" \
-	"s_nop 0\n\t" \
-	"v_sub_f32_dpp v120, v120, %[di] wave_shr:1 row_mask:0xf bank_mask:0xf bound_ctrl:0\n\t" \
-	"v_add_f32_dpp v121, v121, %[dr] wave_shr:1 row_mask:0xf bank_mask:0xf bound_ctrl:0\n\t" \
-	"s_nop 0\n\t" \
+	"v_cvt_f32_i32_sdwa v67, sext(%[p8]) dst_sel:DWORD dst_unused:UNUSED_PAD src0_sel:WORD_1\n\t" \
+	"v_sub_f32_dpp v120, v120, %[di] wave_shr:1 row_mask:0xf bank_mask:0xf bound_ctrl:0\n\t" \
+	"v_add_f32_dpp v121, v121, %[dr] wave_shr:1 row_mask:0xf bank_mask:0xf bound_ctrl:0\n\t" \
+	"v_cvt_f32_i32_sdwa v66, sext(%[p8]) dst_sel:DWORD dst_unused:UNUSED_PAD src0_sel:WORD_0\n\t" \
+	"v_sub_f32_dpp v120, v120, %[dr] wave_shr:1 row_mask:0xf bank_mask:0xf bound_ctrl:0\n\t" \
+	"v_sub_f32_dpp v121, v121, %[di] wave_shr:1 row_mask:0xf bank_mask:0xf bound_ctrl:0\n\t" \
+	"v_cvt_f32_i32_sdwa v69, sext(%[p9]) dst_sel:DWORD dst_unused:UNUSED_PAD src0_sel:WORD_1\n\t" \
+	"v_add_f32_dpp v120, v120, %[di] wave_shr:1 row_mask:0xf bank_mask:0xf bound_ctrl:0\n\t" \
+	"v_sub_f32_dpp v121, v121, %[dr] wave_shr:1 row_mask:0xf bank_mask:0xf bound_ctrl:0\n\t" \
+	"v_cvt_f32_i32_sdwa v68, sext(%[p9]) dst_sel:DWORD dst_unused:UNUSED_PAD src0_sel:WORD_0\n\t" \
+	"v_sub_f32_dpp v120, v120, %[dr] wave_shr:1 row_mask:0xf bank_mask:0xf bound_ctrl:0\n\t" \
+	"v_sub_f32_dpp v121, v121, %[di] wave_shr:1 row_mask:0xf bank_mask:0xf bound_ctrl:0\n\t" \
+	"v_max3_f32 %[amax], %[amax], |v66|, |v67|\n\t" \
+	"v_sub_f32_dpp v120, v120, %[di] wave_shr:1 row_mask:0xf bank_mask:0xf bound_ctrl:0\n\t" \
+	"v_add_f32_dpp v121, v121, %[dr] wave_shr:1 row_mask:0xf bank_mask:0xf bound_ctrl:0\n\t" \
+	"v_max3_f32 %[amax], %[amax], |v68|, |v69|\n\t" \
+	"v_sub_f32_dpp v120, v120, %[dr] wave_shr:1 row_mask:0xf bank_mask:0xf bound_ctrl:0\n\t" \
+	"v_sub_f32_dpp v121, v121, %[di] wave_shr:1 row_mask:0xf bank_mask:0xf bound_ctrl:0\n\t" \
+	"ds_write_b64 %[pl], v[66:67] offset:1024\n\t" \
+	"v_sub_f32_dpp v120, v120, %[di] wave_shr:1 row_mask:0xf bank_mask:0xf bound_ctrl:0\n\t" \
+	"v_add_f32_dpp v121, v121, %[dr] wave_shr:1 row_mask:0xf bank_mask:0xf bound_ctrl:0\n\t" \
+	"s_bfm_b64 exec, 49, 0\n\t" \
+	"ds_write_b64 %[pl], v[68:69] offset:1152\n\t" \
+	"s_mov_b64 exec, -1\n\t" \
 	"v_sub_f32_dpp v120, v120, %[dr] wave_shr:1 row_mask:0xf bank_mask:0xf bound_ctrl:0\n\t" \
 	"v_sub_f32_dpp v121, v121, %[di] wave_shr:1 row_mask:0xf bank_mask:0xf bound_ctrl:0\n\t" \
 	"s_nop 0\n\t" \
@@ -400,28 +463,30 @@
 	".Lnb_corrr_v5:\n\t" \
 	"v_sub_f32_e32 v120, 0, %[dr]\n\t" \
 	"v_sub_f32_e32 v121, 0, %[di]\n\t" \
-	"s_nop 0\n\t" \
-	"v_sub_f32_dpp v120, v120, %[di] wave_shr:1 row_mask:0xf bank_mask:0xf bound_ctrl:0\n\t" \
-	"v_add_f32_dpp v121, v121, %[dr] wave_shr:1 row_mask:0xf bank_mask:0xf bound_ctrl:0\n\t" \
-	"s_nop 0\n\t" \
-	"v_sub_f32_dpp v120, v120, %[dr] wave_shr:1 row_mask:0xf bank_mask:0xf bound_ctrl:0\n\t" \
-	"v_sub_f32_dpp v121, v121, %[di] wave_shr:1 row_mask:0xf bank_mask:0xf bound_ctrl:0\n\t" \
-	"s_nop 0\n\t" \
-	"v_add_f32_dpp v120, v120, %[di] wave_shr:1 row_mask:0xf bank_mask:0xf bound_ctrl:0\n\t" \
-	"v_sub_f32_dpp v121, v121, %[dr] wave_shr:1 row_mask:0xf bank_mask:0xf bound_ctrl:0\n\t" \
-	"s_nop 0\n\t" \
-	"v_add_f32_dpp v120, v120, %[dr] wave_shr:1 row_mask:0xf bank_mask:0xf bound_ctrl:0\n\t" \
-	"v_add_f32_dpp v121, v121, %[di] wave_shr:1 row_mask:0xf bank_mask:0xf bound_ctrl:0\n\t" \
-	"s_nop 0\n\t" \
-	"v_sub_f32_dpp v120, v120, %[di] wave_shr:1 row_mask:0xf bank_mask:0xf bound_ctrl:0\n\t" \
-	"v_add_f32_dpp v121, v121, %[dr] wave_shr:1 row_mask:0xf bank_mask:0xf bound_ctrl:0\n\t" \
-	"s_nop 0\n\t" \
-	"v_add_f32_dpp v120, v120, %[dr] wave_shr:1 row_mask:0xf bank_mask:0xf bound_ctrl:0\n\t" \
-	"v_add_f32_dpp v121, v121, %[di] wave_shr:1 row_mask:0xf bank_mask:0xf bound_ctrl:0\n\t" \
-	"s_nop 0\n\t" \
-	"v_sub_f32_dpp v120, v120, %[di] wave_shr:1 row_mask:0xf bank_mask:0xf bound_ctrl:0\n\t" \
-	"v_add_f32_dpp v121, v121, %[dr] wave_shr:1 row_mask:0xf bank_mask:0xf bound_ctrl:0\n\t" \
-	"s_nop 0\n\t" \
+	"v_cvt_f32_i32_sdwa v67, sext(%[p8]) dst_sel:DWORD dst_unused:UNUSED_PAD src0_sel:WORD_1\n\t" \
+	"v_sub_f32_dpp v120, v120, %[di] wave_shr:1 row_mask:0xf bank_mask:0xf bound_ctrl:0\n\t" \
+	"v_add_f32_dpp v121, v121, %[dr] wave_shr:1 row_mask:0xf bank_mask:0xf bound_ctrl:0\n\t" \
+	"v_cvt_f32_i32_sdwa v66, sext(%[p8]) dst_sel:DWORD dst_unused:UNUSED_PAD src0_sel:WORD_0\n\t" \
+	"v_sub_f32_dpp v120, v120, %[dr] wave_shr:1 row_mask:0xf bank_mask:0xf bound_ctrl:0\n\t" \
+	"v_sub_f32_dpp v121, v121, %[di] wave_shr:1 row_mask:0xf bank_mask:0xf bound_ctrl:0\n\t" \
+	"v_cvt_f32_i32_sdwa v69, sext(%[p9]) dst_sel:DWORD dst_unused:UNUSED_PAD src0_sel:WORD_1\n\t" \
+	"v_add_f32_dpp v120, v120, %[di] wave_shr:1 row_mask:0xf bank_mask:0xf bound_ctrl:0\n\t" \
+	"v_sub_f32_dpp v121, v121, %[dr] wave_shr:1 row_mask:0xf bank_mask:0xf bound_ctrl:0\n\t" \
+	"v_cvt_f32_i32_sdwa v68, sext(%[p9]) dst_sel:DWORD dst_unused:UNUSED_PAD src0_sel:WORD_0\n\t" \
+	"v_add_f32_dpp v120, v120, %[dr] wave_shr:1 row_mask:0xf bank_mask:0xf bound_ctrl:0\n\t" \
+	"v_add_f32_dpp v121, v121, %[di] wave_shr:1 row_mask:0xf bank_mask:0xf bound_ctrl:0\n\t" \
+	"v_max3_f32 %[amax], %[amax], |v66|, |v67|\n\t" \
+	"v_sub_f32_dpp v120, v120, %[di] wave_shr:1 row_mask:0xf bank_mask:0xf bound_ctrl:0\n\t" \
+	"v_add_f32_dpp v121, v121, %[dr] wave_shr:1 row_mask:0xf bank_mask:0xf bound_ctrl:0\n\t" \
+	"v_max3_f32 %[amax], %[amax], |v68|, |v69|\n\t" \
+	"v_add_f32_dpp v120, v120, %[dr] wave_shr:1 row_mask:0xf bank_mask:0xf bound_ctrl:0\n\t" \
+	"v_add_f32_dpp v121, v121, %[di] wave_shr:1 row_mask:0xf bank_mask:0xf bound_ctrl:0\n\t" \
+	"ds_write_b64 %[pl], v[66:67] offset:1024\n\t" \
+	"v_sub_f32_dpp v120, v120, %[di] wave_shr:1 row_mask:0xf bank_mask:0xf bound_ctrl:0\n\t" \
+	"v_add_f32_dpp v121, v121, %[dr] wave_shr:1 row_mask:0xf bank_mask:0xf bound_ctrl:0\n\t" \
+	"s_bfm_b64 exec, 49, 0\n\t" \
+	"ds_write_b64 %[pl], v[68:69] offset:1152\n\t" \
+	"s_mov_b64 exec, -1\n\t" \
 	"v_add_f32_dpp v120, v120, %[dr] wave_shr:1 row_mask:0xf bank_mask:0xf bound_ctrl:0\n\t" \
 	"v_add_f32_dpp v121, v121, %[di] wave_shr:1 row_mask:0xf bank_mask:0xf bound_ctrl:0\n\t" \
 	"s_nop 0\n\t" \
@@ -449,28 +514,30 @@
 	".Lnb_corrr_v6:\n\t" \
 	"v_sub_f32_e32 v120, 0, %[dr]\n\t" \
 	"v_sub_f32_e32 v121, 0, %[di]\n\t" \
-	"s_nop 0\n\t" \
-	"v_sub_f32_dpp v120, v120, %[di] wave_shr:1 row_mask:0xf bank_mask:0xf bound_ctrl:0\n\t" \
-	"v_add_f32_dpp v121, v121, %[dr] wave_shr:1 row_mask:0xf bank_mask:0xf bound_ctrl:0\n\t" \
-	"s_nop 0\n\t" \
-	"v_add_f32_dpp v120, v120, %[dr] wave_shr:1 row_mask:0xf bank_mask:0xf bound_ctrl:0\n\t" \
-	"v_add_f32_dpp v121, v121, %[di] wave_shr:1 row_mask:0xf bank_mask:0xf bound_ctrl:0\n\t" \
-	"s_nop 0\n\t" \
-	"v_add_f32_dpp v120, v120, %[di] wave_shr:1 row_mask:0xf bank_mask:0xf bound_ctrl:0\n\t" \
-	"v_sub_f32_dpp v121, v121, %[dr] wave_shr:1 row_mask:0xf bank_mask:0xf bound_ctrl:0\n\t" \
-	"s_nop 0\n\t" \
-	"v_sub_f32_dpp v120, v120, %[dr] wave_shr:1 row_mask:0xf bank_mask:0xf bound_ctrl:0\n\t" \
-	"v_sub_f32_dpp v121, v121, %[di] wave_shr:1 row_mask:0xf bank_mask:0xf bound_ctrl:0\n\t" \
-	"s_nop 0\n\t" \
-	"v_add_f32_dpp v120, v120, %[di] wave_shr:1 row_mask:0xf bank_mask:0xf bound_ctrl:0\n\t" \
-	"v_sub_f32_dpp v121, v121, %[dr] wave_shr:1 row_mask:0xf bank_mask:0xf bound_ctrl:0\n\t" \
-	"s_nop 0\n\t" \
-	"v_add_f32_dpp v120, v120, %[dr] wave_shr:1 row_mask:0xf bank_mask:0xf bound_ctrl:0\n\t" \
-	"v_add_f32_dpp v121, v121, %[di] wave_shr:1 row_mask:0xf bank_mask:0xf bound_ctrl:0\n\t" \
-	"s_nop 0\n\t" \
-	"v_add_f32_dpp v120, v120, %[di] wave_shr:1 row_mask:0xf bank_mask:0xf bound_ctrl:0\n\t" \
-	"v_sub_f32_dpp v121, v121, %[dr] wave_shr:1 row_mask:0xf bank_mask:0xf bound_ctrl:0\n\t" \
-	"s_nop 0\n\t" \
+	"v_cvt_f32_i32_sdwa v67, sext(%[p8]) dst_sel:DWORD dst_unused:UNUSED_PAD src0_sel:WORD_1\n\t" \
+	"v_sub_f32_dpp v120, v120, %[di] wave_shr:1 row_mask:0xf bank_mask:0xf bound_ctrl:0\n\t" \
+	"v_add_f32_dpp v121, v121, %[dr] wave_shr:1 row_mask:0xf bank_mask:0xf bound_ctrl:0\n\t" \
+	"v_cvt_f32_i32_sdwa v66, sext(%[p8]) dst_sel:DWORD dst_unused:UNUSED_PAD src0_sel:WORD_0\n\t" \
+	"v_add_f32_dpp v120, v120, %[dr] wave_shr:1 row_mask:0xf bank_mask:0xf bound_ctrl:0\n\t" \
+	"v_add_f32_dpp v121, v121, %[di] wave_shr:1 row_mask:0xf bank_mask:0xf bound_ctrl:0\n\t" \
+	"v_cvt_f32_i32_sdwa v69, sext(%[p9]) dst_sel:DWORD dst_unused:UNUSED_PAD src0_sel:WORD_1\n\t" \
+	"v_add_f32_dpp v120, v120, %[di] wave_shr:1 row_mask:0xf bank_mask:0xf bound_ctrl:0\n\t" \
+	"v_sub_f32_dpp v121, v121, %[dr] wave_shr:1 row_mask:0xf bank_mask:0xf bound_ctrl:0\n\t" \
+	"v_cvt_f32_i32_sdwa v68, sext(%[p9]) dst_sel:DWORD dst_unused:UNUSED_PAD src0_sel:WORD_0\n\t" \
+	"v_sub_f32_dpp v120, v120, %[dr] wave_shr:1 row_mask:0xf bank_mask:0xf bound_ctrl:0\n\t" \
+	"v_sub_f32_dpp v121, v121, %[di] wave_shr:1 row_mask:0xf bank_mask:0xf bound_ctrl:0\n\t" \
+	"v_max3_f32 %[amax], %[amax], |v66|, |v67|\n\t" \
+	"v_add_f32_dpp v120, v120, %[di] wave_shr:1 row_mask:0xf bank_mask:0xf bound_ctrl:0\n\t" \
+	"v_sub_f32_dpp v121, v121, %[dr] wave_shr:1 row_mask:0xf bank_mask:0xf bound_ctrl:0\n\t" \
+	"v_max3_f32 %[amax], %[amax], |v68|, |v69|\n\t" \
+	"v_add_f32_dpp v120, v120, %[dr] wave_shr:1 row_mask:0xf bank_mask:0xf bound_ctrl:0\n\t" \
+	"v_add_f32_dpp v121, v121, %[di] wave_shr:1 row_mask:0xf bank_mask:0xf bound_ctrl:0\n\t" \
+	"ds_write_b64 %[pl], v[66:67] offset:1024\n\t" \
+	"v_add_f32_dpp v120, v120, %[di] wave_shr:1 row_mask:0xf bank_mask:0xf bound_ctrl:0\n\t" \
+	"v_sub_f32_dpp v121, v121, %[dr] wave_shr:1 row_mask:0xf bank_mask:0xf bound_ctrl:0\n\t" \
+	"s_bfm_b64 exec, 49, 0\n\t" \
+	"ds_write_b64 %[pl], v[68:69] offset:1152\n\t" \
+	"s_mov_b64 exec, -1\n\t" \
 	"v_add_f32_dpp v120, v120, %[dr] wave_shr:1 row_mask:0xf bank_mask:0xf bound_ctrl:0\n\t" \
 	"v_add_f32_dpp v121, v121, %[di] wave_shr:1 row_mask:0xf bank_mask:0xf bound_ctrl:0\n\t" \
 	"s_nop 0\n\t" \
@@ -498,28 +565,30 @@
 	".Lnb_corrr_v7:\n\t" \
 	"v_sub_f32_e32 v120, 0, %[dr]\n\t" \
 	"v_sub_f32_e32 v121, 0, %[di]\n\t" \
-	"s_nop 0\n\t" \
-	"v_sub_f32_dpp v120, v120, %[di] wave_shr:1 row_mask:0xf bank_mask:0xf bound_ctrl:0\n\t" \
-	"v_add_f32_dpp v121, v121, %[dr] wave_shr:1 row_mask:0xf bank_mask:0xf bound_ctrl:0\n\t" \
-	"s_nop 0\n\t" \
-	"v_add_f32_dpp v120, v120, %[dr] wave_shr:1 row_mask:0xf bank_mask:0xf bound_ctrl:0\n\t" \
-	"v_add_f32_dpp v121, v121, %[di] wave_shr:1 row_mask:0xf bank_mask:0xf bound_ctrl:0\n\t" \
-	"s_nop 0\n\t" \
-	"v_sub_f32_dpp v120, v120, %[di] wave_shr:1 row_mask:0xf bank_mask:0xf bound_ctrl:0\n\t" \
-	"v_add_f32_dpp v121, v121, %[dr] wave_shr:1 row_mask:0xf bank_mask:0xf bound_ctrl:0\n\t" \
-	"s_nop 0\n\t" \
-	"v_add_f32_dpp v120, v120, %[dr] wave_shr:1 row_mask:0xf bank_mask:0xf bound_ctrl:0\n\t" \
-	"v_add_f32_dpp v121, v121, %[di] wave_shr:1 row_mask:0xf bank_mask:0xf bound_ctrl:0\n\t" \
-	"s_nop 0\n\t" \
-	"v_add_f32_dpp v120, v120, %[di] wave_shr:1 row_mask:0xf bank_mask:0xf bound_ctrl:0\n\t" \
-	"v_sub_f32_dpp v121, v121, %[dr] wave_shr:1 row_mask:0xf bank_mask:0xf bound_ctrl:0\n\t" \
-	"s_nop 0\n\t" \
-	"v_add_f32_dpp v120, v120, %[dr] wave_shr:1 row_mask:0xf bank_mask:0xf bound_ctrl:0\n\t" \
-	"v_add_f32_dpp v121, v121, %[di] wave_shr:1 row_mask:0xf bank_mask:0xf bound_ctrl:0\n\t" \
-	"s_nop 0\n\t" \
-	"v_sub_f32_dpp v120, v120, %[di] wave_shr:1 row_mask:0xf bank_mask:0xf bound_ctrl:0\n\t" \
-	"v_add_f32_dpp v121, v121, %[dr] wave_shr:1 row_mask:0xf bank_mask:0xf bound_ctrl:0\n\t" \
-	"s_nop 0\n\t" \
+	"v_cvt_f32_i32_sdwa v67, sext(%[p8]) dst_sel:DWORD dst_unused:UNUSED_PAD src0_sel:WORD_1\n\t" \
+	"v_sub_f32_dpp v120, v120, %[di] wave_shr:1 row_mask:0xf bank_mask:0xf bound_ctrl:0\n\t" \
+	"v_add_f32_dpp v121, v121, %[dr] wave_shr:1 row_mask:0xf bank_mask:0xf bound_ctrl:0\n\t" \
+	"v_cvt_f32_i32_sdwa v66, sext(%[p8]) dst_sel:DWORD dst_unused:UNUSED_PAD src0_sel:WORD_0\n\t" \
+	"v_add_f32_dpp v120, v120, %[dr] wave_shr:1 row_mask:0xf bank_mask:0xf bound_ctrl:0\n\t" \
+	"v_add_f32_dpp v121, v121, %[di] wave_shr:1 row_mask:0xf bank_mask:0xf bound_ctrl:0\n\t" \
+	"v_cvt_f32_i32_sdwa v69, sext(%[p9]) dst_sel:DWORD dst_unused:UNUSED_PAD src0_sel:WORD_1\n\t" \
+	"v_sub_f32_dpp v120, v120, %[di] wave_shr:1 row_mask:0xf bank_mask:0xf bound_ctrl:0\n\t" \
+	"v_add_f32_dpp v121, v121, %[dr] wave_shr:1 row_mask:0xf bank_mask:0xf bound_ctrl:0\n\t" \
+	"v_cvt_f32_i32_sdwa v68, sext(%[p9]) dst_sel:DWORD dst_unused:UNUSED_PAD src0_sel:WORD_0\n\t" \
+	"v_add_f32_dpp v120, v120, %[dr] wave_shr:1 row_mask:0xf bank_mask:0xf bound_ctrl:0\n\t" \
+	"v_add_f32_dpp v121, v121, %[di] wave_shr:1 row_mask:0xf bank_mask:0xf bound_ctrl:0\n\t" \
+	"v_max3_f32 %[amax], %[amax], |v66|, |v67|\n\t" \
+	"v_add_f32_dpp v120, v120, %[di] wave_shr:1 row_mask:0xf bank_mask:0xf bound_ctrl:0\n\t" \
+	"v_sub_f32_dpp v121, v121, %[dr] wave_shr:1 row_mask:0xf bank_mask:0xf bound_ctrl:0\n\t" \
+	"v_max3_f32 %[amax], %[amax], |v68|, |v69|\n\t" \
+	"v_add_f32_dpp v120, v120, %[dr] wave_shr:1 row_mask:0xf bank_mask:0xf bound_ctrl:0\n\t" \
+	"v_add_f32_dpp v121, v121, %[di] wave_shr:1 row_mask:0xf bank_mask:0xf bound_ctrl:0\n\t" \
+	"ds_write_b64 %[pl], v[66:67] offset:1024\n\t" \
+	"v_sub_f32_dpp v120, v120, %[di] wave_shr:1 row_mask:0xf bank_mask:0xf bound_ctrl:0\n\t" \
+	"v_add_f32_dpp v121, v121, %[dr] wave_shr:1 row_mask:0xf bank_mask:0xf bound_ctrl:0\n\t" \
+	"s_bfm_b64 exec, 49, 0\n\t" \
+	"ds_write_b64 %[pl], v[68:69] offset:1152\n\t" \
+	"s_mov_b64 exec, -1\n\t" \
 	"v_add_f32_dpp v120, v120, %[dr] wave_shr:1 row_mask:0xf bank_mask:0xf bound_ctrl:0\n\t" \
 	"v_add_f32_dpp v121, v121, %[di] wave_shr:1 row_mask:0xf bank_mask:0xf bound_ctrl:0\n\t" \
 	"s_nop 0\n\t" \
@@ -556,6 +625,16 @@
 	"s_waitcnt lgkmcnt(0)\n\t" \
 	"s_branch .Lnb_corr_end\n\t" \
 	".Lnb_corrr_mul:\n\t" \
+	"v_cvt_f32_i32_sdwa v67, sext(%[p8]) dst_sel:DWORD dst_unused:UNUSED_PAD src0_sel:WORD_1\n\t" \
+	"v_cvt_f32_i32_sdwa v66, sext(%[p8]) dst_sel:DWORD dst_unused:UNUSED_PAD src0_sel:WORD_0\n\t" \
+	"v_cvt_f32_i32_sdwa v69, sext(%[p9]) dst_sel:DWORD dst_unused:UNUSED_PAD src0_sel:WORD_1\n\t" \
+	"v_cvt_f32_i32_sdwa v68, sext(%[p9]) dst_sel:DWORD dst_unused:UNUSED_PAD src0_sel:WORD_0\n\t" \
+	"v_max3_f32 %[amax], %[amax], |v66|, |v67|\n\t" \
+	"v_max3_f32 %[amax], %[amax], |v68|, |v69|\n\t" \
+	"ds_write_b64 %[pl], v[66:67] offset:1024\n\t" \
+	"s_bfm_b64 exec, 49, 0\n\t" \
+	"ds_write_b64 %[pl], v[68:69] offset:1152\n\t" \
+	"s_mov_b64 exec, -1\n\t" \
 	"s_bfm_b64 exec, %[len], 19\n\t" \
 	"ds_read_b64 v[88:89], %[vdm] offset:0\n\t" \
 	"ds_read_b64 v[90:91], %[vdm] offset:8\n\t" \
@@ -683,6 +762,16 @@
 	"v_pk_add_f32 v[120:121], v[120:121], v[86:87]\n\t" \
 	"s_branch .Lnb_corrr_join\n\t" \
 	".Lnb_corr_wide:\n\t" \
+	"v_cvt_f32_i32_sdwa v67, sext(%[p8]) dst_sel:DWORD dst_unused:UNUSED_PAD src0_sel:WORD_1\n\t" \
+	"v_cvt_f32_i32_sdwa v66, sext(%[p8]) dst_sel:DWORD dst_unused:UNUSED_PAD src0_sel:WORD_0\n\t" \
+	"v_cvt_f32_i32_sdwa v69, sext(%[p9]) dst_sel:DWORD dst_unused:UNUSED_PAD src0_sel:WORD_1\n\t" \
+	"v_cvt_f32_i32_sdwa v68, sext(%[p9]) dst_sel:DWORD dst_unused:UNUSED_PAD src0_sel:WORD_0\n\t" \
+	"v_max3_f32 %[amax], %[amax], |v66|, |v67|\n\t" \
+	"v_max3_f32 %[amax], %[amax], |v68|, |v69|\n\t" \
+	"ds_write_b64 %[pl], v[66:67] offset:1024\n\t" \
+	"s_bfm_b64 exec, 49, 0\n\t" \
+	"ds_write_b64 %[pl], v[68:69] offset:1152\n\t" \
+	"s_mov_b64 exec, -1\n\t" \
 	"v_mov_b64_e32 v[120:121], 0\n\t" \
 	"s_bfm_b64 exec, %[len], 0\n\t" \
 	"ds_read_b64 v[88:89], %[vd] offset:0\n\t" \
```

Result: no change. 1066 (-0.3%).
